# Lagrange-Labs/mapreduce-plonky2

Measured on AMD Instinct MI355X. Metric: leaf proofs/sec (whole node) + NTT GB/s vs HBM peak, 2^20-row table build, 1/2/4/8 GPU, higher is better.
Workload: dtype u64 (Goldilocks field)

## Files before the change

### mapreduce-plonky2_amd/csrc/fri.h

```cpp
#pragma once
#include "gl.cuh"

namespace mp2g {

struct ChState {
  u64 state[12];
  u64 in[8];
  u64 out[8];
  u32 n_in, n_out;
};
struct OracleRef {
  const u64* coeffs;
  const u64* values;
  const u64* levels;
  u64 coeff_bstride, value_bstride, level_bstride;
  u32 w;
};
struct FriShape {
  u32 log_n, rate_bits, cap_h, n_oracles;
  u32 n_polys;
  u32 zs_oracle, zs_count;
  u32 lookup_count;
  OracleRef o[8];
};
GLHD u32 fri_batch_len(const FriShape& sh, u32 batch) { return batch ? sh.zs_count + sh.lookup_count : sh.n_polys; }
GLHD void fri_batch_poly(const FriShape& sh, u32 batch, u32 j, u32& o, u32& p) {
  const u32 zo = sh.zs_oracle, wz = sh.o[zo].w - sh.lookup_count;
  if (batch) { o = zo; p = j < sh.zs_count ? j : wz + (j - sh.zs_count); return; }
  for (u32 oi = 0; oi < sh.n_oracles; oi++) {
    const u32 w = oi == zo ? wz : sh.o[oi].w;
    if (j < w) { o = oi; p = j; return; }
    j -= w;
  }
  o = zo; p = wz + j;
}
struct FriLayers {
  u32 n_layers;
  u32 arity_bits[8];
  const u64* values[8];
  const u64* levels[8];
  u64 value_bstride[8], level_bstride[8];
};

hipError_t challenger_init(hipStream_t s, ChState* st, u32 B);
hipError_t challenger_step(hipStream_t s, int variant, ChState* st, u32 B, const u64* obs, u64 obs_bstride, u32 n_obs,
                           u64* out, u64 out_bstride, u32 n_get);
hipError_t fri_openings(hipStream_t s, const FriShape& sh, u32 B, const u64* zeta, u64 zeta_bstride, u64* out);
hipError_t fri_final_poly(hipStream_t s, const FriShape& sh, u32 B, const u64* alpha, u64 alpha_bstride, const u64* zeta,
                          u64 zeta_bstride, u64* comp, u64* quot, u64* final_poly);
hipError_t fri_fold_values(hipStream_t s, u32 B, u32 log_m, u32 ab, const u64* in, u64 in_bstride, u64* out, u64 out_bstride,
                           const u64* beta, u64 beta_bstride, u64 shift);
hipError_t fri_fold_coeffs(hipStream_t s, u32 B, u32 n_in, u32 ab, const u64* in, u64 in_bstride, u64* out, u64 out_bstride,
                           const u64* beta, u64 beta_bstride, bool aos_out);
hipError_t fri_soa_to_aos(hipStream_t s, u32 B, u32 n, const u64* in, u64 in_bstride, u32 n_in, u64* out, u64 out_bstride);
#define FRI_POW_STRIDE 16
hipError_t fri_pow(hipStream_t s, int variant, const ChState* st, u32 B, u32 bits, u64* witness);
hipError_t fri_queries(hipStream_t s, const FriShape& sh, const FriLayers& ly, u32 B, u32 num_queries, const u64* chal,
                       u64 chal_bstride, u64* proof, u64 proof_bstride, u64 q_off, u64 q_words);
hipError_t bind_public_inputs(hipStream_t s, u32 B, u64* wires, u64 wires_bstride, u64 n, u32 row, const u64* pi_hash);
hipError_t copy_rows(hipStream_t s, u32 B, const u64* src, u64 src_bstride, u64* dst, u64 dst_bstride, u32 words);
}
```

### mapreduce-plonky2_amd/csrc/fri.hip

```cpp
#include "fri.h"
#include "poseidon_wave.cuh"

namespace mp2g {

template <int V>
__device__ void ch_duplex(ChState& c) {
  for (u32 i = 0; i < c.n_in; i++) c.state[i] = c.in[i];
  c.n_in = 0;
  u64 s[12];
#pragma unroll
  for (int i = 0; i < 12; i++) s[i] = c.state[i];
  perm<V>(s);
#pragma unroll
  for (int i = 0; i < 12; i++) c.state[i] = s[i];
#pragma unroll
  for (int i = 0; i < 8; i++) c.out[i] = s[i];
  c.n_out = 8;
}
template <int V>
__global__ void ch_kernel(ChState* st, u32 B, const u64* obs, u64 obs_bstride, u32 n_obs, u64* out, u64 out_bstride, u32 n_get) {
  u32 b = blockIdx.x * blockDim.x + threadIdx.x;
  if (b >= B) return;
  ChState c = st[b];
  const u64* o = obs + b * obs_bstride;
  for (u32 i = 0; i < n_obs; i++) {
    c.n_out = 0;
    c.in[c.n_in++] = o[i];
    if (c.n_in == 8) ch_duplex<V>(c);
  }
  u64* dst = out + b * out_bstride;
  for (u32 i = 0; i < n_get; i++) {
    if (c.n_in || !c.n_out) ch_duplex<V>(c);
    dst[i] = c.out[--c.n_out];
  }
  st[b] = c;
}
__global__ void __launch_bounds__(64) ch_wave_kernel(ChState* st, u32 B, const u64* obs, u64 obs_bstride, u32 n_obs, u64* out,
                                                     u64 out_bstride, u32 n_get) {
  const u32 gid = blockIdx.x * blockDim.x + threadIdx.x;
  const u32 braw = gid >> 4, l = gid & 15;
  const bool active = braw < B;
  const u32 b = active ? braw : B - 1;
  ChState* c = st + b;
  u64 x = l < 12 ? c->state[l] : 0;
  u64 inb = l < 8 ? c->in[l] : 0, outb = l < 8 ? c->out[l] : 0;
  u32 n_in = c->n_in, n_out = c->n_out;
  const u64* o = obs + b * obs_bstride;
  auto duplex = [&]() {
    if (l < n_in) x = inb;
    n_in = 0;
    x = wp2_perm(x, (int)l);
    outb = x;
    n_out = 8;
  };
  for (u32 i = 0; i < n_obs; i++) {
    u64 e = o[i];
    n_out = 0;
    if (l == n_in) inb = e;
    if (++n_in == 8) duplex();
  }
  u64* dst = out + b * out_bstride;
  for (u32 i = 0; i < n_get; i++) {
    if (n_in || !n_out) duplex();
    --n_out;
    if (active && l == n_out) dst[i] = outb;
  }
  if (!active) return;
  if (l < 12) c->state[l] = x;
  if (l < 8) { c->in[l] = inb; c->out[l] = outb; }
  if (l == 0) { c->n_in = n_in; c->n_out = n_out; }
}
__global__ void ch_init_kernel(ChState* st, u32 B) {
  u32 b = blockIdx.x * blockDim.x + threadIdx.x;
  if (b >= B) return;
  ChState c;
  for (int i = 0; i < 12; i++) c.state[i] = 0;
  for (int i = 0; i < 8; i++) { c.in[i] = 0; c.out[i] = 0; }
  c.n_in = c.n_out = 0;
  st[b] = c;
}
hipError_t challenger_init(hipStream_t s, ChState* st, u32 B) {
  hipLaunchKernelGGL(ch_init_kernel, dim3((B + 63) / 64), dim3(64), 0, s, st, B);
  return hipGetLastError();
}
hipError_t challenger_step(hipStream_t s, int variant, ChState* st, u32 B, const u64* obs, u64 obs_bstride, u32 n_obs,
                           u64* out, u64 out_bstride, u32 n_get) {
  if (variant == MP2G_POSEIDON2)
    hipLaunchKernelGGL(ch_wave_kernel, dim3((B * 16 + 63) / 64), dim3(64), 0, s, st, B, obs, obs_bstride, n_obs, out, out_bstride, n_get);
  else
    hipLaunchKernelGGL((ch_kernel<MP2G_POSEIDON>), dim3((B + 63) / 64), dim3(64), 0, s, st, B, obs, obs_bstride, n_obs, out, out_bstride, n_get);
  return hipGetLastError();
}

__global__ void __launch_bounds__(256) openings_kernel(FriShape sh, const u64* zeta , u64 zeta_bstride, u64* out ) {
  const u32 j = blockIdx.x, b = blockIdx.y, t = threadIdx.x;
  const u32 n = 1u << sh.log_n;
  u32 o, p;
  gl2 x = gl2_make(zeta[b * zeta_bstride], zeta[b * zeta_bstride + 1]);
  if (j >= sh.n_polys) {
    fri_batch_poly(sh, 1, j - sh.n_polys, o, p);
    x = gl2_scale(x, gl_root_of_unity(sh.log_n));
  } else {
    fri_batch_poly(sh, 0, j, o, p);
  }
  const u64* c = sh.o[o].coeffs + b * sh.o[o].coeff_bstride + ((u64)p << sh.log_n);
  gl2 x256 = gl2_pow(x, 256), acc = gl2_make(0, 0);
  if (t < n) {
    u32 top = ((n - 1 - t) >> 8);
    for (int k = (int)top; k >= 0; k--) {
      acc = gl2_mul(acc, x256);
      acc.a = gl_add(acc.a, c[t + ((u32)k << 8)]);
    }
    acc = gl2_mul(acc, gl2_pow(x, t));
  }
  __shared__ u64 ra[256], rb[256];
  ra[t] = acc.a; rb[t] = acc.b;
  __syncthreads();
  for (int s = 128; s > 0; s >>= 1) {
    if ((int)t < s) { ra[t] = gl_add(ra[t], ra[t + s]); rb[t] = gl_add(rb[t], rb[t + s]); }
    __syncthreads();
  }
  if (t == 0) {
    u64* d = out + ((u64)b * (sh.n_polys + sh.zs_count + sh.lookup_count) + j) * 2;
    d[0] = ra[0]; d[1] = rb[0];
  }
}

__global__ void __launch_bounds__(256) compose_kernel(FriShape sh, const u64* alpha, u64 alpha_bstride, u64* comp) {
  const u32 n = 1u << sh.log_n;
  const u32 i = blockIdx.x * 256 + threadIdx.x, b = blockIdx.y, batch = blockIdx.z;
  if (i >= n) return;
  gl2 al = gl2_make(alpha[b * alpha_bstride], alpha[b * alpha_bstride + 1]);
  gl2 acc = gl2_make(0, 0);
  const u32 zo = sh.zs_oracle, wz = sh.o[zo].w - sh.lookup_count;
  auto run = [&](u32 o, u32 first, u32 count) {
    const u64* base = sh.o[o].coeffs + b * sh.o[o].coeff_bstride + i;
    for (int p = (int)(first + count) - 1; p >= (int)first; p--) {
      acc = gl2_mul(acc, al);
      acc.a = gl_add(acc.a, base[(u64)p << sh.log_n]);
    }
  };
  if (sh.lookup_count) run(zo, wz, sh.lookup_count);
  if (batch == 0) {
    for (int o = (int)sh.n_oracles - 1; o >= 0; o--) run((u32)o, 0, (u32)o == zo ? wz : sh.o[o].w);
  } else {
    run(zo, 0, sh.zs_count);
  }
  u64* d = comp + (((u64)b * 2 + batch) * 2) * n;
  d[i] = acc.a;
  d[n + i] = acc.b;
}

__global__ void __launch_bounds__(1024) divide_kernel(u32 log_n, const u64* zeta, u64 zeta_bstride, const u64* comp, u64* quot) {
  const u32 n = 1u << log_n, batch = blockIdx.x, b = blockIdx.y, t = threadIdx.x;
  const u32 T = n < 1024 ? n : 1024, S = n / T;
  gl2 z = gl2_make(zeta[b * zeta_bstride], zeta[b * zeta_bstride + 1]);
  if (batch == 1) z = gl2_scale(z, gl_root_of_unity(log_n));
  const u64* c0 = comp + (((u64)b * 2 + batch) * 2) * n;
  const u64* c1 = c0 + n;
  u64* q0 = quot + (((u64)b * 2 + batch) * 2) * n;
  u64* q1 = q0 + n;
  __shared__ u64 la[1024], lb[1024];
  gl2 L = gl2_make(0, 0);
  if (t < T) {
    for (int k = (int)S - 1; k >= 0; k--) {
      L = gl2_mul(L, z);
      L.a = gl_add(L.a, c0[t * S + k]);
      L.b = gl_add(L.b, c1[t * S + k]);
    }
  }
  la[t] = 0; lb[t] = 0;
  __syncthreads();
  if (t < T && t >= 1) { la[t - 1] = L.a; lb[t - 1] = L.b; }
  __syncthreads();
  gl2 zp = gl2_pow(z, S);
  for (u32 d = 1; d < T; d <<= 1) {
    gl2 add = gl2_make(0, 0);
    if (t + d < T) add = gl2_mul(zp, gl2_make(la[t + d], lb[t + d]));
    __syncthreads();
    if (t < T) { la[t] = gl_add(la[t], add.a); lb[t] = gl_add(lb[t], add.b); }
    __syncthreads();
    zp = gl2_mul(zp, zp);
  }
  if (t < T) {
    gl2 s = gl2_make(la[t], lb[t]);
    for (int k = (int)S - 1; k >= 0; k--) {
      u32 i = t * S + k;
      s = gl2_mul(s, z);
      s.a = gl_add(s.a, c0[i]);
      s.b = gl_add(s.b, c1[i]);
      if (i >= 1) { q0[i - 1] = s.a; q1[i - 1] = s.b; }
    }
    if (t == T - 1) { q0[n - 1] = 0; q1[n - 1] = 0; }
  }
}
__global__ void __launch_bounds__(256) combine_kernel(u32 log_n, u32 zs_count, const u64* alpha, u64 alpha_bstride, const u64* quot, u64* final_poly) {
  const u32 n = 1u << log_n, i = blockIdx.x * 256 + threadIdx.x, b = blockIdx.y;
  if (i >= n) return;
  gl2 sh = gl2_pow(gl2_make(alpha[b * alpha_bstride], alpha[b * alpha_bstride + 1]), zs_count);
  const u64* q = quot + (u64)b * 4 * n;
  gl2 r = gl2_add(gl2_mul(gl2_make(q[i], q[n + i]), sh), gl2_make(q[2 * n + i], q[3 * n + i]));
  final_poly[(u64)b * 2 * n + i] = r.a;
  final_poly[(u64)b * 2 * n + n + i] = r.b;
}

template <int AB>
__global__ void __launch_bounds__(256) fold_values_kernel(u32 log_m, const u64* in, u64 in_bstride, u64* out, u64 out_bstride,
                                                            const u64* beta, u64 beta_bstride, u64 shift_inv, u64 w_m_inv, u64 arity_inv) {
  constexpr int A = 1 << AB;
  const u32 m = 1u << log_m, chunks = m >> AB;
  const u32 c = blockIdx.x * 256 + threadIdx.x, b = blockIdx.y;
  if (c >= chunks) return;
  const u64* v0 = in + b * in_bstride + ((u64)c << AB);
  const u64* v1 = v0 + m;
  gl2 x[A];
#pragma unroll
  for (int k = 0; k < A; k++) x[k] = gl2_make(v0[k], v1[k]);
  const u64 wA_inv = gl_pow(w_m_inv, m >> AB);
#pragma unroll
  for (int s = 1; s <= AB; s++) {
    const int mm = 1 << s, h = mm >> 1;
    u64 wstep = wA_inv;
    for (int e = s; e < AB; e++) wstep = gl_sqr(wstep);
    u64 w = 1;
#pragma unroll
    for (int j = 0; j < h; j++) {
#pragma unroll
      for (int k = 0; k < A; k += mm) {
        gl2 t = j == 0 ? x[k + j + h] : gl2_scale(x[k + j + h], w);
        gl2 u = x[k + j];
        x[k + j] = gl2_add(u, t);
        x[k + j + h] = gl2_sub(u, t);
      }
      w = gl_mul(w, wstep);
    }
  }
  u64 x0_inv = gl_mul(shift_inv, gl_pow(w_m_inv, bitrev32(c, log_m - AB)));
  gl2 g = gl2_scale(gl2_make(beta[b * beta_bstride], beta[b * beta_bstride + 1]), x0_inv);
  gl2 acc = x[A - 1];
#pragma unroll
  for (int j = A - 2; j >= 0; j--) acc = gl2_add(gl2_mul(acc, g), x[j]);
  acc = gl2_scale(acc, arity_inv);
  u64* o = out + b * out_bstride;
  o[c] = acc.a;
  o[chunks + c] = acc.b;
}
__global__ void __launch_bounds__(256) fold_coeffs_kernel(u32 n_out, u32 ab, const u64* in, u64 in_bstride, u32 n_in, u64* out, u64 out_bstride,
                                                            const u64* beta, u64 beta_bstride, int aos_out) {
  const u32 i = blockIdx.x * 256 + threadIdx.x, b = blockIdx.y;
  if (i >= n_out) return;
  const u32 A = 1u << ab;
  const u64* c0 = in + b * in_bstride + ((u64)i << ab);
  const u64* c1 = c0 + n_in;
  gl2 be = gl2_make(beta[b * beta_bstride], beta[b * beta_bstride + 1]);
  gl2 acc = gl2_make(0, 0);
  for (int j = (int)A - 1; j >= 0; j--) acc = gl2_add(gl2_mul(acc, be), gl2_make(c0[j], c1[j]));
  u64* o = out + b * out_bstride;
  if (aos_out) { o[2 * i] = acc.a; o[2 * i + 1] = acc.b; }
  else { o[i] = acc.a; o[n_out + i] = acc.b; }
}
__global__ void soa_to_aos_kernel(u32 n, const u64* in, u64 in_bstride, u32 n_in, u64* out, u64 out_bstride) {
  const u32 i = blockIdx.x * blockDim.x + threadIdx.x, b = blockIdx.y;
  if (i >= n) return;
  out[b * out_bstride + 2 * i] = in[b * in_bstride + i];
  out[b * out_bstride + 2 * i + 1] = in[b * in_bstride + n_in + i];
}

#define POW_THREADS 256
#define POW_STRIDE 16
template <int V>
__global__ void __launch_bounds__(POW_THREADS) pow_kernel(const ChState* st, u32 bits, unsigned long long* witness) {
  const u32 b = blockIdx.y;
  const ChState& c = st[b];
  unsigned long long* wit = witness + (u64)b * POW_STRIDE;
  __shared__ unsigned long long s_best;
  u64 base[12];
#pragma unroll
  for (int i = 0; i < 12; i++) base[i] = c.state[i];
  const u32 pos = c.n_in;
#pragma unroll
  for (int i = 0; i < 8; i++)
    if ((u32)i < pos) base[i] = c.in[i];
  const u64 stride = (u64)gridDim.x * blockDim.x;
  for (u64 cand = (u64)blockIdx.x * blockDim.x + threadIdx.x;; cand += stride) {
    if (threadIdx.x == 0) s_best = atomicMin(wit, ~0ull);
    __syncthreads();
    const unsigned long long best = s_best;
    __syncthreads();
    if (cand - threadIdx.x > best) break;
    u64 s[12];
#pragma unroll
    for (int i = 0; i < 12; i++) s[i] = base[i];
#pragma unroll
    for (int i = 0; i < 8; i++)
      if ((u32)i == pos) s[i] = cand;
    perm<V>(s);
    if (cand < GL_P && (bits == 0 || (s[7] >> (64 - bits)) == 0)) atomicMin(wit, (unsigned long long)cand);
  }
}
__global__ void fill_u64_kernel(u64* p, u64 v, u32 n) {
  u32 i = blockIdx.x * blockDim.x + threadIdx.x;
  if (i < n) p[i] = v;
}

__global__ void __launch_bounds__(256) query_kernel(FriShape sh, FriLayers ly, const u64* chal , u64 chal_bstride,
                                                      u64* proof, u64 proof_bstride, u64 q_off, u64 q_words) {
  const u32 q = blockIdx.x, b = blockIdx.y, t = threadIdx.x;
  const u32 lg = sh.log_n + sh.rate_bits;
  const u64 N = (u64)1 << lg;
  u64 x = chal[b * chal_bstride + q] % N;
  u64* o = proof + b * proof_bstride + q_off + q * q_words;
  const u32 depth = lg - sh.cap_h;
  for (u32 oi = 0; oi < sh.n_oracles; oi++) {
    const OracleRef& r = sh.o[oi];
    const u64* vals = r.values + b * r.value_bstride;
    for (u32 p = t; p < r.w; p += 256) o[p] = vals[(u64)p * N + x];
    o += r.w;
    const u64* lv = r.levels + b * r.level_bstride;
    for (u32 e = t; e < depth * 4; e += 256) {
      u32 l = e >> 2, k = e & 3;
      u64 off = 0;
      for (u32 j = 0; j < l; j++) off += (u64)4 << (lg - j);
      o[e] = lv[off + 4 * ((x >> l) ^ 1) + k];
    }
    o += depth * 4;
  }
  u32 clg = lg;
  for (u32 li = 0; li < ly.n_layers; li++) {
    const u32 ab = ly.arity_bits[li], A = 1u << ab;
    const u64 m = (u64)1 << clg;
    x >>= ab;
    clg -= ab;
    const u64* v = ly.values[li] + b * ly.value_bstride[li];
    for (u32 e = t; e < 2 * A; e += 256) o[e] = v[(e & 1) * m + (x << ab) + (e >> 1)];
    o += 2 * A;
    const u32 d2 = clg - sh.cap_h;
    const u64* lv = ly.levels[li] + b * ly.level_bstride[li];
    for (u32 e = t; e < d2 * 4; e += 256) {
      u32 l = e >> 2, k = e & 3;
      u64 off = 0;
      for (u32 j = 0; j < l; j++) off += (u64)4 << (clg - j);
      o[e] = lv[off + 4 * ((x >> l) ^ 1) + k];
    }
    o += d2 * 4;
  }
}
__global__ void copy_rows_kernel(const u64* src, u64 src_bstride, u64* dst, u64 dst_bstride, u32 words) {
  u32 i = blockIdx.x * blockDim.x + threadIdx.x, b = blockIdx.y;
  if (i < words) dst[b * dst_bstride + i] = src[b * src_bstride + i];
}

__global__ void bind_pi_kernel(u64* wires, u64 wires_bstride, u64 n, u32 row, const u64* pi_hash, u32 B) {
  u32 t = blockIdx.x * blockDim.x + threadIdx.x;
  if (t < 4 * B) wires[(t >> 2) * wires_bstride + (u64)(t & 3) * n + row] = pi_hash[t];
}

#define HIPCHK(x) do { hipError_t e_ = (x); if (e_ != hipSuccess) return e_; } while (0)

hipError_t fri_openings(hipStream_t s, const FriShape& sh, u32 B, const u64* zeta, u64 zeta_bstride, u64* out) {
  hipLaunchKernelGGL(openings_kernel, dim3(sh.n_polys + sh.zs_count + sh.lookup_count, B), dim3(256), 0, s, sh, zeta, zeta_bstride, out);
  return hipGetLastError();
}
hipError_t fri_final_poly(hipStream_t s, const FriShape& sh, u32 B, const u64* alpha, u64 alpha_bstride, const u64* zeta, u64 zeta_bstride,
                          u64* comp, u64* quot, u64* final_poly) {
  const u32 n = 1u << sh.log_n;
  hipLaunchKernelGGL(compose_kernel, dim3((n + 255) / 256, B, 2), dim3(256), 0, s, sh, alpha, alpha_bstride, comp);
  hipLaunchKernelGGL(divide_kernel, dim3(2, B), dim3(1024), 0, s, sh.log_n, zeta, zeta_bstride, comp, quot);
  hipLaunchKernelGGL(combine_kernel, dim3((n + 255) / 256, B), dim3(256), 0, s, sh.log_n, sh.zs_count + sh.lookup_count, alpha, alpha_bstride, quot,
                     final_poly);
  return hipGetLastError();
}
hipError_t fri_fold_values(hipStream_t s, u32 B, u32 log_m, u32 ab, const u64* in, u64 in_bstride, u64* out, u64 out_bstride,
                           const u64* beta, u64 beta_bstride, u64 shift) {
  const u32 chunks = (1u << log_m) >> ab;
  const u64 shift_inv = gl_inv(shift), w_m_inv = gl_inv(gl_root_of_unity(log_m)), a_inv = gl_inv((u64)1 << ab);
  dim3 g((chunks + 255) / 256, B), bl(256);
#define FV(N) case N: hipLaunchKernelGGL((fold_values_kernel<N>), g, bl, 0, s, log_m, in, in_bstride, out, out_bstride, beta, beta_bstride, shift_inv, w_m_inv, a_inv); break;
  switch (ab) { FV(1) FV(2) FV(3) FV(4) default: return hipErrorInvalidValue; }
#undef FV
  return hipGetLastError();
}
hipError_t fri_fold_coeffs(hipStream_t s, u32 B, u32 n_in, u32 ab, const u64* in, u64 in_bstride, u64* out, u64 out_bstride,
                           const u64* beta, u64 beta_bstride, bool aos_out) {
  const u32 n_out = n_in >> ab;
  hipLaunchKernelGGL(fold_coeffs_kernel, dim3((n_out + 255) / 256, B), dim3(256), 0, s, n_out, ab, in, in_bstride, n_in, out, out_bstride, beta, beta_bstride, aos_out ? 1 : 0);
  return hipGetLastError();
}
hipError_t fri_soa_to_aos(hipStream_t s, u32 B, u32 n, const u64* in, u64 in_bstride, u32 n_in, u64* out, u64 out_bstride) {
  hipLaunchKernelGGL(soa_to_aos_kernel, dim3((n + 255) / 256, B), dim3(256), 0, s, n, in, in_bstride, n_in, out, out_bstride);
  return hipGetLastError();
}
hipError_t fri_pow(hipStream_t s, int variant, const ChState* st, u32 B, u32 bits, u64* witness) {
  hipLaunchKernelGGL(fill_u64_kernel, dim3((B * POW_STRIDE + 63) / 64), dim3(64), 0, s, witness, ~(u64)0, B * POW_STRIDE);
  const u32 lanes = 1u << 19;
  u32 blocks = lanes / POW_THREADS / (B ? B : 1);
  if (blocks < 8) blocks = 8;
  if (blocks > 1024) blocks = 1024;
  dim3 g(blocks, B), bl(POW_THREADS);
  if (variant == MP2G_POSEIDON2) hipLaunchKernelGGL((pow_kernel<MP2G_POSEIDON2>), g, bl, 0, s, st, bits, (unsigned long long*)witness);
  else hipLaunchKernelGGL((pow_kernel<MP2G_POSEIDON>), g, bl, 0, s, st, bits, (unsigned long long*)witness);
  return hipGetLastError();
}
hipError_t fri_queries(hipStream_t s, const FriShape& sh, const FriLayers& ly, u32 B, u32 num_queries, const u64* chal, u64 chal_bstride,
                       u64* proof, u64 proof_bstride, u64 q_off, u64 q_words) {
  if (!num_queries) return hipSuccess;
  hipLaunchKernelGGL(query_kernel, dim3(num_queries, B), dim3(256), 0, s, sh, ly, chal, chal_bstride, proof, proof_bstride, q_off, q_words);
  return hipGetLastError();
}
hipError_t bind_public_inputs(hipStream_t s, u32 B, u64* wires, u64 wires_bstride, u64 n, u32 row, const u64* pi_hash) {
  hipLaunchKernelGGL(bind_pi_kernel, dim3((4 * B + 63) / 64), dim3(64), 0, s, wires, wires_bstride, n, row, pi_hash, B);
  return hipGetLastError();
}
hipError_t copy_rows(hipStream_t s, u32 B, const u64* src, u64 src_bstride, u64* dst, u64 dst_bstride, u32 words) {
  if (!words) return hipSuccess;
  hipLaunchKernelGGL(copy_rows_kernel, dim3((words + 255) / 256, B), dim3(256), 0, s, src, src_bstride, dst, dst_bstride, words);
  return hipGetLastError();
}
}
```

### mapreduce-plonky2_amd/csrc/gates.h

```cpp
#pragma once
#include "gl.cuh"
#include "mp2g.h"
namespace mp2g {
struct GateTable {
  u32 n_gates, num_selectors;
  u32 num_lookup_selectors;
  mp2g_gate g[MP2G_MAX_GATES];
};
const char* gate_table_check(const GateTable& t, u32 num_constants, u32 wires_w);
u32 gate_num_constraints(const mp2g_gate& g);
u32 gate_degree(const mp2g_gate& g);
hipError_t gate_constraints_lde(hipStream_t s, u32 B, const GateTable& t, const u64* C, const u64* W, u64 w_bstride, u32 lg,
                                const u64* alphas, u64 al_bstride, u32 nc, const u64* pi_hash, u64* q);
hipError_t gate_constraints_points(hipStream_t s, const GateTable& t, const u64* consts, const u64* wires, u64 npts, u32 max_j,
                                   const u64* pi_hash, u64* out);
hipError_t gate_check(hipStream_t s, u32 B, const GateTable& t, const u64* consts, const u64* wires, u64 w_bstride, u64 npts,
                      const u64* pi_hash, u32* flags);
}
```

### mapreduce-plonky2_amd/csrc/gates.hip

```cpp
#include "gates.h"
#include "poseidon.cuh"

namespace mp2g {

u32 gate_num_constraints(const mp2g_gate& g) {
  switch (g.kind) {
    case MP2G_GATE_CONSTANT: return g.p0;
    case MP2G_GATE_PUBLIC_INPUT: return 4;
    case MP2G_GATE_ARITHMETIC: return g.p0;
    case MP2G_GATE_BASE_SUM: return 1 + g.p0;
    case MP2G_GATE_ARITHMETIC_EXT: case MP2G_GATE_MUL_EXT: return 2 * g.p0;
    case MP2G_GATE_POSEIDON2: case MP2G_GATE_POSEIDON: return 1 + 4 + 36 + 22 + 48 + 12;
    case MP2G_GATE_POSEIDON_MDS: return 24;
    case MP2G_GATE_COSET_INTERPOLATION: return 4 + 4 * (((1u << g.p0) - 2) / (g.p1 - 1));
    case MP2G_GATE_U32_ARITHMETIC: return 36 * g.p0;
    case MP2G_GATE_U32_RANGE_CHECK: return 17 * g.p0;
    case MP2G_GATE_U32_SUBTRACTION: return 19 * g.p0;
    case MP2G_GATE_U32_ADD_MANY: return 21 * g.p1;
    case MP2G_GATE_COMPARISON: return g.p1 ? 6 + 5 * g.p1 + (g.p0 + g.p1 - 1) / g.p1 : 0;
    case MP2G_GATE_EXPONENTIATION: return g.p0 + 1;
    case MP2G_GATE_REDUCING: case MP2G_GATE_REDUCING_EXT: return 2 * g.p0;
    case MP2G_GATE_RANDOM_ACCESS: return (g.p0 + 2) * g.p1 + g.p2;
    case MP2G_GATE_U32_INTERLEAVE: return 34 * g.p0;
    case MP2G_GATE_UNINTERLEAVE_TO_B32: case MP2G_GATE_UNINTERLEAVE_TO_U32: return 67 * g.p0;
// ... 273 lines not shown
        s[i + 4] = gl_sub(rhs, delta);
      }
#pragma unroll
      for (int i = 8; i < 12; i++) s[i] = wire(i);
#pragma unroll 1
      for (int r = 0; r < 30; r++) {
        if (r >= 4 && r < 26) {
          u64 in = wire(65 + (r - 4));
          emit(diff(s[0], c_p_rc[12 * r], in));
          s[0] = p2_sbox(in, 0);
#pragma unroll
          for (int i = 1; i < 12; i++) s[i] = gl_addw(s[i], c_p_rc[12 * r + i]);
        } else if (r == 0) {
#pragma unroll
          for (int i = 0; i < 12; i++) s[i] = p2_sbox(s[i], c_p_rc[i]);
        } else {
          const int base = r < 4 ? 29 + 12 * (r - 1) : 87 + 12 * (r - 26);
#pragma unroll
          for (int i = 0; i < 12; i++) {
            u64 in = wire(base + i);
            emit(diff(s[i], c_p_rc[12 * r + i], in));
            s[i] = p2_sbox(in, 0);
          }
        }
        poseidon_mds(s);
      }
#pragma unroll
      for (int i = 0; i < 12; i++) emit(diff0(s[i], wire(12 + i)));
      break;
    }
    case MP2G_GATE_POSEIDON_MDS: {
      u64 s0[12], s1[12];
#pragma unroll
      for (int i = 0; i < 12; i++) { s0[i] = wire(2 * i); s1[i] = wire(2 * i + 1); }
      poseidon_mds(s0);
      poseidon_mds(s1);
#pragma unroll
      for (int i = 0; i < 12; i++) {
        emit(gl_sub(wire(24 + 2 * i), gl_canon(s0[i])));
        emit(gl_sub(wire(25 + 2 * i), gl_canon(s1[i])));
      }
      break;
    }
    case MP2G_GATE_COSET_INTERPOLATION: {
      const u32 npts = 1u << g.p0, deg = g.p1, nint = (npts - 2) / (deg - 1);
      const u32 w_pt = 1 + 2 * npts, w_val = w_pt + 2, w_int = w_val + 2, w_sh = w_int + 4 * nint;
      const Alg pt{wire(w_pt), wire(w_pt + 1)}, sh{wire(w_sh), wire(w_sh + 1)};
      Alg d0 = alg_sub(pt, alg_scale(sh, wire(0)));
      emit(d0.a); emit(d0.b);
      const u64 om = gl_root_of_unity(g.p0), ninv = gl_inv(npts);
      u64 xi = 1;
      Alg ev{0, 0}, pr{1, 0};
      u32 start = 0, end = deg;
      for (u32 c = 0; c <= nint; c++) {
        for (u32 i = start; i < end; i++) {
          Alg val = alg_scale(Alg{wire(1 + 2 * i), wire(2 + 2 * i)}, gl_mul(xi, ninv));
          Alg term{gl_sub(sh.a, xi), sh.b};
          Alg nev = alg_add(alg_mul(ev, term), alg_mul(val, pr));
          pr = alg_mul(pr, term);
          ev = nev;
          xi = gl_mul(xi, om);
        }
        if (c == nint) break;
        Alg iev{wire(w_int + 2 * c), wire(w_int + 2 * c + 1)}, ipr{wire(w_int + 2 * (nint + c)), wire(w_int + 2 * (nint + c) + 1)};
        Alg d1 = alg_sub(iev, ev), d2 = alg_sub(ipr, pr);
        emit(d1.a); emit(d1.b); emit(d2.a); emit(d2.b);
        ev = iev; pr = ipr;
        start = 1 + (deg - 1) * (c + 1);
        end = start + deg - 1 < npts ? start + deg - 1 : npts;
      }
      Alg d3 = alg_sub(Alg{wire(w_val), wire(w_val + 1)}, ev);
      emit(d3.a); emit(d3.b);
      break;
    }
    case MP2G_GATE_U32_ARITHMETIC: {
      const u32 ops = g.p0;
      for (u32 i = 0; i < ops; i++) {
        const u32 b = 6 * i;
        const u64 computed = gl_mul_add(wire(b), wire(b + 1), wire(b + 2));
        const u64 lo = wire(b + 3), hi = wire(b + 4), inv = wire(b + 5);
        const u64 hi_not_max = gl_sub(gl_mul(inv, gl_sub(0xFFFFFFFFull, hi)), 1);
        emit(gl_mul(hi_not_max, lo));
        emit(gl_sub(gl_mul_add(hi, (u64)1 << 32, lo), computed));
        u64 clo = 0, chi = 0, lm[16];
        load16(6 * ops + 32 * i + 16, 16, lm);
#pragma unroll
        for (int j = 15; j >= 0; j--) { emit(range4(lm[j])); chi = horner4(chi, lm[j]); }
        load16(6 * ops + 32 * i, 16, lm);
#pragma unroll
        for (int j = 15; j >= 0; j--) { emit(range4(lm[j])); clo = horner4(clo, lm[j]); }
        emit(subx(clo, lo));
        emit(subx(chi, hi));
      }
      break;
    }
    case MP2G_GATE_U32_RANGE_CHECK: {
      const u32 k = g.p0;
      for (u32 i = 0; i < k; i++) {
        u64 lm[16];
        load16(k + 16 * i, 16, lm);
        u64 acc = 0;
#pragma unroll
        for (int j = 15; j >= 0; j--) acc = horner4(acc, lm[j]);
        emit(subx(acc, wire(i)));
#pragma unroll
        for (int j = 0; j < 16; j++) emit(range4(lm[j]));
      }
      break;
    }
    case MP2G_GATE_U32_SUBTRACTION: {
      const u32 ops = g.p0;
      for (u32 i = 0; i < ops; i++) {
        const u32 b = 5 * i;
        const u64 initial = gl_sub(gl_sub(wire(b), wire(b + 1)), wire(b + 2));
        const u64 res = wire(b + 3), bo = wire(b + 4);
        emit(gl_sub(res, gl_add(initial, gl_mul((u64)1 << 32, bo))));
        u64 comb = 0, lm[16];
        load16(5 * ops + 16 * i, 16, lm);
#pragma unroll
        for (int j = 15; j >= 0; j--) { emit(range4(lm[j])); comb = horner4(comb, lm[j]); }
        emit(subx(comb, res));
        emit(gl_mul(bo, gl_sub(1, bo)));
      }
      break;
    }
    case MP2G_GATE_U32_ADD_MANY: {
      const u32 na = g.p0, ops = g.p1, per = na + 3;
      for (u32 i = 0; i < ops; i++) {
        const u32 b = per * i;
        u64 computed = wire(b + na);
        for (u32 j = 0; j < na; j++) computed = gl_add(computed, wire(b + j));
        const u64 res = wire(b + na + 1), co = wire(b + na + 2);
        emit(gl_sub(gl_mul_add(co, (u64)1 << 32, res), computed));
        u64 cres = 0, ccar = 0, lm[16];
        {
          const u64 l17 = wire(per * ops + 18 * i + 17), l16 = wire(per * ops + 18 * i + 16);
          load16(per * ops + 18 * i, 16, lm);
          emit(range4(l17)); ccar = l17;
          emit(range4(l16)); ccar = horner4(ccar, l16);
        }
#pragma unroll
        for (int j = 15; j >= 0; j--) { emit(range4(lm[j])); cres = horner4(cres, lm[j]); }
        emit(subx(cres, res));
        emit(subx(ccar, co));
      }
      break;
    }
    case MP2G_GATE_COMPARISON: {
      const u32 nch = g.p1, cb = (g.p0 + nch - 1) / nch, cs = 1u << cb;
      const u32 o_fc = 4, o_sc = 4 + nch, o_ed = 4 + 2 * nch, o_ce = 4 + 3 * nch, o_iv = 4 + 4 * nch, o_bits = 4 + 5 * nch;
      u64 a1 = 0, a2 = 0;
      for (u32 i = nch; i-- > 0;) { a1 = gl_add(gl_mul_small(a1, cs), wire(o_fc + i)); a2 = gl_add(gl_mul_small(a2, cs), wire(o_sc + i)); }
      emit(gl_sub(a1, wire(0)));
      emit(gl_sub(a2, wire(1)));
      u64 msd = 0;
      for (u32 i = 0; i < nch; i++) {
        const u64 f = wire(o_fc + i), sc = wire(o_sc + i), ce = wire(o_ce + i), iv = wire(o_iv + i);
        u64 p1 = f, p2 = sc;
        for (u32 x = 1; x < cs; x++) { p1 = mulx(p1, gl_sub(f, x)); p2 = mulx(p2, gl_sub(sc, x)); }
        emit(p1);
        emit(p2);
        const u64 diff = gl_sub(sc, f);
        emit(gl_sub(gl_mul(diff, wire(o_ed + i)), gl_sub(1, ce)));
        emit(gl_mul(ce, diff));
        emit(gl_sub(iv, gl_mul(ce, msd)));
        msd = gl_add(iv, gl_mul(gl_sub(1, ce), diff));
      }
      const u64 msd_w = wire(3);
      emit(gl_sub(msd_w, msd));
      u64 bc = 0;
      for (u32 i = cb + 1; i-- > 0;) bc = gl_add(gl_add(bc, bc), wire(o_bits + i));
      for (u32 i = 0; i <= cb; i++) { const u64 bit = wire(o_bits + i); emit(gl_mul(bit, gl_sub(1, bit))); }
      emit(gl_sub(gl_add(cs, msd_w), bc));
      emit(gl_sub(wire(2), wire(o_bits + cb)));
      break;
    }
    case MP2G_GATE_EXPONENTIATION: {
      const u32 nb = g.p0;
      const u64 base = wire(0);
      u64 prev_int = 1;
      for (u32 i = 0; i < nb; i++) {
        u64 prev = i == 0 ? 1 : gl_mul(prev_int, prev_int);
        u64 bit = wire(1 + (nb - 1 - i));
        u64 mulby = gl_mul_add(bit, base, gl_sub(1, bit));
        u64 cur = wire(nb + 2 + i);
        emit(gl_sub(gl_mul(prev, mulby), cur));
        prev_int = cur;
      }
      emit(gl_sub(wire(nb + 1), prev_int));
      break;
    }
    case MP2G_GATE_REDUCING:
    case MP2G_GATE_REDUCING_EXT: {
      const u32 n = g.p0;
      const bool ext = g.kind == MP2G_GATE_REDUCING_EXT;
      const u32 start_accs = 6 + (ext ? 2 * n : n);
      Alg alpha{wire(2), wire(3)}, acc{wire(4), wire(5)};
      for (u32 i = 0; i < n; i++) {
        Alg coeff = ext ? Alg{wire(6 + 2 * i), wire(7 + 2 * i)} : Alg{wire(6 + i), 0};
        Alg nxt = i == n - 1 ? Alg{wire(0), wire(1)} : Alg{wire(start_accs + 2 * i), wire(start_accs + 2 * i + 1)};
        Alg d = alg_sub(alg_add(alg_mul(acc, alpha), coeff), nxt);
        emit(d.a); emit(d.b);
        acc = nxt;
      }
      break;
    }
    case MP2G_GATE_RANDOM_ACCESS: {
      const u32 bits = g.p0, copies = g.p1, extra = g.p2, vs = 1u << bits;
      const u32 routed = (2 + vs) * copies + extra;
      for (u32 c = 0; c < copies; c++) {
        const u32 w0 = (2 + vs) * c, b0 = routed + c * bits;
        switch (bits) {
          case 1: ra_copy<1>(wire, emit, w0, b0); break;
          case 2: ra_copy<2>(wire, emit, w0, b0); break;
          case 3: ra_copy<3>(wire, emit, w0, b0); break;
          case 4: ra_copy<4>(wire, emit, w0, b0); break;
          default: {
            u64 items[32];
            for (u32 i = 0; i < bits; i++) {
              u64 b = wire(b0 + i);
              emit(gl_mul(b, gl_sub(b, 1)));
            }
            u64 idx = 0;
            for (u32 i = bits; i-- > 0;) idx = gl_add(gl_add(idx, idx), wire(b0 + i));
            emit(gl_sub(idx, wire(w0)));
            {
              const u64 b = wire(b0);
              for (u32 k = 0; k < vs / 2; k++) {
                u64 x = wire(w0 + 2 + 2 * k), y = wire(w0 + 3 + 2 * k);
                items[k] = gl_add(x, gl_mul(b, gl_sub(y, x)));
              }
            }
            for (u32 i = 1, len = vs / 2; i < bits; i++, len >>= 1) {
              const u64 b = wire(b0 + i);
              for (u32 k = 0; k < len / 2; k++) items[k] = gl_add(items[2 * k], gl_mul(b, gl_sub(items[2 * k + 1], items[2 * k])));
            }
            emit(gl_sub(items[0], wire(w0 + 1)));
          }
        }
      }
      for (u32 i = 0; i < extra; i++) emit(gl_sub(cst(i), wire((2 + vs) * copies + i)));
      break;
    }
    case MP2G_GATE_U32_INTERLEAVE: {
      const u32 ops = g.p0;
      u64 bt[16];
      for (u32 i = 0; i < ops; i++) {
        u64 x = 0, xi = 0;
        for (u32 h = 0; h < 2; h++) {
          load16(2 * ops + 32 * i + 16 * h, 16, bt);
#pragma unroll
          for (int j = 0; j < 16; j++) {
            emit(mulx(bt[j], gl_sub(1, bt[j])));
            x = gl_add(gl_add(x, x), bt[j]);
            xi = gl_add(gl_mul_small(xi, 4), bt[j]);
          }
        }
        emit(gl_sub(x, wire(2 * i)));
        emit(gl_sub(xi, wire(2 * i + 1)));
      }
      break;
    }
    case MP2G_GATE_UNINTERLEAVE_TO_B32:
    case MP2G_GATE_UNINTERLEAVE_TO_U32: {
      const u32 ops = g.p0;
      const bool spread = g.kind == MP2G_GATE_UNINTERLEAVE_TO_B32;
      u64 bt[16];
      for (u32 i = 0; i < ops; i++) {
        u64 x = 0, ev = 0, od = 0;
        for (u32 h = 0; h < 4; h++) {
          load16(3 * ops + 64 * i + 16 * h, 16, bt);
#pragma unroll
          for (int j = 0; j < 16; j++) {
            emit(mulx(bt[j], gl_sub(1, bt[j])));
            x = gl_add(gl_add(x, x), bt[j]);
            u64& d = (j & 1) ? ev : od;
            d = gl_add(spread ? gl_mul_small(d, 4) : gl_add(d, d), bt[j]);
          }
        }
        emit(gl_sub(x, wire(3 * i)));
        emit(gl_sub(ev, wire(3 * i + 1)));
        emit(gl_sub(od, wire(3 * i + 2)));
      }
      break;
    }
    default: break;
  }
}

template <class ConstAll>
GLD u64 gate_filter(const GateTable& t, u32 gi, ConstAll call) {
  const mp2g_gate& g = t.g[gi];
  const u64 s = call(g.selector_index);
  u64 f = 1;
  for (u32 r = g.group_start; r < g.group_end; r++)
    if (r != gi) f = gl_mul(f, gl_sub(r, s));
  if (t.num_selectors > 1) f = gl_mul(f, gl_sub(0xFFFFFFFFull, s));
  return f;
}

template <u32 KIND>
__global__ void __launch_bounds__(256) gate_constraints_lde_kernel(mp2g_gate g, u32 gi, u32 num_selectors, u32 cst_off, u32 n_cons,
                                                                   const u64* __restrict__ C, const u64* __restrict__ W,
                                                                   u64 w_bstride, u32 lg, const u64* __restrict__ alphas,
                                                                   u64 al_bstride, u32 nc, const u64* __restrict__ pi_hash,
                                                                   u64* __restrict__ q, int first) {
  __shared__ u64 apw[2][MP2G_MAX_GATE_CONSTRAINTS];
  const u64 N = (u64)1 << lg;
  const u32 p = blockIdx.x * 256 + threadIdx.x, b = blockIdx.y;
  for (u32 j = threadIdx.x; j < 2 * n_cons; j += 256) {
    const u32 a = j >= n_cons ? 1 : 0, e = j - a * n_cons;
    apw[a][e] = a < nc ? gl_pow(alphas[b * al_bstride + a], e) : 0;
  }
  __syncthreads();
  if (p >= N) return;
  g.kind = KIND;
  const u64* w = W + b * w_bstride + p;
  const u64* c = C + p;
  const u64* pih = pi_hash + 4 * b;
  auto wire = [&](u32 j) { return w[(u64)j << lg]; };
  auto cst = [&](u32 j) { return c[(u64)(cst_off + j) << lg]; };
  u64 f = 1;
  {
    const u64 s = c[(u64)g.selector_index << lg];
    for (u32 r = g.group_start; r < g.group_end; r++)
      if (r != gi) f = gl_mul(f, gl_sub(r, s));
    if (num_selectors > 1) f = gl_mul(f, gl_sub(0xFFFFFFFFull, s));
  }
  LazySum acc[2];
  u32 j = 0;
  eval_gate<true>(g, wire, cst, pih, [&](u64 v) {
#pragma unroll
    for (u32 a = 0; a < 2; a++) acc[a].add(v, apw[a][j]);
    j++;
  });
  const u32 i = bitrev32(p, lg);
  for (u32 a = 0; a < nc; a++) {
    u64 r = gl_mul(f, acc[a].value());
    u64* dst = q + (((u64)b * nc + a) << lg) + i;
    *dst = first ? r : gl_add(*dst, r);
  }
}

#define MP2G_MAX_LIGHT_GATES 12
struct LightGates {
  u32 n;
  mp2g_gate g[MP2G_MAX_LIGHT_GATES];
  u32 gi[MP2G_MAX_LIGHT_GATES];
};
static bool gate_is_light(const mp2g_gate& g) {
  switch (g.kind) {
    case MP2G_GATE_CONSTANT: case MP2G_GATE_PUBLIC_INPUT: case MP2G_GATE_ARITHMETIC: case MP2G_GATE_BASE_SUM:
    case MP2G_GATE_ARITHMETIC_EXT: case MP2G_GATE_MUL_EXT: return true;
    default: return false;
  }
}
__global__ void __launch_bounds__(256) gate_constraints_lde_light_kernel(LightGates lg_, u32 num_selectors, u32 cst_off, u32 max_cons,
                                                                         const u64* __restrict__ C, const u64* __restrict__ W,
                                                                         u64 w_bstride, u32 lg, const u64* __restrict__ alphas,
                                                                         u64 al_bstride, u32 nc, const u64* __restrict__ pi_hash,
                                                                         u64* __restrict__ q, int first) {
  __shared__ u64 apw[2][MP2G_MAX_GATE_CONSTRAINTS];
  const u64 N = (u64)1 << lg;
  const u32 p = blockIdx.x * 256 + threadIdx.x, b = blockIdx.y;
  for (u32 j = threadIdx.x; j < 2 * max_cons; j += 256) {
    const u32 a = j >= max_cons ? 1 : 0, e = j - a * max_cons;
    apw[a][e] = a < nc ? gl_pow(alphas[b * al_bstride + a], e) : 0;
  }
  __syncthreads();
  if (p >= N) return;
  const u64* w = W + b * w_bstride + p;
  const u64* c = C + p;
  const u64* pih = pi_hash + 4 * b;
  auto wire = [&](u32 j) { return w[(u64)j << lg]; };
  auto cst = [&](u32 j) { return c[(u64)(cst_off + j) << lg]; };
  u64 total[2] = {0, 0};
  for (u32 k = 0; k < lg_.n; k++) {
    mp2g_gate g = lg_.g[k];
    const u32 gi = lg_.gi[k];
    u64 f = 1;
    {
      const u64 s = c[(u64)g.selector_index << lg];
      for (u32 r = g.group_start; r < g.group_end; r++)
        if (r != gi) f = gl_mul(f, gl_sub(r, s));
      if (num_selectors > 1) f = gl_mul(f, gl_sub(0xFFFFFFFFull, s));
    }
    LazySum acc[2];
    u32 j = 0;
    auto emit = [&](u64 v) {
#pragma unroll
      for (u32 a = 0; a < 2; a++) acc[a].add(v, apw[a][j]);
      j++;
    };
    switch (g.kind) {
#define LIGHT_CASE(K) case K: g.kind = K; eval_gate<true>(g, wire, cst, pih, emit); break;
      LIGHT_CASE(MP2G_GATE_CONSTANT)
      LIGHT_CASE(MP2G_GATE_PUBLIC_INPUT)
      LIGHT_CASE(MP2G_GATE_ARITHMETIC)
      LIGHT_CASE(MP2G_GATE_BASE_SUM)
      LIGHT_CASE(MP2G_GATE_ARITHMETIC_EXT)
      LIGHT_CASE(MP2G_GATE_MUL_EXT)
#undef LIGHT_CASE
      default: break;
    }
    for (u32 a = 0; a < nc; a++) total[a] = gl_add(total[a], gl_mul(f, acc[a].value()));
  }
  const u32 i = bitrev32(p, lg);
  for (u32 a = 0; a < nc; a++) {
    u64* dst = q + (((u64)b * nc + a) << lg) + i;
    *dst = first ? total[a] : gl_add(*dst, total[a]);
  }
}

__global__ void __launch_bounds__(256) gate_constraints_points_kernel(GateTable t, const u64* __restrict__ consts,
                                                                      const u64* __restrict__ wires, u64 npts, u32 max_j,
                                                                      const u64* __restrict__ pih, u64* __restrict__ out) {
  const u64 p = (u64)blockIdx.x * 256 + threadIdx.x;
  if (p >= npts) return;
  auto wire = [&](u32 j) { return wires[(u64)j * npts + p]; };
  auto call = [&](u32 j) { return consts[(u64)j * npts + p]; };
  const u32 ns = t.num_selectors + t.num_lookup_selectors;
  auto cst = [&](u32 j) { return consts[(u64)(ns + j) * npts + p]; };
  for (u32 j = 0; j < max_j; j++) out[(u64)j * npts + p] = 0;
  for (u32 gi = 0; gi < t.n_gates; gi++) {
    if (t.g[gi].kind == MP2G_GATE_NOOP) continue;
    const u64 f = gate_filter(t, gi, call);
    u32 j = 0;
    eval_gate<false>(t.g[gi], wire, cst, pih, [&](u64 v) {
      u64* o = out + (u64)j * npts + p;
      *o = gl_add(*o, gl_mul(f, v));
      j++;
    });
  }
}

__global__ void __launch_bounds__(256) gate_check_kernel(GateTable t, const u64* __restrict__ consts, const u64* __restrict__ wires,
                                                         u64 w_bstride, u64 npts, const u64* __restrict__ pi_hash, u32* __restrict__ flags) {
  const u64 p = (u64)blockIdx.x * 256 + threadIdx.x;
  const u32 b = blockIdx.y;
  if (p >= npts) return;
  const u64* w = wires + b * w_bstride;
  auto wire = [&](u32 j) { return w[(u64)j * npts + p]; };
  auto call = [&](u32 j) { return consts[(u64)j * npts + p]; };
  const u32 ns = t.num_selectors + t.num_lookup_selectors;
  auto cst = [&](u32 j) { return consts[(u64)(ns + j) * npts + p]; };
  bool bad = false;
  for (u32 gi = 0; gi < t.n_gates; gi++) {
    if (t.g[gi].kind == MP2G_GATE_NOOP) continue;
    if (gate_filter(t, gi, call) == 0) continue;
    eval_gate<false>(t.g[gi], wire, cst, pi_hash + 4 * b, [&](u64 v) { bad |= v != 0; });
  }
  if (bad) atomicOr(&flags[b], 2u);
}
hipError_t gate_check(hipStream_t s, u32 B, const GateTable& t, const u64* consts, const u64* wires, u64 w_bstride, u64 npts,
                      const u64* pi_hash, u32* flags) {
  if (!npts || !B) return hipSuccess;
  hipLaunchKernelGGL(gate_check_kernel, dim3((u32)((npts + 255) / 256), B), dim3(256), 0, s, t, consts, wires, w_bstride, npts, pi_hash,
                     flags);
  return hipGetLastError();
}

hipError_t gate_constraints_lde(hipStream_t s, u32 B, const GateTable& t, const u64* C, const u64* W, u64 w_bstride, u32 lg,
                                const u64* alphas, u64 al_bstride, u32 nc, const u64* pi_hash, u64* q) {
  if (nc < 1 || nc > 2) return hipErrorInvalidValue;
  const u64 N = (u64)1 << lg;
  const dim3 grid((u32)((N + 255) / 256), B), block(256);
  int first = 1;
  LightGates lgs{};
  u32 light_cons = 0;
  for (u32 gi = 0; gi < t.n_gates; gi++) {
    const u32 n_cons = gate_num_constraints(t.g[gi]);
    if (n_cons && gate_is_light(t.g[gi]) && lgs.n < MP2G_MAX_LIGHT_GATES) {
      lgs.g[lgs.n] = t.g[gi]; lgs.gi[lgs.n] = gi; lgs.n++;
      if (n_cons > light_cons) light_cons = n_cons;
    }
  }
  if (lgs.n < 2) lgs.n = 0;
  if (lgs.n) {
    hipLaunchKernelGGL(gate_constraints_lde_light_kernel, grid, block, 0, s, lgs, t.num_selectors, t.num_selectors + t.num_lookup_selectors,
                       light_cons, C, W, w_bstride, lg, alphas, al_bstride, nc, pi_hash, q, first);
    first = 0;
  }
  for (u32 gi = 0; gi < t.n_gates; gi++) {
    const mp2g_gate& g = t.g[gi];
    const u32 n_cons = gate_num_constraints(g);
    if (!n_cons) continue;
    bool fused = false;
    for (u32 k = 0; k < lgs.n; k++) fused |= lgs.gi[k] == gi;
    if (fused) continue;
#define GATE_CASE(K)                                                                                                        \
  case K:                                                                                                                   \
    hipLaunchKernelGGL(gate_constraints_lde_kernel<K>, grid, block, 0, s, g, gi, t.num_selectors,                          \
                       t.num_selectors + t.num_lookup_selectors, n_cons, C, W, w_bstride, lg, alphas, al_bstride, nc, pi_hash, q, \
                       first);                                                                                              \
    break;
    switch (g.kind) {
      GATE_CASE(MP2G_GATE_CONSTANT)
      GATE_CASE(MP2G_GATE_PUBLIC_INPUT)
      GATE_CASE(MP2G_GATE_ARITHMETIC)
      GATE_CASE(MP2G_GATE_BASE_SUM)
      GATE_CASE(MP2G_GATE_ARITHMETIC_EXT)
      GATE_CASE(MP2G_GATE_MUL_EXT)
      GATE_CASE(MP2G_GATE_POSEIDON2)
      GATE_CASE(MP2G_GATE_EXPONENTIATION)
      GATE_CASE(MP2G_GATE_REDUCING)
      GATE_CASE(MP2G_GATE_REDUCING_EXT)
      GATE_CASE(MP2G_GATE_RANDOM_ACCESS)
      GATE_CASE(MP2G_GATE_POSEIDON)
      GATE_CASE(MP2G_GATE_POSEIDON_MDS)
      GATE_CASE(MP2G_GATE_COSET_INTERPOLATION)
      GATE_CASE(MP2G_GATE_U32_ARITHMETIC)
      GATE_CASE(MP2G_GATE_U32_RANGE_CHECK)
      GATE_CASE(MP2G_GATE_U32_SUBTRACTION)
      GATE_CASE(MP2G_GATE_U32_ADD_MANY)
      GATE_CASE(MP2G_GATE_COMPARISON)
      GATE_CASE(MP2G_GATE_U32_INTERLEAVE)
      GATE_CASE(MP2G_GATE_UNINTERLEAVE_TO_B32)
      GATE_CASE(MP2G_GATE_UNINTERLEAVE_TO_U32)
      default: return hipErrorInvalidValue;
    }
#undef GATE_CASE
    first = 0;
  }
  if (first) return hipMemsetAsync(q, 0, (size_t)B * nc * N * sizeof(u64), s);
  return hipGetLastError();
}
hipError_t gate_constraints_points(hipStream_t s, const GateTable& t, const u64* consts, const u64* wires, u64 npts, u32 max_j,
                                   const u64* pi_hash, u64* out) {
  if (!npts) return hipSuccess;
  hipLaunchKernelGGL(gate_constraints_points_kernel, dim3((u32)((npts + 255) / 256)), dim3(256), 0, s, t, consts, wires, npts, max_j,
                     pi_hash, out);
  return hipGetLastError();
}
}
```

### mapreduce-plonky2_amd/csrc/ntt.h

```cpp
#pragma once
#include "gl.cuh"
#include <map>
#include <memory>

namespace mp2g {

struct NttPlan {
  u32 log_n = 0, log_n1 = 0, log_n2 = 0;
  u64 *tw_a = nullptr, *tw_b = nullptr, *tw4_lo = nullptr, *tw4_hi = nullptr, *tw4_full = nullptr;
  u64 *tc_a = nullptr, *tc_b = nullptr;
  u64 n_inv = 0;
  ~NttPlan();
};
struct CosetTables {
  u32 log_n = 0, logK = 0;
  u64 shift = 0;
  u64 *lo = nullptr, *hi = nullptr, *full = nullptr;
  ~CosetTables();
};

struct NttEngine {
  hipStream_t stream = nullptr;
  std::map<u32, std::unique_ptr<NttPlan>> plans;
  std::map<u64, std::unique_ptr<CosetTables>> cosets;
  u64* scratch = nullptr;
  size_t scratch_words = 0;
  u64 generation = 0;
  ~NttEngine();

  hipError_t plan(u32 log_n, bool inverse, NttPlan** out);
  hipError_t coset(u32 log_n, u32 logK, u64 shift, CosetTables** out);
  hipError_t ensure_scratch(size_t words);
  hipError_t run(const u64* in, u64* out, u32 log_n, u32 polys, u32 logK, u64 in_poly_stride,
                 u64 out_poly_stride, bool inverse, const CosetTables* pre, bool bitrev_out);
  hipError_t scale_powers(u64* data, u32 log_n, u32 batch, u64 base, u64 first);
};

}
```

### mapreduce-plonky2_amd/csrc/ntt.hip

```cpp
#include "ntt.h"
#include <cstdlib>

namespace mp2g {

__device__ __forceinline__ int lds_pad(int a) { return a + (a >> 4); }

struct NttArgs {
  const u64* in;
  u64* out;
  u64 in_poly_stride, out_poly_stride;
  u32 logK;
  u32 log_n, log_n1, log_n2;
  u32 batch;
  const u64* tw;
  const u64* tw4_lo;
  const u64* tw4_hi;
  const u64* pre_lo;
  const u64* pre_hi;
  const u64* tw4_full;
  const u64* pre_full;
  u64 post;
  u32 bitrev_out;
  u32 inverse;
  const u64* tc;
// ... 242 lines not shown
  }
}

template <int LT, int LW>
__global__ void __launch_bounds__((NttGeom<LT, LW>::NT)) ntt_cols_kernel(NttArgs a, u64* dst_dense) {
  constexpr int T = 1 << LT, W = 1 << LW, E = T << LW, NT = NttGeom<LT, LW>::NT;
  extern __shared__ __align__(16) u64 smem[];
  u64* s = smem;
  u64* tw = smem + lds_pad(E) + 1;
  const int tid = threadIdx.x;
  for (int i = tid; i < R8Tw<LT>::LDS_WORDS; i += NT) tw[i] = a.tw[R8Tw<LT>::LDS_OFF + i];
  const u32 tiles_per = 1u << (a.log_n2 - LW);
  u32 bid = blockIdx.x;
  if ((gridDim.x & 7) == 0) bid = (bid & 7) * (gridDim.x >> 3) + (bid >> 3);
  const u32 b = bid / tiles_per, c0 = (bid % tiles_per) << LW;
  const u32 coset = b & ((1u << a.logK) - 1);
  const u64* src = in_base(a, b);
  for (int e = tid; e < E; e += NT) {
    int c = e & (W - 1), j = e >> LW;
    u64 v = src[((u64)j << a.log_n2) + c0 + c];
    if (a.pre_full) {
      v = gl_mul(v, a.pre_full[((u64)coset << a.log_n) + ((u64)j << a.log_n2) + c0 + c]);
    } else if (a.pre_lo) {
      v = gl_mul(v, a.pre_lo[((u64)coset << a.log_n2) + c0 + c]);
      v = gl_mul(v, a.pre_hi[((u64)coset << LT) + j]);
    }
    s[lds_pad(e)] = v;
  }
  __syncthreads();
  dif_all<LT, LT - 1, true, LW, NT>(s, tw, a.tw, tid, a.inverse != 0);
  u64* dst = dst_dense ? dst_dense + (u64)b * ((u64)1 << a.log_n) : out_base(a, b);
  for (int e = tid; e < E; e += NT) {
    int c = e & (W - 1), j = e >> LW;
    u64 v = s[lds_pad(e)];
    u64 w;
    if (a.tw4_full) {
      w = a.tw4_full[((u64)j << a.log_n2) + c0 + c];
    } else {
      u32 k1 = bitrev32((u32)j, LT);
      u32 ex = (c0 + c) * k1;
      w = gl_mul(a.tw4_lo[ex & 4095], a.tw4_hi[ex >> 12]);
    }
    dst[((u64)j << a.log_n2) + c0 + c] = gl_mul(v, w);
  }
}

template <int LT, int LW, bool COLS> struct WaveGeom {
  static constexpr int NBR = LT > 12 ? 2 : 1;
  static constexpr int LTS = LT - 3 * NBR;
  static constexpr int LWL = 9 - LTS;
  static constexpr bool OK = LT >= 3 && LT <= 13 && (!COLS || LT <= 12) && ((1 << LT) << LW) == 8 * NttGeom<LT, LW>::NT && (!COLS || LW >= LWL);
};
template <int LT, int LW, bool COLS> struct ShiftGeom {
  using G = WaveGeom<LT, LW, COLS>;
  static constexpr int L0 = LT - 3;
  static constexpr bool OK = G::OK && G::NBR == 1 && G::LTS >= 6 && (COLS ? (LW + L0 - 3 >= 6) : (LW == 0 && L0 - 3 >= 6));
  static constexpr int TC_WORDS = 64 << (L0 - 3);
};
__device__ __forceinline__ void wave_sync() {
  __builtin_amdgcn_fence(__ATOMIC_RELEASE, "wavefront");
  __builtin_amdgcn_wave_barrier();
  __builtin_amdgcn_fence(__ATOMIC_ACQUIRE, "wavefront");
}
template <int LT, int LTS, int HI, int R, bool COLS, int LWL, int LWS, bool MERGED = false>
__device__ __forceinline__ void wave_round(u64* s, int base, const u64* tw, int lane, bool inverse, const u64* __restrict__ tcw = nullptr) {
  constexpr int LO = HI - R + 1, WL = 1 << LWL;
  constexpr int ITEMS = 512 >> R;
#pragma unroll
  for (int item0 = 0; item0 < ITEMS; item0 += 64) {
    int item = item0 + lane;
    int c, rest;
    if (COLS) { c = item & (WL - 1); rest = item >> LWL; }
    else { rest = item & ((1 << (LTS - R)) - 1); c = item >> (LTS - R); }
    int below = rest & ((1 << LO) - 1), above = rest >> LO;
    int j0 = (above << (HI + 1)) | below;
    u64 x[1 << R];
#pragma unroll
    for (int m = 0; m < (1 << R); m++) {
      int j = j0 + (m << LO);
      x[m] = s[lds_pad(base + (COLS ? (j << LWS) + c : (c << LTS) + j))];
    }
    butterfly<LT, HI, R, false, MERGED>(x, below, tw, tcw, inverse);
#pragma unroll
    for (int m = 0; m < (1 << R); m++) {
      int j = j0 + (m << LO);
      s[lds_pad(base + (COLS ? (j << LWS) + c : (c << LTS) + j))] = x[m];
    }
  }
}
template <int LT, int LTS, int HI, bool COLS, int LWL, int LWS, bool SHIFT = false>
__device__ __forceinline__ void wave_rounds(u64* s, int base, const u64* tw, int lane, bool inverse, const u64* __restrict__ tcw = nullptr) {
  if constexpr (HI >= 0) {
    constexpr int R = (HI + 1 >= 3) ? 3 : HI + 1;
    wave_sync();
    wave_round<LT, LTS, HI, R, COLS, LWL, LWS, SHIFT>(s, base, tw, lane, inverse, tcw);
    wave_rounds<LT, LTS, HI - R, COLS, LWL, LWS, false>(s, base, tw, lane, inverse);
  }
}

template <int LT, int LW, bool SHIFT = false>
__global__ void __launch_bounds__((NttGeom<LT, LW>::NT)) __attribute__((amdgpu_waves_per_eu(8))) ntt_rows_v2_kernel(NttArgs a) {
  using G = WaveGeom<LT, LW, false>;
  static_assert(!SHIFT || ShiftGeom<LT, LW, false>::OK, "tile shape without wave-uniform shift twiddles");
  constexpr int T = 1 << LT, E = T << LW, NT = NttGeom<LT, LW>::NT, LTS = G::LTS, L0 = LT - 3;
  extern __shared__ __align__(16) u64 smem[];
  u64* s = smem;
  u64* tw = smem + lds_pad(E) + 1;
  const int tid = threadIdx.x, lane = tid & 63, wave = tid >> 6;
  for (int i = tid; i < R8Tw<LT>::LDS_WORDS; i += NT) tw[i] = a.tw[R8Tw<LT>::LDS_OFF + i];
  const u32 n1 = 1u << a.log_n1;
  const u64 total_rows = (u64)a.batch << a.log_n1;
  const u64 row0 = (u64)blockIdx.x << LW;
  const bool two_pass = a.log_n1 != 0, inverse = a.inverse != 0;
  {
    const int c = tid >> L0, below = tid & ((1 << L0) - 1);
    const u64 g = row0 + c;
    u64 x[8];
    if (g < total_rows) {
      u32 b = (u32)(g >> a.log_n1), jr = (u32)(g & (n1 - 1));
      if (two_pass) {
        const u64* src = out_base(a, b) + ((u64)jr << LT);
#pragma unroll
        for (int m = 0; m < 8; m++) x[m] = src[below + (m << L0)];
      } else {
        const u64* src = in_base(a, b);
#pragma unroll
        for (int m = 0; m < 8; m++) x[m] = src[below + (m << L0)];
        if (a.pre_lo) {
          const u64* pre = a.pre_lo + ((u64)(b & ((1u << a.logK) - 1)) << LT);
#pragma unroll
          for (int m = 0; m < 8; m++) x[m] = gl_mul(x[m], pre[below + (m << L0)]);
        }
      }
    } else {
#pragma unroll
      for (int m = 0; m < 8; m++) x[m] = 0;
    }
    if constexpr (SHIFT) {
      butterfly<LT, 2, 3>(x, 0, nullptr, nullptr, inverse);
      shift_twiddles(x, __builtin_amdgcn_readfirstlane(below >> (L0 - 3)), inverse);
    } else {
      butterfly<LT, LT - 1, 3, true>(x, below, tw, a.tw, inverse);
    }
#pragma unroll
    for (int m = 0; m < 8; m++) s[lds_pad((c << LT) + below + (m << L0))] = x[m];
  }
  __syncthreads();
  if constexpr (G::NBR == 2) {
    dif_round<LT, LT - 4, 3, false, LW, NT>(s, tw, a.tw, tid, inverse);
    __syncthreads();
  }
  if constexpr (SHIFT) {
    const int r = __builtin_amdgcn_readfirstlane((int)bitrev32((u32)(wave & 7), 3));
    wave_rounds<LT, LTS, LTS - 1, false, G::LWL, 0, true>(s, wave << 9, tw, lane, inverse, a.tc + (r << (L0 - 3)));
  } else {
    wave_rounds<LT, LTS, LTS - 1, false, G::LWL, 0>(s, wave << 9, tw, lane, inverse);
  }
  if (a.bitrev_out) {
    wave_sync();
    u64 v[8];
#pragma unroll
    for (int k = 0; k < 8; k++) v[k] = s[lds_pad((wave << 9) + lane + (k << 6))];
    if (a.post) {
#pragma unroll
      for (int k = 0; k < 8; k++) v[k] = gl_mul(v[k], a.post);
    }
#pragma unroll
    for (int k = 0; k < 8; k++) {
      int e = (wave << 9) + lane + (k << 6);
      int r = e >> LT, p = e & (T - 1);
      u64 g = row0 + r;
      if (g >= total_rows) continue;
      u32 b = (u32)(g >> a.log_n1), jr = (u32)(g & (n1 - 1));
      out_base(a, b)[((u64)jr << LT) + p] = v[k];
    }
  } else {
    __syncthreads();
    for (int e = tid; e < E; e += NT) {
      int r = e >> LT, p = e & (T - 1);
      u64 g = row0 + r;
      if (g >= total_rows) continue;
      u32 b = (u32)(g >> a.log_n1), jr = (u32)(g & (n1 - 1));
      u64 v = s[lds_pad((r << LT) + (int)bitrev32((u32)p, LT))];
      if (a.post) v = gl_mul(v, a.post);
      out_base(a, b)[((u64)jr << LT) + p] = v;
    }
  }
}

template <int LT, int LW, bool SHIFT = false>
__global__ void __launch_bounds__((NttGeom<LT, LW>::NT)) __attribute__((amdgpu_waves_per_eu(8))) ntt_cols_v2_kernel(NttArgs a, u64* dst_dense) {
  using G = WaveGeom<LT, LW, true>;
  static_assert(!SHIFT || ShiftGeom<LT, LW, true>::OK, "tile shape without wave-uniform shift twiddles");
  constexpr int W = 1 << LW, E = (1 << LT) << LW, NT = NttGeom<LT, LW>::NT, LTS = G::LTS, LWL = G::LWL;
  extern __shared__ __align__(16) u64 smem[];
  u64* s = smem;
  u64* tw = smem + lds_pad(E) + 1;
  const int tid = threadIdx.x, lane = tid & 63, wave = tid >> 6;
  for (int i = tid; i < R8Tw<LT>::LDS_WORDS; i += NT) tw[i] = a.tw[R8Tw<LT>::LDS_OFF + i];
  const u32 tiles_per = 1u << (a.log_n2 - LW);
  u32 bid = blockIdx.x;
  if ((gridDim.x & 7) == 0) bid = (bid & 7) * (gridDim.x >> 3) + (bid >> 3);
  const u32 b = bid / tiles_per, c0 = (bid % tiles_per) << LW;
  const u32 coset = b & ((1u << a.logK) - 1);
  const u64* src = in_base(a, b);
  const bool inverse = a.inverse != 0;
  {
    const int c = tid & (W - 1), below = tid >> LW;
    u64 x[8];
#pragma unroll
    for (int m = 0; m < 8; m++) x[m] = src[((u64)(below + (m << LTS)) << a.log_n2) + c0 + c];
    if (a.pre_full) {
      const u64* pre = a.pre_full + ((u64)coset << a.log_n) + c0 + c;
#pragma unroll
      for (int m = 0; m < 8; m++) x[m] = gl_mul(x[m], pre[(u64)(below + (m << LTS)) << a.log_n2]);
    } else if (a.pre_lo) {
      u64 pl = a.pre_lo[((u64)coset << a.log_n2) + c0 + c];
#pragma unroll
      for (int m = 0; m < 8; m++) x[m] = gl_mul(gl_mul(x[m], pl), a.pre_hi[((u64)coset << LT) + below + (m << LTS)]);
    }
    if constexpr (SHIFT) {
      butterfly<LT, 2, 3>(x, 0, nullptr, nullptr, inverse);
      shift_twiddles(x, __builtin_amdgcn_readfirstlane(below >> (LTS - 3)), inverse);
    } else {
      butterfly<LT, LT - 1, 3, true>(x, below, tw, a.tw, inverse);
    }
#pragma unroll
    for (int m = 0; m < 8; m++) s[lds_pad(((below + (m << LTS)) << LW) + c)] = x[m];
  }
  __syncthreads();
  {
    constexpr int GW = W >> LWL;
    const int cg = wave & (GW - 1), jh = wave / GW;
    if constexpr (SHIFT) {
      const int r = __builtin_amdgcn_readfirstlane((int)bitrev32((u32)jh, 3));
      wave_rounds<LT, LTS, LTS - 1, true, LWL, LW, true>(s, ((jh << LTS) << LW) + (cg << LWL), tw, lane, inverse, a.tc + (r << (LTS - 3)));
    } else {
      wave_rounds<LT, LTS, LTS - 1, true, LWL, LW>(s, ((jh << LTS) << LW) + (cg << LWL), tw, lane, inverse);
    }
  }
  __syncthreads();
  u64* dst = dst_dense ? dst_dense + (u64)b * ((u64)1 << a.log_n) : out_base(a, b);
#pragma unroll
  for (int k = 0; k < 8; k++) {
    int e = tid + k * NT;
    int c = e & (W - 1), j = e >> LW;
    u64 v = s[lds_pad(e)];
    u64 w;
    if (a.tw4_full) {
      w = a.tw4_full[((u64)j << a.log_n2) + c0 + c];
    } else {
      u32 k1 = bitrev32((u32)j, LT);
      u32 ex = (c0 + c) * k1;
      w = gl_mul(a.tw4_lo[ex & 4095], a.tw4_hi[ex >> 12]);
    }
    dst[((u64)j << a.log_n2) + c0 + c] = gl_mul(v, w);
  }
}

__global__ void r8_round_twiddles_kernel(u64* out, u64 w, u32 lo, u32 shift) {
  u32 i = blockIdx.x * blockDim.x + threadIdx.x;
  if (i >= (7u << lo)) return;
  u32 r = (i >> lo) + 1, below = i & ((1u << lo) - 1);
  out[i] = gl_pow(w, ((u64)below << shift) * r);
}
__global__ void merged_twiddles_kernel(u64* out, u64 w, u32 lb) {
  u32 i = blockIdx.x * blockDim.x + threadIdx.x;
  if (i >= (64u << lb)) return;
  out[i] = gl_pow(w, (u64)(i & ((1u << lb) - 1)) * (i >> lb));
}
__global__ void powers_kernel(u64* out, u64 base, u64 first, u64 stride_exp, u32 count) {
  u32 i = blockIdx.x * blockDim.x + threadIdx.x;
  if (i >= count) return;
  out[i] = gl_mul(first, gl_pow(base, (u64)i * stride_exp));
}
__global__ void coset_tables_kernel(u64* lo, u64* hi, u64 shift, u64 w_nk, u32 log_n1, u32 log_n2, u32 K) {
  u32 i = blockIdx.x * blockDim.x + threadIdx.x;
  u32 n1 = 1u << log_n1, n2 = 1u << log_n2;
  u32 per = n1 + n2;
  if (i >= per * K) return;
  u32 j = i / per, r = i % per;
  u64 sj = gl_mul(shift, gl_pow(w_nk, j));
  if (r < n2) lo[(u64)j * n2 + r] = gl_pow(sj, r);
  else hi[(u64)j * n1 + (r - n2)] = gl_pow(sj, (u64)(r - n2) << log_n2);
}
__global__ void tw4_full_kernel(u64* out, u64 wn, u32 log_n1, u32 log_n2) {
  u64 i = (u64)blockIdx.x * blockDim.x + threadIdx.x;
  if (i >= ((u64)1 << (log_n1 + log_n2))) return;
  u32 j = (u32)(i >> log_n2), i2 = (u32)(i & ((1u << log_n2) - 1));
  out[i] = gl_pow(wn, (u64)i2 * bitrev32(j, log_n1));
}
__global__ void pre_full_kernel(u64* out, u64 shift, u64 w_nk, u32 log_n, u32 K) {
  u64 i = (u64)blockIdx.x * blockDim.x + threadIdx.x;
  if (i >= ((u64)K << log_n)) return;
  u32 c = (u32)(i >> log_n);
  out[i] = gl_pow(gl_mul(shift, gl_pow(w_nk, c)), i & (((u64)1 << log_n) - 1));
}
__global__ void scale_powers_kernel(u64* data, u32 log_n, u32 batch, u64 base, u64 first) {
  u64 i = (u64)blockIdx.x * blockDim.x + threadIdx.x;
  if (i >= ((u64)batch << log_n)) return;
  u64 k = i & (((u64)1 << log_n) - 1);
  data[i] = gl_mul(data[i], gl_mul(first, gl_pow(base, k)));
}

#define HIPCHK(x) do { hipError_t e_ = (x); if (e_ != hipSuccess) return e_; } while (0)

static hipError_t dev_alloc(u64** p, size_t words) { return hipMalloc((void**)p, words * sizeof(u64)); }

NttPlan::~NttPlan() {
  (void)hipFree(tw_a); (void)hipFree(tw_b); (void)hipFree(tw4_lo); (void)hipFree(tw4_hi); (void)hipFree(tw4_full);
  (void)hipFree(tc_a); (void)hipFree(tc_b);
}
CosetTables::~CosetTables() { (void)hipFree(lo); (void)hipFree(hi); (void)hipFree(full); }

static u32 split_log_n1(u32 log_n) {
  if (log_n <= 13) return 0;
  u32 l1 = (log_n + 1) / 2;
  if (log_n >= 22) l1 = log_n - 12;
  return l1;
}
template <int LT> static constexpr int rows_lw() { return LT >= 12 ? 0 : (LT == 11 ? 2 : 12 - LT); }
template <int LT> static constexpr int cols_lw() { return LT >= 11 ? 2 : (LT == 10 ? 3 : 12 - LT); }
template <int LT> static constexpr bool shift_rows_lt() { return ShiftGeom<LT, rows_lw<LT>(), false>::OK; }
template <int LT> static constexpr bool shift_cols_lt() { return ShiftGeom<LT, cols_lw<LT>(), true>::OK; }
static bool shift_rows_ok(u32 lt) {
  switch (lt) { case 12: return shift_rows_lt<12>(); case 13: return shift_rows_lt<13>(); default: return false; }
}
static bool shift_cols_ok(u32 lt) {
  switch (lt) { case 9: return shift_cols_lt<9>(); case 10: return shift_cols_lt<10>(); case 11: return shift_cols_lt<11>(); case 12: return shift_cols_lt<12>(); default: return false; }
}
hipError_t NttEngine::plan(u32 log_n, bool inverse, NttPlan** out) {
  u32 key = log_n * 2 + (inverse ? 1 : 0);
  auto it = plans.find(key);
  if (it != plans.end()) { *out = it->second.get(); return hipSuccess; }
  std::unique_ptr<NttPlan> p(new NttPlan());
  p->log_n = log_n;
  p->log_n1 = split_log_n1(log_n);
  p->log_n2 = log_n - p->log_n1;
  u64 wn = gl_root_of_unity(log_n);
  if (inverse) wn = gl_inv(wn);
  auto powers = [&](u64** dst, u64 base, u32 count) -> hipError_t {
    HIPCHK(dev_alloc(dst, count ? count : 1));
    if (count) hipLaunchKernelGGL(powers_kernel, dim3((count + 255) / 256), dim3(256), 0, stream, *dst, base, (u64)1, (u64)1, count);
    return hipGetLastError();
  };
  u64 w2 = gl_pow(wn, (u64)1 << p->log_n1), w1 = gl_pow(wn, (u64)1 << p->log_n2);
  auto stage_tw = [&](u64** dst, u64 base, u32 lt) -> hipError_t {
    HIPCHK(dev_alloc(dst, (size_t)1 << lt));
    u32 off = 0;
    for (u32 rho = 0; (int)lt - 3 - 3 * (int)rho >= 1; rho++) {
      u32 lo = lt - 3 - 3 * rho, count = 7u << lo;
      hipLaunchKernelGGL(r8_round_twiddles_kernel, dim3((count + 255) / 256), dim3(256), 0, stream, *dst + off, base, lo, 3 * rho);
      HIPCHK(hipGetLastError());
      off += count;
    }
    return hipSuccess;
  };
  auto merged_tw = [&](u64** dst, u64 base, u32 lt) -> hipError_t {
    const u32 lb = lt - 6, count = 64u << lb;
    HIPCHK(dev_alloc(dst, count));
    hipLaunchKernelGGL(merged_twiddles_kernel, dim3((count + 255) / 256), dim3(256), 0, stream, *dst, base, lb);
    return hipGetLastError();
  };
  HIPCHK(stage_tw(&p->tw_b, w2, p->log_n2));
  if (shift_rows_ok(p->log_n2)) HIPCHK(merged_tw(&p->tc_b, w2, p->log_n2));
  if (p->log_n1) {
    HIPCHK(stage_tw(&p->tw_a, w1, p->log_n1));
    if (shift_cols_ok(p->log_n1)) HIPCHK(merged_tw(&p->tc_a, w1, p->log_n1));
    HIPCHK(powers(&p->tw4_lo, wn, 4096));
    HIPCHK(powers(&p->tw4_hi, gl_pow(wn, 4096), log_n > 12 ? (1u << (log_n - 12)) : 1));
    if (log_n <= 22) {
      HIPCHK(dev_alloc(&p->tw4_full, (size_t)1 << log_n));
      hipLaunchKernelGGL(tw4_full_kernel, dim3((u32)((((u64)1 << log_n) + 255) / 256)), dim3(256), 0, stream, p->tw4_full, wn, p->log_n1, p->log_n2);
      HIPCHK(hipGetLastError());
    }
  }
  p->n_inv = inverse ? gl_inv(((u64)1 << log_n) % GL_P) : 0;
  *out = p.get();
  plans[key] = std::move(p);
  return hipSuccess;
}

hipError_t NttEngine::coset(u32 log_n, u32 logK, u64 shift, CosetTables** out) {
  u64 key = ((u64)log_n << 8 | logK) ^ (shift * 0x9E3779B97F4A7C15ULL);
  auto it = cosets.find(key);
  if (it != cosets.end() && it->second->shift == shift && it->second->log_n == log_n && it->second->logK == logK) {
    *out = it->second.get(); return hipSuccess;
  }
  std::unique_ptr<CosetTables> c(new CosetTables());
  c->log_n = log_n; c->logK = logK; c->shift = shift;
  u32 log_n1 = split_log_n1(log_n), log_n2 = log_n - log_n1;
  u32 K = 1u << logK, n1 = 1u << log_n1, n2 = 1u << log_n2;
  HIPCHK(dev_alloc(&c->lo, (size_t)K * n2));
  HIPCHK(dev_alloc(&c->hi, (size_t)K * n1));
  u32 total = (n1 + n2) * K;
  hipLaunchKernelGGL(coset_tables_kernel, dim3((total + 255) / 256), dim3(256), 0, stream, c->lo, c->hi, shift,
                     gl_root_of_unity(log_n + logK), log_n1, log_n2, K);
  HIPCHK(hipGetLastError());
  if (log_n1 && ((u64)K << log_n) <= ((u64)1 << 23)) {
    HIPCHK(dev_alloc(&c->full, (size_t)K << log_n));
    u64 tot = (u64)K << log_n;
    hipLaunchKernelGGL(pre_full_kernel, dim3((u32)((tot + 255) / 256)), dim3(256), 0, stream, c->full, shift,
                       gl_root_of_unity(log_n + logK), log_n, K);
    HIPCHK(hipGetLastError());
  }
  *out = c.get();
  if (cosets.count(key)) generation++;
  cosets[key] = std::move(c);
  return hipSuccess;
}

hipError_t NttEngine::ensure_scratch(size_t words) {
  if (words <= scratch_words) return hipSuccess;
  if (scratch) HIPCHK(hipFree(scratch));
  scratch = nullptr; scratch_words = 0;
  generation++;
  HIPCHK(dev_alloc(&scratch, words));
  scratch_words = words;
  return hipSuccess;
}

template <int LT, int LW> static size_t lds_bytes() {
  int e = (1 << LT) << LW;
  return (size_t)(e + (e >> 4) + 1 + R8Tw<LT>::LDS_WORDS + 1) * sizeof(u64);
}

#define MP2G_MAX_DEVICES 64
static bool* attr_flag(bool* flags) {
  int dev = 0;
  (void)hipGetDevice(&dev);
  return &flags[dev >= 0 && dev < MP2G_MAX_DEVICES ? dev : 0];
}
static bool use_v1() {
  static int v = -1;
  if (v < 0) { const char* e = getenv("MP2G_NTT_V1"); v = e ? atoi(e) : 0; }
  return v != 0;
}
template <int LT, int LW>
static hipError_t launch_rows(const NttArgs& a, bool nat_two_pass, hipStream_t st) {
  constexpr int NT = NttGeom<LT, LW>::NT;
  size_t lds = lds_bytes<LT, LW>();
  u64 total_rows = (u64)a.batch << a.log_n1;
  if constexpr (ShiftGeom<LT, LW, false>::OK) {
    if (!nat_two_pass && !use_v1() && a.tc) {
      static bool flags[MP2G_MAX_DEVICES];
      bool* attr = attr_flag(flags);
      if (!*attr) { HIPCHK(hipFuncSetAttribute((const void*)ntt_rows_v2_kernel<LT, LW, true>, hipFuncAttributeMaxDynamicSharedMemorySize, (int)lds)); *attr = true; }
      hipLaunchKernelGGL((ntt_rows_v2_kernel<LT, LW, true>), dim3((u32)((total_rows + (1u << LW) - 1) >> LW)), dim3(NT), lds, st, a);
      return hipGetLastError();
    }
  }
  if constexpr (WaveGeom<LT, LW, false>::OK) {
    if (!nat_two_pass && !use_v1()) {
      static bool flags[MP2G_MAX_DEVICES];
      bool* attr = attr_flag(flags);
      if (!*attr) { HIPCHK(hipFuncSetAttribute((const void*)ntt_rows_v2_kernel<LT, LW>, hipFuncAttributeMaxDynamicSharedMemorySize, (int)lds)); *attr = true; }
      hipLaunchKernelGGL((ntt_rows_v2_kernel<LT, LW>), dim3((u32)((total_rows + (1u << LW) - 1) >> LW)), dim3(NT), lds, st, a);
      return hipGetLastError();
    }
  }
  if (nat_two_pass) {
    static bool flags[MP2G_MAX_DEVICES];
    bool* attr = attr_flag(flags);
    if (!*attr) { HIPCHK(hipFuncSetAttribute((const void*)ntt_rows_nat_kernel<LT, LW>, hipFuncAttributeMaxDynamicSharedMemorySize, (int)lds)); *attr = true; }
    hipLaunchKernelGGL((ntt_rows_nat_kernel<LT, LW>), dim3((u32)(total_rows >> LW)), dim3(NT), lds, st, a);
  } else {
    static bool flags[MP2G_MAX_DEVICES];
    bool* attr = attr_flag(flags);
    if (!*attr) { HIPCHK(hipFuncSetAttribute((const void*)ntt_rows_kernel<LT, LW>, hipFuncAttributeMaxDynamicSharedMemorySize, (int)lds)); *attr = true; }
    hipLaunchKernelGGL((ntt_rows_kernel<LT, LW>), dim3((u32)((total_rows + (1u << LW) - 1) >> LW)), dim3(NT), lds, st, a);
  }
  return hipGetLastError();
}
template <int LT, int LW>
static hipError_t launch_cols(const NttArgs& a, u64* dst_dense, hipStream_t st) {
  constexpr int NT = NttGeom<LT, LW>::NT;
  size_t lds = lds_bytes<LT, LW>();
  if constexpr (ShiftGeom<LT, LW, true>::OK) {
    if (!use_v1() && a.tc) {
      static bool flags[MP2G_MAX_DEVICES];
      bool* attr = attr_flag(flags);
      if (!*attr) { HIPCHK(hipFuncSetAttribute((const void*)ntt_cols_v2_kernel<LT, LW, true>, hipFuncAttributeMaxDynamicSharedMemorySize, (int)lds)); *attr = true; }
      hipLaunchKernelGGL((ntt_cols_v2_kernel<LT, LW, true>), dim3(a.batch << (a.log_n2 - LW)), dim3(NT), lds, st, a, dst_dense);
      return hipGetLastError();
    }
  }
  if constexpr (WaveGeom<LT, LW, true>::OK) {
    if (!use_v1()) {
      static bool flags[MP2G_MAX_DEVICES];
      bool* attr = attr_flag(flags);
      if (!*attr) { HIPCHK(hipFuncSetAttribute((const void*)ntt_cols_v2_kernel<LT, LW>, hipFuncAttributeMaxDynamicSharedMemorySize, (int)lds)); *attr = true; }
      hipLaunchKernelGGL((ntt_cols_v2_kernel<LT, LW>), dim3(a.batch << (a.log_n2 - LW)), dim3(NT), lds, st, a, dst_dense);
      return hipGetLastError();
    }
  }
  static bool flags[MP2G_MAX_DEVICES];
  bool* attr = attr_flag(flags);
  if (!*attr) { HIPCHK(hipFuncSetAttribute((const void*)ntt_cols_kernel<LT, LW>, hipFuncAttributeMaxDynamicSharedMemorySize, (int)lds)); *attr = true; }
  hipLaunchKernelGGL((ntt_cols_kernel<LT, LW>), dim3(a.batch << (a.log_n2 - LW)), dim3(NT), lds, st, a, dst_dense);
  return hipGetLastError();
}
#define ROWS_CASE(N) case N: return launch_rows<N, rows_lw<N>()>(a, nat, st);
static hipError_t dispatch_rows(u32 lt, const NttArgs& a, bool nat, hipStream_t st) {
  switch (lt) {
    ROWS_CASE(1) ROWS_CASE(2) ROWS_CASE(3) ROWS_CASE(4) ROWS_CASE(5) ROWS_CASE(6)
    ROWS_CASE(7) ROWS_CASE(8) ROWS_CASE(9) ROWS_CASE(10) ROWS_CASE(11) ROWS_CASE(12) ROWS_CASE(13)
    default: return hipErrorInvalidValue;
  }
}
#define COLS_CASE(N) case N: return launch_cols<N, cols_lw<N>()>(a, dense, st);
static hipError_t dispatch_cols(u32 lt, const NttArgs& a, u64* dense, hipStream_t st) {
  switch (lt) {
    COLS_CASE(7) COLS_CASE(8) COLS_CASE(9) COLS_CASE(10) COLS_CASE(11) COLS_CASE(12)
    default: return hipErrorInvalidValue;
  }
}

hipError_t NttEngine::run(const u64* in, u64* out, u32 log_n, u32 polys, u32 logK, u64 in_poly_stride,
                          u64 out_poly_stride, bool inverse, const CosetTables* pre, bool bitrev_out) {
  if (log_n == 0 || log_n > 24) return hipErrorInvalidValue;
  NttPlan* p;
  HIPCHK(plan(log_n, inverse, &p));
  NttArgs a{};
  a.in = in; a.out = out;
  a.in_poly_stride = in_poly_stride; a.out_poly_stride = out_poly_stride;
  a.logK = logK; a.log_n = log_n; a.log_n1 = p->log_n1; a.log_n2 = p->log_n2;
  a.batch = polys << logK;
  a.tw4_lo = p->tw4_lo; a.tw4_hi = p->tw4_hi; a.tw4_full = p->tw4_full;
  a.pre_lo = pre ? pre->lo : nullptr; a.pre_hi = pre ? pre->hi : nullptr; a.pre_full = pre ? pre->full : nullptr;
  a.post = p->n_inv;
  a.bitrev_out = bitrev_out ? 1 : 0;
  a.inverse = inverse ? 1 : 0;
  if (p->log_n1 == 0) {
    a.tw = p->tw_b; a.tc = p->tc_b;
    return dispatch_rows(p->log_n2, a, false, stream);
  }
  u64* dense = nullptr;
  if (!bitrev_out) {
    HIPCHK(ensure_scratch((size_t)a.batch << log_n));
    dense = scratch;
  }
  a.tw = p->tw_a; a.tc = p->tc_a;
  HIPCHK(dispatch_cols(p->log_n1, a, dense, stream));
  a.tw = p->tw_b; a.tc = p->tc_b;
  a.pre_lo = a.pre_hi = a.pre_full = nullptr;
  if (!bitrev_out) a.in = dense;
  return dispatch_rows(p->log_n2, a, !bitrev_out, stream);
}

hipError_t NttEngine::scale_powers(u64* data, u32 log_n, u32 batch, u64 base, u64 first) {
  u64 total = (u64)batch << log_n;
  hipLaunchKernelGGL(scale_powers_kernel, dim3((u32)((total + 255) / 256)), dim3(256), 0, stream, data, log_n, batch, base, first);
  return hipGetLastError();
}

NttEngine::~NttEngine() { if (scratch) (void)hipFree(scratch); }

}
```

### mapreduce-plonky2_amd/csrc/prover.hip

```cpp
#include "ctx.h"
#include "fri.h"
#include "zperm.h"
#include "gates.h"
#include "lookup.h"
#include <cstring>
#include <new>
#include <vector>

using namespace mp2g;

#define CK(x) do { hipError_t e_ = (x); if (e_ != hipSuccess) return fail("%s: %s (%s:%d)", #x, hipGetErrorString(e_), __FILE__, __LINE__); } while (0)
#define NEED(c, msg) do { if (!(c)) return fail("invalid argument: %s", msg); } while (0)

struct mp2g_challenger {
  mp2g_ctx* ctx = nullptr;
  int variant = 0;
  uint32_t count = 0;
  DevBuf st;
};

struct mp2g_prover {
  mp2g_ctx* ctx = nullptr;
  mp2g_fri_params P{};
  uint32_t B = 0;
  uint32_t Bcap = 0;
  bool have_pre = false;
  size_t capw = 0, levels_words = 0, proof_words = 0, q_words = 0, q_off = 0, final_off = 0, final_len = 0, n_open = 0;
  DevBuf coeffs[8], values[8], levels[8];
  DevBuf ch, chal, zeta, alpha, betas, comp, quot, final_poly, witness, qchal;
  DevBuf fvals[9], flevels[8], fcoeffs[9];
  uint32_t num_routed = 0, degree = 0;
  bool quotient = false;
  DevBuf pre_values, zs_values, chunk_q, bg, alphas, qvals;
  GateTable gates{};
  LookupDev lookups{};
  DevBuf lut_tables, lut_eval;
  int64_t pi_row = -1;
  bool wcheck = false;
  DevBuf wflags;
  bool timing = false;
  hipEvent_t ev[MP2G_N_STAGES + 1] = {};
  bool graph_on = false;
  int plain_calls = 0;
  hipGraphExec_t gexec = nullptr;
  const void* gkey[12] = {};
  u64 ggen = 0;
  void drop_graph() {
    if (gexec) (void)hipGraphExecDestroy(gexec);
    gexec = nullptr;
  }
  std::vector<std::pair<DevBuf*, size_t>> shared;
  const u64* bound_base = nullptr;
  size_t bound_total = 0;
  bool counted = false;
  hipError_t want(DevBuf& d, size_t bytes) {
    if (!ctx->share_scratch) return d.alloc(bytes);
    for (auto& e : shared)
      if (e.first == &d) { e.second = bytes; bound_base = nullptr; return hipSuccess; }
    shared.emplace_back(&d, bytes);
    bound_base = nullptr;
    return hipSuccess;
  }
  ~mp2g_prover() {
    drop_graph();
    for (hipEvent_t e : ev)
      if (e) (void)hipEventDestroy(e);
  }
};
#define STAGE_MARK(pr, i) do { if ((pr)->timing) CK(hipEventRecord((pr)->ev[i], (pr)->ctx->stream)); } while (0)

namespace {
struct ProverGuard {
  mp2g_prover* pr = nullptr;
  ~ProverGuard();
};
}

namespace mp2g {
int params_check(const mp2g_fri_params* p) {
  NEED(p, "params");
  NEED(p->variant <= 1, "variant");
  NEED(p->log_n >= 1 && p->log_n <= 20, "1 <= log_n <= 20");
  NEED(p->rate_bits >= 1 && p->rate_bits <= 6, "rate_bits");
  NEED(p->n_oracles >= 1 && p->n_oracles <= 8, "n_oracles");
  NEED(p->n_layers <= 8, "n_layers");
  NEED(p->pow_bits <= 32, "pow_bits <= 32");
  NEED(p->num_queries <= 64, "num_queries <= 64");
  NEED(p->zs_oracle < p->n_oracles && p->zs_count <= p->oracle_w[p->zs_oracle], "zs_oracle/zs_count");
  uint32_t deg = p->log_n, lg = p->log_n + p->rate_bits;
  NEED(p->cap_height <= lg, "cap_height");
  for (uint32_t i = 0; i < p->n_layers; i++) {
    NEED(p->arity_bits[i] >= 1 && p->arity_bits[i] <= 4, "arity_bits in 1..4");
    NEED(deg >= p->arity_bits[i], "arity exceeds degree");
    deg -= p->arity_bits[i];
    lg -= p->arity_bits[i];
    NEED(lg >= p->cap_height, "layer smaller than cap");
  }
  for (uint32_t o = 0; o < p->n_oracles; o++) NEED(p->oracle_w[o] >= 1, "oracle_w >= 1");
  NEED(p->num_lookup_polys <= 16, "num_lookup_polys <= 16");
  NEED((uint64_t)p->zs_count * (1 + p->num_lookup_polys) <= p->oracle_w[p->zs_oracle], "Z + lookup polynomials exceed the zs oracle");
  return 0;
}
}

extern "C" {

uint32_t mp2g_reduction_arity_bits(uint32_t degree_bits, uint32_t rate_bits, uint32_t cap_height, uint32_t arity_bits,
                                   uint32_t final_poly_bits, uint32_t* out) {
  uint32_t n = 0;
  if (arity_bits == 0) return 0;
  while (degree_bits > final_poly_bits && degree_bits >= arity_bits && degree_bits + rate_bits >= cap_height + arity_bits && n < 8) {
    out[n++] = arity_bits;
    degree_bits -= arity_bits;
  }
  return n;
}
size_t mp2g_fri_n_openings(const mp2g_fri_params* p) {
  size_t t = p->zs_count + (size_t)p->zs_count * p->num_lookup_polys;
  for (uint32_t o = 0; o < p->n_oracles; o++) t += p->oracle_w[o];
  return t;
}
static size_t query_words(const mp2g_fri_params* p) {
  uint32_t lg = p->log_n + p->rate_bits;
  size_t q = 0;
  for (uint32_t o = 0; o < p->n_oracles; o++) q += p->oracle_w[o] + 4 * (lg - p->cap_height);
  uint32_t cur = lg;
  for (uint32_t i = 0; i < p->n_layers; i++) {
    cur -= p->arity_bits[i];
    q += ((size_t)2 << p->arity_bits[i]) + 4 * (cur - p->cap_height);
  }
  return q;
}
static size_t final_poly_len(const mp2g_fri_params* p) {
  uint32_t deg = p->log_n;
  for (uint32_t i = 0; i < p->n_layers; i++) deg -= p->arity_bits[i];
  return (size_t)1 << deg;
}
size_t mp2g_fri_proof_words(const mp2g_fri_params* p) {
  return p->n_layers * ((size_t)4 << p->cap_height) + p->num_queries * query_words(p) + 2 * final_poly_len(p) + 1;
}

int mp2g_challenger_create(mp2g_ctx* c, int variant, uint32_t count, mp2g_challenger** out) {
  NEED(c && out && count >= 1, "ctx/out/count");
  NEED(variant == 0 || variant == 1, "variant");
  mp2g_challenger* ch = new (std::nothrow) mp2g_challenger();
  if (!ch) return fail("out of memory");
  ch->ctx = c; ch->variant = variant; ch->count = count;
  hipError_t e = ch->st.alloc(sizeof(ChState) * count);
  if (e == hipSuccess) e = challenger_init(c->stream, (ChState*)ch->st.p, count);
  if (e != hipSuccess) { delete ch; return fail("challenger_create: %s", hipGetErrorString(e)); }
  *out = ch;
  return 0;
}
int mp2g_challenger_observe(mp2g_challenger* ch, const uint64_t* elems, uint32_t n) {
  NEED(ch && (elems || !n), "challenger/elems");
  if (!n) return 0;
  mp2g_ctx* c = ch->ctx;
  DevBuf d;
  CK(d.alloc((size_t)ch->count * n * sizeof(u64)));
  CK(hipMemcpyAsync(d.p, elems, (size_t)ch->count * n * sizeof(u64), hipMemcpyHostToDevice, c->stream));
  CK(challenger_step(c->stream, ch->variant, (ChState*)ch->st.p, ch->count, d.p, n, n, d.p, 0, 0));
  CK(hipStreamSynchronize(c->stream));
  return 0;
}
int mp2g_challenger_get(mp2g_challenger* ch, uint32_t n, uint64_t* out) {
  NEED(ch && (out || !n), "challenger/out");
  if (!n) return 0;
  mp2g_ctx* c = ch->ctx;
  DevBuf d;
  CK(d.alloc((size_t)ch->count * n * sizeof(u64)));
  CK(challenger_step(c->stream, ch->variant, (ChState*)ch->st.p, ch->count, d.p, 0, 0, d.p, n, n));
  CK(hipMemcpyAsync(out, d.p, (size_t)ch->count * n * sizeof(u64), hipMemcpyDeviceToHost, c->stream));
  CK(hipStreamSynchronize(c->stream));
  return 0;
}
void mp2g_challenger_free(mp2g_challenger* ch) {
  if (!ch) return;
  (void)hipStreamSynchronize(ch->ctx->stream);
  delete ch;
}

int mp2g_fri_fold(mp2g_ctx* c, const uint64_t* evals, uint32_t log_m, uint32_t arity_bits, const uint64_t beta[2],
                  uint64_t shift, uint64_t* out) {
  NEED(c && evals && beta && out, "ctx/pointers");
  NEED(arity_bits >= 1 && arity_bits <= 4 && log_m >= arity_bits && log_m <= 28, "arity_bits in 1..4, log_m >= arity_bits");
  NEED(shift != 0 && shift < GL_P, "shift");
  const size_t m = (size_t)1 << log_m, m2 = m >> arity_bits;
  std::vector<u64> soa(2 * m);
  for (size_t i = 0; i < m; i++) { soa[i] = evals[2 * i]; soa[m + i] = evals[2 * i + 1]; }
  DevBuf din, dout, db;
  CK(din.alloc(2 * m * sizeof(u64)));
  CK(dout.alloc(2 * m2 * sizeof(u64)));
  CK(db.alloc(2 * sizeof(u64)));
  CK(hipMemcpyAsync(din.p, soa.data(), 2 * m * sizeof(u64), hipMemcpyHostToDevice, c->stream));
  CK(hipMemcpyAsync(db.p, beta, 2 * sizeof(u64), hipMemcpyHostToDevice, c->stream));
  CK(fri_fold_values(c->stream, 1, log_m, arity_bits, din.p, 0, dout.p, 0, db.p, 0, shift));
  std::vector<u64> res(2 * m2);
  CK(hipMemcpyAsync(res.data(), dout.p, 2 * m2 * sizeof(u64), hipMemcpyDeviceToHost, c->stream));
  CK(hipStreamSynchronize(c->stream));
  for (size_t i = 0; i < m2; i++) { out[2 * i] = res[i]; out[2 * i + 1] = res[m2 + i]; }
  return 0;
}
int mp2g_fri_pow(mp2g_ctx* c, int variant, const uint64_t state[12], uint32_t pos, uint32_t bits, uint64_t* witness) {
  NEED(c && state && witness, "ctx/pointers");
  NEED(variant == 0 || variant == 1, "variant");
  NEED(pos < 8 && bits <= 32, "pos < 8, bits <= 32");
  ChState h{};
  for (int i = 0; i < 12; i++) h.state[i] = state[i];
  for (uint32_t i = 0; i < pos; i++) h.in[i] = state[i];
  h.n_in = pos;
  DevBuf ds, dw;
  CK(ds.alloc(sizeof(ChState)));
  CK(dw.alloc(FRI_POW_STRIDE * sizeof(u64)));
  CK(hipMemcpyAsync(ds.p, &h, sizeof h, hipMemcpyHostToDevice, c->stream));
  CK(fri_pow(c->stream, variant, (const ChState*)ds.p, 1, bits, dw.p));
  CK(hipMemcpyAsync(witness, dw.p, sizeof(u64), hipMemcpyDeviceToHost, c->stream));
  CK(hipStreamSynchronize(c->stream));
  return 0;
}

static int prover_create_impl(mp2g_ctx* c, const mp2g_fri_params* params, uint32_t batch, bool alloc_oracles, mp2g_prover** out) {
  NEED(c && out, "ctx/out");
  NEED(batch >= 1 && batch <= 4096, "1 <= batch <= 4096");
  int rc = params_check(params);
  if (rc) return rc;
  mp2g_prover* pr = new (std::nothrow) mp2g_prover();
  if (!pr) return fail("out of memory");
  pr->ctx = c; pr->P = *params; pr->B = pr->Bcap = batch;
  const mp2g_fri_params& P = pr->P;
  const size_t n = (size_t)1 << P.log_n, N = n << P.rate_bits, B = batch;
  const uint32_t lg = P.log_n + P.rate_bits;
  pr->capw = (size_t)4 << P.cap_height;
  pr->levels_words = merkle_levels_words(lg, P.cap_height);
  pr->proof_words = mp2g_fri_proof_words(&P);
  pr->q_words = query_words(&P);
  pr->q_off = P.n_layers * pr->capw;
  pr->final_len = final_poly_len(&P);
  pr->final_off = pr->q_off + P.num_queries * pr->q_words;
  pr->n_open = mp2g_fri_n_openings(&P);
  hipError_t e = hipSuccess;
  auto A = [&](DevBuf& d, size_t words) { if (e == hipSuccess) e = d.alloc(words * sizeof(u64)); };
  auto S = [&](DevBuf& d, size_t words) { if (e == hipSuccess) e = pr->want(d, words * sizeof(u64)); };
  for (uint32_t o = 0; o < P.n_oracles && alloc_oracles; o++) {
    if (o == 0) {
      A(pr->coeffs[o], (size_t)P.oracle_w[o] * n); A(pr->values[o], (size_t)P.oracle_w[o] * N); A(pr->levels[o], pr->levels_words);
    } else {
      S(pr->coeffs[o], B * P.oracle_w[o] * n); S(pr->values[o], B * P.oracle_w[o] * N); S(pr->levels[o], B * pr->levels_words);
    }
  }
  if (e == hipSuccess) e = pr->ch.alloc(B * sizeof(ChState));
  A(pr->chal, B * 8); A(pr->zeta, B * 2); A(pr->alpha, B * 2); A(pr->betas, B * 16);
  S(pr->comp, B * 4 * n); S(pr->quot, B * 4 * n); S(pr->final_poly, B * 2 * n);
  A(pr->witness, B * FRI_POW_STRIDE); A(pr->qchal, B * (P.num_queries ? P.num_queries : 1));
  size_t m = N, nc = n;
  uint32_t clg = lg;
  S(pr->fvals[0], B * 2 * m);
  for (uint32_t li = 0; li < P.n_layers; li++) {
    clg -= P.arity_bits[li];
    S(pr->flevels[li], B * merkle_levels_words(clg, P.cap_height));
    m >>= P.arity_bits[li]; nc >>= P.arity_bits[li];
    S(pr->fvals[li + 1], B * 2 * m);
    S(pr->fcoeffs[li + 1], B * 2 * nc);
  }
  if (e != hipSuccess) { delete pr; return fail("prover_create: %s", hipGetErrorString(e)); }
  *out = pr;
  return 0;
}
int mp2g_prover_create(mp2g_ctx* c, const mp2g_fri_params* params, uint32_t batch, mp2g_prover** out) {
  return prover_create_impl(c, params, batch, true, out);
}
}
ProverGuard::~ProverGuard() { if (pr) mp2g_prover_free(pr); }
extern "C" {
void mp2g_prover_free(mp2g_prover* pr) {
  if (!pr) return;
  mp2g_ctx* c = pr->ctx;
  (void)hipStreamSynchronize(c->stream);
  const bool counted = pr->counted;
  delete pr;
  if (counted && c->scratch_users && --c->scratch_users == 0) c->prover_scratch.release();
}
static hipError_t commit_oracle_coeffs(mp2g_prover* pr, uint32_t o, uint32_t nb) {
  mp2g_ctx* c = pr->ctx;
  const mp2g_fri_params& P = pr->P;
  const u64 n = (u64)1 << P.log_n, N = n << P.rate_bits;
  const uint32_t w = P.oracle_w[o], lg = P.log_n + P.rate_bits;
  hipError_t e;
  CosetTables* pre;
  e = c->ntt.coset(P.log_n, P.rate_bits, GL_MULT_GEN, &pre);
  if (e != hipSuccess) return e;
  e = c->ntt.run(pr->coeffs[o].p, pr->values[o].p, P.log_n, nb * w, P.rate_bits, n, N, false, pre, true);
  if (e != hipSuccess) return e;
  e = leaf_hash_poly_major(c->stream, P.variant, pr->values[o].p, w, N, N, pr->levels[o].p, nb, (u64)w * N, pr->levels_words);
  if (e != hipSuccess) return e;
  return merkle_reduce(c->stream, P.variant, pr->levels[o].p, lg, P.cap_height, nb, pr->levels_words);
}
static hipError_t commit_oracle(mp2g_prover* pr, uint32_t o, const u64* d_values, uint32_t nb) {
  const mp2g_fri_params& P = pr->P;
  const u64 n = (u64)1 << P.log_n;
  hipError_t e = pr->ctx->ntt.run(d_values, pr->coeffs[o].p, P.log_n, nb * P.oracle_w[o], 0, n, n, true, nullptr, false);
  if (e != hipSuccess) return e;
  return commit_oracle_coeffs(pr, o, nb);
}
int mp2g_prover_set_preprocessed_dev(mp2g_prover* pr, const uint64_t* d_values) {
  NEED(pr && d_values, "prover/values");
  const size_t words = (size_t)pr->P.oracle_w[0] << pr->P.log_n;
  CK(pr->pre_values.alloc(words * sizeof(u64)));
  CK(hipMemcpyAsync(pr->pre_values.p, d_values, words * sizeof(u64), hipMemcpyDeviceToDevice, pr->ctx->stream));
  CK(commit_oracle(pr, 0, (const u64*)d_values, 1));
  pr->drop_graph();
  pr->have_pre = true;
  return 0;
}
int mp2g_prover_enable_permutation(mp2g_prover* pr, uint32_t num_routed, uint32_t degree) {
  NEED(pr && pr->have_pre, "call mp2g_prover_set_preprocessed_dev first");
  const mp2g_fri_params& P = pr->P;
  NEED(P.n_oracles >= 3 && P.zs_oracle == 2, "needs wires = oracle 1 and Z/partial products = oracle 2");
  NEED(degree >= 1 && num_routed >= degree && num_routed % degree == 0 && num_routed / degree <= 16, "num_routed/degree");
  NEED(num_routed <= P.oracle_w[0] && num_routed <= P.oracle_w[1], "num_routed exceeds the sigma / wire counts");
  NEED(P.zs_count >= 1 && P.zs_count <= 2, "1 or 2 challenges");
  NEED(P.oracle_w[2] == P.zs_count * (num_routed / degree + P.num_lookup_polys), "oracle_w[2] must be zs_count * (num_routed/degree + num_lookup_polys)");
  const size_t n = (size_t)1 << P.log_n;
  CK(pr->want(pr->zs_values, (size_t)pr->Bcap * P.oracle_w[2] * n * sizeof(u64)));
  CK(pr->want(pr->chunk_q, (size_t)pr->Bcap * P.zs_count * (num_routed / degree) * n * sizeof(u64)));
  CK(pr->bg.alloc((size_t)pr->Bcap * 8 * sizeof(u64)));
  CK(pr->alphas.alloc((size_t)pr->Bcap * 2 * sizeof(u64)));
  pr->num_routed = num_routed; pr->degree = degree;
  pr->drop_graph();
  return 0;
}
int mp2g_prover_enable_quotient(mp2g_prover* pr) {
  NEED(pr && pr->num_routed, "call mp2g_prover_enable_permutation first");
  const mp2g_fri_params& P = pr->P;
  NEED(P.n_oracles == 4 && P.rate_bits == 3, "needs the four plonky2 oracles and rate_bits 3 (quotient degree factor 8)");
  NEED(P.oracle_w[3] == P.zs_count * 8, "oracle_w[3] must be zs_count * 8 quotient chunks");
  NEED(P.log_n + 3 <= 24, "log_n <= 21");
  CK(pr->want(pr->qvals, (size_t)pr->Bcap * P.zs_count * ((size_t)8 << P.log_n) * sizeof(u64)));
  pr->quotient = true;
  pr->drop_graph();
  return 0;
}
int mp2g_prover_set_gates(mp2g_prover* pr, const mp2g_gate* gates, uint32_t n_gates, uint32_t num_selectors) {
  NEED(pr && pr->quotient, "call mp2g_prover_enable_quotient first");
  NEED(n_gates <= MP2G_MAX_GATES, "at most MP2G_MAX_GATES gates");
  GateTable t{};
  t.n_gates = n_gates; t.num_selectors = num_selectors;
  t.num_lookup_selectors = pr->gates.num_lookup_selectors;
  if (n_gates) {
    NEED(gates, "gates");
    for (uint32_t i = 0; i < n_gates; i++) t.g[i] = gates[i];
    const char* msg = gate_table_check(t, pr->P.oracle_w[0] - pr->num_routed, pr->P.oracle_w[1]);
    if (msg) return fail("invalid gate table: %s", msg);
    for (uint32_t i = 0; i < n_gates; i++) {
      uint32_t fdeg = t.g[i].group_end - t.g[i].group_start - 1 + (num_selectors > 1 ? 1 : 0);
      if (fdeg + gate_degree(t.g[i]) > 9) return fail("invalid gate table: filtered degree of gate %u exceeds quotient degree factor + 1 = 9", i);
    }
  }
  pr->gates = t;
  pr->drop_graph();
  return 0;
}
}

static int fri_tail(mp2g_prover* pr, const FriShape& sh, ChState* st, u64* d_proof) {
  mp2g_ctx* c = pr->ctx;
  hipStream_t s = c->stream;
  const mp2g_fri_params& P = pr->P;
  const uint32_t B = pr->B, lg = P.log_n + P.rate_bits, V = P.variant;
  const u64 n = (u64)1 << P.log_n, N = n << P.rate_bits;
  const size_t capw = pr->capw;
  u64* chal = pr->chal.p;
  CK(challenger_step(s, V, st, B, chal, 0, 0, pr->alpha.p, 2, 2));
  CK(fri_final_poly(s, sh, B, pr->alpha.p, 2, pr->zeta.p, 2, pr->comp.p, pr->quot.p, pr->final_poly.p));
  CosetTables* pre;
  CK(c->ntt.coset(P.log_n, P.rate_bits, GL_MULT_GEN, &pre));
  CK(c->ntt.run(pr->final_poly.p, pr->fvals[0].p, P.log_n, 2 * B, P.rate_bits, n, N, false, pre, true));

  FriLayers ly{};
  ly.n_layers = P.n_layers;
  u64 m = N, nc = n, shift = GL_MULT_GEN;
  uint32_t clg = lg;
  u64* proof = (u64*)d_proof;
  const u64* cur_coeffs = pr->final_poly.p;
  for (uint32_t li = 0; li < P.n_layers; li++) {
    const uint32_t ab = P.arity_bits[li];
    const uint32_t log_leaves = clg - ab;
    const size_t lw = merkle_levels_words(log_leaves, P.cap_height);
    CK(leaf_hash_ext_soa(s, V, pr->fvals[li].p, pr->fvals[li].p + m, ab, (u64)1 << log_leaves, pr->flevels[li].p, B, 2 * m, lw));
    CK(merkle_reduce(s, V, pr->flevels[li].p, log_leaves, P.cap_height, B, lw));
    CK(copy_rows(s, B, pr->flevels[li].p + lw - capw, lw, proof + li * capw, pr->proof_words, (u32)capw));
    u64* beta = pr->betas.p + 2 * li;
    CK(challenger_step(s, V, st, B, proof + li * capw, pr->proof_words, (u32)capw, beta, 16, 2));
    ly.arity_bits[li] = ab;
    ly.values[li] = pr->fvals[li].p; ly.value_bstride[li] = 2 * m;
    ly.levels[li] = pr->flevels[li].p; ly.level_bstride[li] = lw;
    CK(fri_fold_values(s, B, clg, ab, pr->fvals[li].p, 2 * m, pr->fvals[li + 1].p, 2 * (m >> ab), beta, 16, shift));
    const bool last = li + 1 == P.n_layers;
    if (last) CK(fri_fold_coeffs(s, B, (u32)nc, ab, cur_coeffs, 2 * nc, proof + pr->final_off, pr->proof_words, beta, 16, true));
    else CK(fri_fold_coeffs(s, B, (u32)nc, ab, cur_coeffs, 2 * nc, pr->fcoeffs[li + 1].p, 2 * (nc >> ab), beta, 16, false));
    cur_coeffs = pr->fcoeffs[li + 1].p;
    shift = gl_pow(shift, (u64)1 << ab);
    m >>= ab; nc >>= ab; clg -= ab;
  }
  if (P.n_layers == 0) CK(fri_soa_to_aos(s, B, (u32)n, pr->final_poly.p, 2 * n, (u32)n, proof + pr->final_off, pr->proof_words));
  CK(challenger_step(s, V, st, B, proof + pr->final_off, pr->proof_words, (u32)(2 * pr->final_len), chal, 8, 0));
  STAGE_MARK(pr, 5);
  CK(fri_pow(s, V, st, B, P.pow_bits, pr->witness.p));
  STAGE_MARK(pr, 6);
  CK(copy_rows(s, B, pr->witness.p, FRI_POW_STRIDE, proof + pr->final_off + 2 * pr->final_len, pr->proof_words, 1));
  CK(challenger_step(s, V, st, B, pr->witness.p, FRI_POW_STRIDE, 1, chal, 8, 1));
  if (P.num_queries) {
    CK(challenger_step(s, V, st, B, chal, 0, 0, pr->qchal.p, P.num_queries, P.num_queries));
    CK(fri_queries(s, sh, ly, B, P.num_queries, pr->qchal.p, P.num_queries, proof, pr->proof_words, pr->q_off, pr->q_words));
  }
  return 0;
}

extern "C" {

static int prove_impl(mp2g_prover* pr, const uint64_t* const* d_values, const uint64_t* d_circuit_digest,
                      const uint64_t* d_pi_hash, uint64_t* d_caps, uint64_t* d_openings, uint64_t* d_proof);
static int bind_scratch(mp2g_prover* pr) {
  if (pr->shared.empty()) return 0;
  mp2g_ctx* c = pr->ctx;
  if (!pr->counted) { pr->counted = true; c->scratch_users++; }
  size_t total = 0;
  for (auto& e : pr->shared) total += (e.second + 255) & ~(size_t)255;
  if (c->prover_scratch.bytes < total) {
    CK(hipStreamSynchronize(c->stream));
    hipError_t e = c->prover_scratch.alloc(total);
    if (e != hipSuccess) return fail("prover scratch of %zu bytes: %s", total, hipGetErrorString(e));
  }
  if (pr->bound_base == c->prover_scratch.p && pr->bound_total == total) return 0;
  size_t off = 0;
  for (auto& e : pr->shared) {
    e.first->borrow(c->prover_scratch.p + off / sizeof(u64), e.second);
    off += (e.second + 255) & ~(size_t)255;
  }
  pr->bound_base = c->prover_scratch.p;
  pr->bound_total = total;
  pr->drop_graph();
  return 0;
}
int mp2g_prover_prove_dev(mp2g_prover* pr, const uint64_t* const* d_values, const uint64_t* d_circuit_digest,
                          const uint64_t* d_pi_hash, uint64_t* d_caps, uint64_t* d_openings, uint64_t* d_proof) {
  NEED(pr && d_values && d_circuit_digest && d_pi_hash && d_caps && d_openings && d_proof, "prover/pointers");
  NEED(pr->have_pre, "call mp2g_prover_set_preprocessed_dev first");
  { int rcb = bind_scratch(pr); if (rcb) return rcb; }
  if (!pr->graph_on || pr->timing || pr->plain_calls == 0) {
    pr->plain_calls++;
    return prove_impl(pr, d_values, d_circuit_digest, d_pi_hash, d_caps, d_openings, d_proof);
  }
  const void* key[12] = {d_circuit_digest, d_pi_hash, d_caps, d_openings, d_proof};
  for (uint32_t o = 1; o < pr->P.n_oracles && o < 8; o++) key[4 + o] = d_values[o - 1];
  hipStream_t s = pr->ctx->stream;
  if (pr->gexec && memcmp(key, pr->gkey, sizeof key) == 0 && pr->ggen == pr->ctx->ntt.generation) {
    CK(hipGraphLaunch(pr->gexec, s));
    return 0;
  }
  pr->drop_graph();
  hipGraph_t g = nullptr;
  if (pr->quotient)
    CK(pr->ctx->ntt.ensure_scratch((size_t)pr->B * pr->P.zs_count * ((size_t)8 << pr->P.log_n)));
  for (uint32_t o = 1; o < pr->P.n_oracles; o++) CK(pr->ctx->ntt.ensure_scratch((size_t)pr->B * pr->P.oracle_w[o] << pr->P.log_n));
  const u64 gen0 = pr->ctx->ntt.generation;
  CK(hipStreamBeginCapture(s, hipStreamCaptureModeThreadLocal));
  int rc = prove_impl(pr, d_values, d_circuit_digest, d_pi_hash, d_caps, d_openings, d_proof);
  hipError_t e = hipStreamEndCapture(s, &g);
  if (!rc && e == hipSuccess && pr->ctx->ntt.generation != gen0) {
    if (g) (void)hipGraphDestroy(g);
    return fail("graph capture: an NTT buffer was reallocated inside the capture");
  }
  if (rc || e != hipSuccess) {
    if (g) (void)hipGraphDestroy(g);
    return rc ? rc : fail("graph capture: %s", hipGetErrorString(e));
  }
  e = hipGraphInstantiate(&pr->gexec, g, nullptr, nullptr, 0);
  (void)hipGraphDestroy(g);
  if (e != hipSuccess) { pr->gexec = nullptr; return fail("hipGraphInstantiate: %s", hipGetErrorString(e)); }
  memcpy(pr->gkey, key, sizeof key);
  pr->ggen = gen0;
  CK(hipGraphLaunch(pr->gexec, s));
  return 0;
}
int mp2g_prover_enable_graph(mp2g_prover* pr, int on) {
  NEED(pr, "prover");
  pr->graph_on = on != 0;
  if (!on) pr->drop_graph();
  return 0;
}
static int prove_impl(mp2g_prover* pr, const uint64_t* const* d_values, const uint64_t* d_circuit_digest,
                      const uint64_t* d_pi_hash, uint64_t* d_caps, uint64_t* d_openings, uint64_t* d_proof) {
  mp2g_ctx* c = pr->ctx;
  hipStream_t s = c->stream;
  const mp2g_fri_params& P = pr->P;
  const uint32_t B = pr->B, V = P.variant;
  const u64 n = (u64)1 << P.log_n, N = n << P.rate_bits;
  const size_t capw = pr->capw, LW = pr->levels_words;
  ChState* st = (ChState*)pr->ch.p;
  u64* chal = pr->chal.p;
  const u64 caps_b = P.n_oracles * capw;

  STAGE_MARK(pr, 0);
  if (pr->pi_row >= 0)
    CK(bind_public_inputs(s, B, (u64*)d_values[0], (u64)P.oracle_w[1] * n, n, (u32)pr->pi_row, (const u64*)d_pi_hash));
  if (pr->wcheck) {
    CK(hipMemsetAsync(pr->wflags.p, 0, B * sizeof(u32), s));
    if (pr->gates.n_gates)
      CK(gate_check(s, B, pr->gates, pr->pre_values.p, (const u64*)d_values[0], (u64)P.oracle_w[1] * n, n, (const u64*)d_pi_hash,
                    (u32*)pr->wflags.p));
  }
  CK(challenger_init(s, st, B));
  CK(challenger_step(s, V, st, B, (const u64*)d_circuit_digest, 0, 4, chal, 8, 0));
  CK(challenger_step(s, V, st, B, (const u64*)d_pi_hash, 4, 4, chal, 8, 0));
  CK(copy_rows(s, B, pr->levels[0].p + LW - capw, 0, (u64*)d_caps, caps_b, (u32)capw));
  for (uint32_t o = 1; o < P.n_oracles; o++) {
    const u64* vals = (const u64*)d_values[o - 1];
    if (o == 2 && pr->num_routed) {
      CK(zpp_compute(s, B, (const u64*)d_values[0], (u64)P.oracle_w[1] * n, pr->pre_values.p + (u64)(P.oracle_w[0] - pr->num_routed) * n,
                     P.log_n, pr->num_routed, pr->degree, pr->bg.p, pr->bg.p + P.zs_count, 8, P.zs_count, pr->chunk_q.p, pr->zs_values.p,
                     (u64)P.oracle_w[2] * n));
      if (pr->lookups.n_luts) {
        CK(lookup_table_polys(s, B, pr->lookups, pr->bg.p, 8, P.zs_count, pr->lut_eval.p));
        CK(lookup_polys(s, B, pr->lookups, (const u64*)d_values[0], (u64)P.oracle_w[1] * n, P.log_n, pr->bg.p, 8, P.zs_count,
                        pr->zs_values.p + (u64)P.zs_count * (pr->num_routed / pr->degree) * n, (u64)P.oracle_w[2] * n, pr->lut_eval.p,
                        pr->wcheck ? (u32*)pr->wflags.p : nullptr));
      }
      vals = pr->zs_values.p;
      if (pr->wcheck)
        CK(zpp_wrap_check(s, B, pr->chunk_q.p, pr->zs_values.p, (u64)P.oracle_w[2] * n, P.log_n, pr->num_routed / pr->degree, P.zs_count,
                          (u32*)pr->wflags.p));
    }
    if (o == 3 && pr->quotient) {
      const u32 nc = P.zs_count;
      if (pr->gates.n_gates)
        CK(gate_constraints_lde(s, B, pr->gates, pr->values[0].p, pr->values[1].p, (u64)P.oracle_w[1] * N, P.log_n + 3, pr->alphas.p, 2,
                                nc, (const u64*)d_pi_hash, pr->qvals.p));
      if (pr->lookups.n_luts)
        CK(quotient_lookup_values(s, B, pr->lookups, pr->values[0].p, pr->gates.num_selectors, pr->values[1].p, (u64)P.oracle_w[1] * N,
                                  pr->values[2].p, (u64)P.oracle_w[2] * N, nc * (pr->num_routed / pr->degree), P.log_n, pr->bg.p, 8,
                                  pr->lut_eval.p, pr->alphas.p, 2, nc, pr->qvals.p));
      CK(quotient_perm_values(s, B, pr->values[1].p, (u64)P.oracle_w[1] * N, pr->values[0].p + (u64)(P.oracle_w[0] - pr->num_routed) * N,
                              pr->values[2].p, (u64)P.oracle_w[2] * N, P.log_n, pr->num_routed, pr->degree, pr->bg.p, 8,
                              pr->alphas.p, 2, nc, pr->gates.n_gates != 0, pr->qvals.p));
      CK(c->ntt.run(pr->qvals.p, pr->coeffs[3].p, P.log_n + 3, B * nc, 0, N, N, true, nullptr, false));
      CK(c->ntt.scale_powers(pr->coeffs[3].p, P.log_n + 3, B * nc, gl_inv(GL_MULT_GEN), 1));
      CK(commit_oracle_coeffs(pr, 3, B));
    } else {
      NEED(vals, "d_values[o]");
      CK(commit_oracle(pr, o, vals, B));
    }
    u64* cap_dst = (u64*)d_caps + o * capw;
    CK(copy_rows(s, B, pr->levels[o].p + LW - capw, LW, cap_dst, caps_b, (u32)capw));
    const uint32_t nch = P.zs_count >= 1 && P.zs_count <= 2 ? P.zs_count : 2;
    uint32_t n_get = o == 1 ? (pr->lookups.n_luts ? 4 : 2) * nch : (o == 2 ? nch : 0);
    u64* dst = chal;
    u64 dst_stride = 8;
    if (pr->num_routed && o == 1) { dst = pr->bg.p; dst_stride = 8; }
    if (pr->num_routed && o == 2) { dst = pr->alphas.p; dst_stride = 2; }
    CK(challenger_step(s, V, st, B, cap_dst, caps_b, (u32)capw, dst, dst_stride, n_get));
    if (o <= 3) STAGE_MARK(pr, o);
  }
  if (P.n_oracles < 4) for (uint32_t o = P.n_oracles; o <= 3; o++) STAGE_MARK(pr, o);
  CK(challenger_step(s, V, st, B, chal, 0, 0, pr->zeta.p, 2, 2));

  FriShape sh{};
  sh.log_n = P.log_n; sh.rate_bits = P.rate_bits; sh.cap_h = P.cap_height; sh.n_oracles = P.n_oracles;
  sh.zs_oracle = P.zs_oracle; sh.zs_count = P.zs_count; sh.lookup_count = P.zs_count * P.num_lookup_polys;
  for (uint32_t o = 0; o < P.n_oracles; o++) {
    OracleRef& r = sh.o[o];
    r.coeffs = pr->coeffs[o].p; r.values = pr->values[o].p; r.levels = pr->levels[o].p; r.w = P.oracle_w[o];
    r.coeff_bstride = o ? (u64)r.w * n : 0;
    r.value_bstride = o ? (u64)r.w * N : 0;
    r.level_bstride = o ? LW : 0;
    sh.n_polys += r.w;
  }
  CK(fri_openings(s, sh, B, pr->zeta.p, 2, (u64*)d_openings));
  CK(challenger_step(s, V, st, B, (const u64*)d_openings, 2 * pr->n_open, (u32)(2 * pr->n_open), chal, 8, 0));
  STAGE_MARK(pr, 4);
  int rc = fri_tail(pr, sh, st, (u64*)d_proof);
  if (rc) return rc;
  STAGE_MARK(pr, 7);
  return 0;
}
int mp2g_prover_set_lookups(mp2g_prover* pr, const mp2g_lookup* luts, uint32_t n_luts) {
  NEED(pr && pr->quotient, "call mp2g_prover_enable_quotient first");
  NEED(n_luts <= MP2G_MAX_LUTS, "at most MP2G_MAX_LUTS lookup tables");
  const mp2g_fri_params& P = pr->P;
  LookupDev L{};
  if (!n_luts) {
    NEED(P.num_lookup_polys == 0, "params.num_lookup_polys != 0 needs lookup tables");
    pr->lookups = L;
    pr->gates.num_lookup_selectors = 0;
    pr->drop_graph();
    return 0;
  }
  NEED(luts && pr->gates.n_gates, "luts; call mp2g_prover_set_gates first");
  L.n_luts = n_luts;
  L.num_lu_slots = pr->num_routed / 2; L.num_lut_slots = pr->num_routed / 3;
  L.lu_degree = pr->degree - 1;
  NEED(L.lu_degree >= 1 && L.num_lu_slots <= 40 && L.num_lut_slots >= 1, "slot geometry (num_routed <= 80, degree >= 2)");
  L.num_sldc = (L.num_lu_slots + L.lu_degree - 1) / L.lu_degree;
  L.lut_degree = (L.num_lut_slots + L.num_sldc - 1) / L.num_sldc;
  NEED(P.num_lookup_polys == L.num_sldc + 1, "params.num_lookup_polys must be ceil((num_routed/2) / (degree-1)) + 1");
  NEED(P.oracle_w[1] >= 3 * L.num_lut_slots && P.oracle_w[1] >= 2 * L.num_lu_slots, "wires");
  const uint32_t n_sel = 4 + n_luts, num_constants = P.oracle_w[0] - pr->num_routed;
  NEED(pr->gates.num_selectors + n_sel <= num_constants, "the constants must hold 4 + n_luts lookup selectors after the selectors");
  const uint64_t n = (uint64_t)1 << P.log_n;
  size_t total = 0;
  for (uint32_t r = 0; r < n_luts; r++) {
    const mp2g_lookup& u = luts[r];
    NEED(u.table && u.table_len >= 1 && u.table_len <= 65536, "table");
    NEED(u.last_lu_row < u.last_lut_row && u.last_lut_row <= u.first_lut_row && (uint64_t)u.first_lut_row + 1 < n, "lookup rows");
    NEED((uint64_t)(u.first_lut_row - u.last_lut_row + 1) * L.num_lut_slots >= u.table_len, "the table does not fit its LookupTableGate rows");
    total += (size_t)u.table_len * 2;
  }
  pr->drop_graph();
  pr->lookups = LookupDev{};
  pr->gates.num_lookup_selectors = 0;
  CK(pr->lut_tables.alloc(total * sizeof(uint16_t)));
  CK(pr->lut_eval.alloc((size_t)pr->Bcap * P.zs_count * MP2G_MAX_LUTS * sizeof(u64)));
  size_t off = 0;
  for (uint32_t r = 0; r < n_luts; r++) {
    const mp2g_lookup& u = luts[r];
    L.last_lu_row[r] = u.last_lu_row; L.last_lut_row[r] = u.last_lut_row; L.first_lut_row[r] = u.first_lut_row; L.table_len[r] = u.table_len;
    L.table[r] = (const uint16_t*)pr->lut_tables.p + off;
    CK(hipMemcpyAsync((uint16_t*)pr->lut_tables.p + off, u.table, (size_t)u.table_len * 2 * sizeof(uint16_t), hipMemcpyHostToDevice, pr->ctx->stream));
    off += (size_t)u.table_len * 2;
  }
  CK(hipStreamSynchronize(pr->ctx->stream));
  pr->lookups = L;
  pr->gates.num_lookup_selectors = n_sel;
  const char* msg = gate_table_check(pr->gates, num_constants, P.oracle_w[1]);
  if (msg) { pr->lookups = LookupDev{}; pr->gates.num_lookup_selectors = 0; return fail("invalid gate table with lookups: %s", msg); }
  pr->drop_graph();
  return 0;
}
int mp2g_prover_bind_public_inputs(mp2g_prover* pr, int64_t row) {
  NEED(pr, "prover");
  NEED(row < (int64_t)1 << pr->P.log_n, "row < 2^log_n");
  NEED(pr->P.n_oracles >= 2 && pr->P.oracle_w[1] >= 4, "needs a wires oracle of at least 4 columns");
  pr->pi_row = row < 0 ? -1 : row;
  pr->drop_graph();
  return 0;
}
int mp2g_prover_set_active(mp2g_prover* pr, uint32_t n) {
  NEED(pr && n >= 1 && n <= pr->Bcap, "1 <= n <= the batch the prover was created for");
  if (n != pr->B) pr->drop_graph();
  pr->B = n;
  return 0;
}
int mp2g_prover_enable_witness_check(mp2g_prover* pr, int on) {
  NEED(pr && pr->num_routed, "call mp2g_prover_enable_permutation first");
  if (on && !pr->wflags.p) CK(pr->wflags.alloc((size_t)pr->Bcap * sizeof(u32)));
  pr->wcheck = on != 0;
  pr->drop_graph();
  return 0;
}
int mp2g_prover_witness_check_enabled(const mp2g_prover* pr) { return pr && pr->wcheck ? 1 : 0; }
int mp2g_prover_witness_status(mp2g_prover* pr, uint32_t* flags) {
  NEED(pr && pr->wcheck, "call mp2g_prover_enable_witness_check first");
  std::vector<uint32_t> h(pr->B);
  CK(hipMemcpyAsync(h.data(), pr->wflags.p, pr->B * sizeof(u32), hipMemcpyDeviceToHost, pr->ctx->stream));
  CK(hipStreamSynchronize(pr->ctx->stream));
  if (flags) memcpy(flags, h.data(), pr->B * sizeof(u32));
  for (uint32_t b = 0; b < pr->B; b++)
    if (h[b])
      return fail("invalid witness: proof %u of the batch violates%s%s%s", b, (h[b] & 1) ? " a copy constraint" : "",
                  (h[b] & 2) ? " a gate constraint" : "", (h[b] & 4) ? " the lookup argument" : "");
  return 0;
}
}
namespace mp2g { int prover_flags_to_host_async(mp2g_prover* pr, uint32_t* h_dst); }
int mp2g::prover_flags_to_host_async(mp2g_prover* pr, uint32_t* h_dst) {
  NEED(pr && pr->wcheck && h_dst, "prover with the witness check on / destination");
  CK(hipMemcpyAsync(h_dst, pr->wflags.p, pr->B * sizeof(u32), hipMemcpyDeviceToHost, pr->ctx->stream));
  return 0;
}
extern "C" {
int mp2g_prover_enable_timing(mp2g_prover* pr, int on) {
  NEED(pr, "prover");
  if (on)
    for (hipEvent_t& e : pr->ev)
      if (!e) CK(hipEventCreate(&e));
  pr->timing = on != 0;
  return 0;
}
int mp2g_prover_stage_ms(mp2g_prover* pr, float out[MP2G_N_STAGES]) {
  NEED(pr && out, "prover/out");
  NEED(pr->timing, "call mp2g_prover_enable_timing first");
  CK(hipStreamSynchronize(pr->ctx->stream));
  for (int i = 0; i < MP2G_N_STAGES; i++) CK(hipEventElapsedTime(&out[i], pr->ev[i], pr->ev[i + 1]));
  return 0;
}

int mp2g_partial_products_and_zs(mp2g_ctx* c, const uint64_t* wires, uint32_t wires_w, const uint64_t* sigmas, uint32_t log_n,
                                 uint32_t num_routed, uint32_t degree, const uint64_t* betas, const uint64_t* gammas, uint32_t nc,
                                 uint64_t* out) {
  NEED(c && wires && sigmas && betas && gammas && out, "ctx/pointers");
  NEED(log_n >= 1 && log_n <= 20 && nc >= 1 && nc <= 4, "log_n/nc");
  NEED(degree >= 1 && num_routed >= degree && num_routed % degree == 0 && num_routed / degree <= 16 && num_routed <= wires_w, "num_routed/degree");
  const size_t n = (size_t)1 << log_n, chunks = num_routed / degree;
  DevBuf dw, ds, dc, dq, dout;
  CK(dw.alloc(wires_w * n * sizeof(u64)));
  CK(ds.alloc(num_routed * n * sizeof(u64)));
  CK(dc.alloc(2 * nc * sizeof(u64)));
  CK(dq.alloc(nc * chunks * n * sizeof(u64)));
  CK(dout.alloc(nc * chunks * n * sizeof(u64)));
  CK(hipMemcpyAsync(dw.p, wires, wires_w * n * sizeof(u64), hipMemcpyHostToDevice, c->stream));
  CK(hipMemcpyAsync(ds.p, sigmas, num_routed * n * sizeof(u64), hipMemcpyHostToDevice, c->stream));
  CK(hipMemcpyAsync(dc.p, betas, nc * sizeof(u64), hipMemcpyHostToDevice, c->stream));
  CK(hipMemcpyAsync(dc.p + nc, gammas, nc * sizeof(u64), hipMemcpyHostToDevice, c->stream));
  CK(zpp_compute(c->stream, 1, dw.p, 0, ds.p, log_n, num_routed, degree, dc.p, dc.p + nc, 0, nc, dq.p, dout.p, 0));
  CK(hipMemcpyAsync(out, dout.p, nc * chunks * n * sizeof(u64), hipMemcpyDeviceToHost, c->stream));
  CK(hipStreamSynchronize(c->stream));
  return 0;
}

uint32_t mp2g_gate_num_constraints(const mp2g_gate* g) { return g ? gate_num_constraints(*g) : 0; }
uint32_t mp2g_gate_degree(const mp2g_gate* g) { return g ? gate_degree(*g) : 0; }
int mp2g_eval_gate_constraints(mp2g_ctx* c, const mp2g_gate* gates, uint32_t n_gates, uint32_t num_selectors, const uint64_t* consts,
                               uint32_t num_constants, const uint64_t* wires, uint32_t wires_w, uint64_t npts,
                               const uint64_t pi_hash[4], uint64_t* out) {
  NEED(c && gates && consts && wires && pi_hash && out, "ctx/pointers");
  NEED(n_gates >= 1 && n_gates <= MP2G_MAX_GATES, "1..MP2G_MAX_GATES gates");
  NEED(npts >= 1 && npts <= ((uint64_t)1 << 28), "npts");
  GateTable t{};
  t.n_gates = n_gates; t.num_selectors = num_selectors;
  uint32_t max_j = 0;
  for (uint32_t i = 0; i < n_gates; i++) {
    t.g[i] = gates[i];
    uint32_t k = gate_num_constraints(gates[i]);
    if (k > max_j) max_j = k;
  }
  const char* msg = gate_table_check(t, num_constants, wires_w);
  if (msg) return fail("invalid gate table: %s", msg);
  if (!max_j) return 0;
  DevBuf dc, dw, dp, dout;
  CK(dc.alloc((size_t)num_constants * npts * sizeof(u64)));
  CK(dw.alloc((size_t)wires_w * npts * sizeof(u64)));
  CK(dp.alloc(4 * sizeof(u64)));
  CK(dout.alloc((size_t)max_j * npts * sizeof(u64)));
  CK(hipMemcpyAsync(dc.p, consts, (size_t)num_constants * npts * sizeof(u64), hipMemcpyHostToDevice, c->stream));
  CK(hipMemcpyAsync(dw.p, wires, (size_t)wires_w * npts * sizeof(u64), hipMemcpyHostToDevice, c->stream));
  CK(hipMemcpyAsync(dp.p, pi_hash, 4 * sizeof(u64), hipMemcpyHostToDevice, c->stream));
  CK(gate_constraints_points(c->stream, t, dc.p, dw.p, npts, max_j, dp.p, dout.p));
  CK(hipMemcpyAsync(out, dout.p, (size_t)max_j * npts * sizeof(u64), hipMemcpyDeviceToHost, c->stream));
  CK(hipStreamSynchronize(c->stream));
  return 0;
}

int mp2g_batch_eval_ext(const mp2g_batch* b, const uint64_t point[2], uint64_t* out) {
  NEED(b && point && out, "batch/point/out");
  NEED(point[0] < GL_P && point[1] < GL_P, "point canonical");
  mp2g_ctx* c = b->ctx;
  FriShape sh{};
  sh.log_n = b->log_n; sh.rate_bits = b->rate_bits; sh.cap_h = b->cap_h; sh.n_oracles = 1; sh.n_polys = b->w;
  sh.o[0].coeffs = b->coeffs.p; sh.o[0].w = b->w;
  DevBuf dz, dout;
  CK(dz.alloc(2 * sizeof(u64)));
  CK(dout.alloc((size_t)b->w * 2 * sizeof(u64)));
  CK(hipMemcpyAsync(dz.p, point, 2 * sizeof(u64), hipMemcpyHostToDevice, c->stream));
  CK(fri_openings(c->stream, sh, 1, dz.p, 0, dout.p));
  CK(hipMemcpyAsync(out, dout.p, (size_t)b->w * 2 * sizeof(u64), hipMemcpyDeviceToHost, c->stream));
  CK(hipStreamSynchronize(c->stream));
  return 0;
}

int mp2g_fri_prove(mp2g_ctx* c, const mp2g_fri_params* params, mp2g_batch* const* oracles, const uint64_t zeta[2],
                   mp2g_challenger* ch, uint64_t* proof) {
  NEED(c && params && oracles && zeta && ch && proof, "ctx/pointers");
  NEED(ch->ctx == c && ch->count == 1, "challenger must live on this context with count 1");
  NEED(ch->variant == (int)params->variant, "challenger / params hash variant differ");
  mp2g_prover* pr;
  int rc = prover_create_impl(c, params, 1, false, &pr);
  if (rc) return rc;
  ProverGuard guard;
  guard.pr = pr;
  const mp2g_fri_params& P = pr->P;
  FriShape sh{};
  sh.log_n = P.log_n; sh.rate_bits = P.rate_bits; sh.cap_h = P.cap_height; sh.n_oracles = P.n_oracles;
  sh.zs_oracle = P.zs_oracle; sh.zs_count = P.zs_count; sh.lookup_count = P.zs_count * P.num_lookup_polys;
  for (uint32_t o = 0; o < P.n_oracles; o++) {
    const mp2g_batch* b = oracles[o];
    if (!b || b->ctx != c || b->log_n != P.log_n || b->w != P.oracle_w[o] || b->rate_bits != P.rate_bits ||
        b->cap_h != P.cap_height || b->variant != (int)P.variant) {
      return fail("oracle %u does not match the FRI parameters", o);
    }
    OracleRef& r = sh.o[o];
    r.coeffs = b->coeffs.p; r.values = b->values.p; r.levels = b->levels.p; r.w = b->w;
    sh.n_polys += r.w;
  }
  DevBuf dproof;
  hipError_t e = dproof.alloc(pr->proof_words * sizeof(u64));
  if (e == hipSuccess) e = hipMemcpyAsync(pr->zeta.p, zeta, 2 * sizeof(u64), hipMemcpyHostToDevice, c->stream);
  if (e != hipSuccess) return fail("fri_prove setup: %s", hipGetErrorString(e));
  rc = bind_scratch(pr);
  if (!rc) rc = fri_tail(pr, sh, (ChState*)ch->st.p, dproof.p);
  if (!rc) {
    e = hipMemcpyAsync(proof, dproof.p, pr->proof_words * sizeof(u64), hipMemcpyDeviceToHost, c->stream);
    if (e == hipSuccess) e = hipStreamSynchronize(c->stream);
    if (e != hipSuccess) rc = fail("fri_prove copy-out: %s", hipGetErrorString(e));
  }
  return rc;
}

int mp2g_pcs_prove(mp2g_ctx* c, const mp2g_fri_params* params, const uint64_t* const* values, const uint64_t circuit_digest[4],
                   const uint64_t pi_hash[4], uint64_t* caps, uint64_t* openings, uint64_t* proof) {
  NEED(c && values && circuit_digest && pi_hash && caps && openings && proof, "ctx/pointers");
  mp2g_prover* pr;
  int rc = mp2g_prover_create(c, params, 1, &pr);
  if (rc) return rc;
  ProverGuard guard;
  guard.pr = pr;
  const mp2g_fri_params& P = pr->P;
  const size_t n = (size_t)1 << P.log_n;
  DevBuf dv[8], dd, dp, dcaps, dopen, dproof;
  const uint64_t* dptr[8] = {};
  hipError_t e = hipSuccess;
  for (uint32_t o = 0; o < P.n_oracles && e == hipSuccess; o++) {
    e = dv[o].alloc(P.oracle_w[o] * n * sizeof(u64));
    if (e == hipSuccess) e = hipMemcpyAsync(dv[o].p, values[o], P.oracle_w[o] * n * sizeof(u64), hipMemcpyHostToDevice, c->stream);
    if (o) dptr[o - 1] = dv[o].p;
  }
  if (e == hipSuccess) e = dd.alloc(32);
  if (e == hipSuccess) e = dp.alloc(32);
  if (e == hipSuccess) e = dcaps.alloc(P.n_oracles * pr->capw * sizeof(u64));
  if (e == hipSuccess) e = dopen.alloc(pr->n_open * 2 * sizeof(u64));
  if (e == hipSuccess) e = dproof.alloc(pr->proof_words * sizeof(u64));
  if (e == hipSuccess) e = hipMemcpyAsync(dd.p, circuit_digest, 32, hipMemcpyHostToDevice, c->stream);
  if (e == hipSuccess) e = hipMemcpyAsync(dp.p, pi_hash, 32, hipMemcpyHostToDevice, c->stream);
  if (e != hipSuccess) return fail("pcs_prove setup: %s", hipGetErrorString(e));
  rc = mp2g_prover_set_preprocessed_dev(pr, dv[0].p);
  if (!rc) rc = mp2g_prover_prove_dev(pr, dptr, dd.p, dp.p, dcaps.p, dopen.p, dproof.p);
  if (!rc) {
    e = hipMemcpyAsync(caps, dcaps.p, P.n_oracles * pr->capw * sizeof(u64), hipMemcpyDeviceToHost, c->stream);
    if (e == hipSuccess) e = hipMemcpyAsync(openings, dopen.p, pr->n_open * 2 * sizeof(u64), hipMemcpyDeviceToHost, c->stream);
    if (e == hipSuccess) e = hipMemcpyAsync(proof, dproof.p, pr->proof_words * sizeof(u64), hipMemcpyDeviceToHost, c->stream);
    if (e == hipSuccess) e = hipStreamSynchronize(c->stream);
    if (e != hipSuccess) rc = fail("pcs_prove copy-out: %s", hipGetErrorString(e));
  }
  return rc;
}

}
```

### mapreduce-plonky2_amd/csrc/zperm.h

```cpp
#pragma once
#include "gl.cuh"
namespace mp2g {
hipError_t zpp_compute(hipStream_t s, u32 B, const u64* wires, u64 wires_bstride, const u64* sigmas, u32 log_n, u32 num_routed,
                       u32 degree, const u64* betas, const u64* gammas, u64 chal_bstride, u32 nc, u64* chunk_q, u64* out,
                       u64 out_bstride);
hipError_t quotient_perm_values(hipStream_t s, u32 B, const u64* W, u64 w_bstride, const u64* S, const u64* Z, u64 z_bstride,
                                u32 log_n, u32 num_routed, u32 degree, const u64* bg, u64 bg_bstride, const u64* alphas,
                                u64 al_bstride, u32 nc, bool gates, u64* q);
hipError_t zpp_wrap_check(hipStream_t s, u32 B, const u64* chunk_q, const u64* zs, u64 zs_bstride, u32 log_n, u32 chunks, u32 nc,
                          u32* flags);
}
```

### mapreduce-plonky2_amd/csrc/zperm.hip

```cpp
#include "zperm.h"

namespace mp2g {

#define ZP_MAX_CHUNKS 16
#define ZP_MAX_ROUTED 256
__device__ __forceinline__ void fill_k_is(u64* kis, u32 num_routed) {
  for (u32 j = threadIdx.x; j < num_routed; j += blockDim.x) kis[j] = gl_pow(GL_MULT_GEN, j);
  __syncthreads();
}

__global__ void __launch_bounds__(256) zpp_chunk_kernel(const u64* __restrict__ wires, u64 wires_bstride, const u64* __restrict__ sigmas,
                                                        u32 log_n, u32 num_routed, u32 degree, const u64* __restrict__ betas,
                                                        const u64* __restrict__ gammas, u64 chal_bstride, u32 nc, u64* __restrict__ chunk_q) {
  const u32 n = 1u << log_n, i = blockIdx.x * 256 + threadIdx.x, c = blockIdx.y, b = blockIdx.z;
  __shared__ u64 kis[ZP_MAX_ROUTED];
  fill_k_is(kis, num_routed);
  if (i >= n) return;
  const u32 chunks = num_routed / degree;
  const u64 beta = betas[b * chal_bstride + c], gamma = gammas[b * chal_bstride + c];
  const u64 bx = gl_mul(beta, gl_pow(gl_root_of_unity(log_n), i));
  const u64* w = wires + b * wires_bstride + i;
  const u64* sg = sigmas + i;
  u64 num[ZP_MAX_CHUNKS], den[ZP_MAX_CHUNKS];
  u32 j = 0;
  for (u32 k = 0; k < chunks; k++) {
    u64 pn = 1, pd = 1;
    for (u32 t = 0; t < degree; t++, j++) {
      u64 wv = w[(u64)j << log_n];
      const u64 wg = gl_addw(wv, gamma);
      pn = gl_mulw(pn, gl_mul_addw(bx, kis[j], wg));
      pd = gl_mulw(pd, gl_mul_addw(beta, sg[(u64)j << log_n], wg));
    }
    num[k] = pn; den[k] = gl_canon(pd);
  }
  u64 pre[ZP_MAX_CHUNKS];
  u64 acc = 1;
  for (u32 k = 0; k < chunks; k++) { pre[k] = acc; acc = gl_mul(acc, den[k] ? den[k] : 1); }
  u64 inv = gl_inv(acc);
  u64* out = chunk_q + ((u64)(b * nc + c) * chunks << log_n) + i;
  for (int k = (int)chunks - 1; k >= 0; k--) {
    u64 dinv = den[k] ? gl_mul(inv, pre[k]) : 0;
    inv = gl_mul(inv, den[k] ? den[k] : 1);
    out[(u64)k << log_n] = gl_mul(num[k], dinv);
  }
}
__global__ void __launch_bounds__(1024) zpp_scan_kernel(const u64* __restrict__ chunk_q, u32 log_n, u32 chunks, u32 nc, u64* __restrict__ out,
                                                        u64 out_bstride) {
  const u32 n = 1u << log_n, c = blockIdx.x, b = blockIdx.y, t = threadIdx.x;
  const u32 T = n < 1024 ? n : 1024, S = n / T;
  const u32 num_prods = chunks - 1;
  const u64* q = chunk_q + ((u64)(b * nc + c) * chunks << log_n);
  __shared__ u64 sc[1024];
  u64 local = 1;
  if (t < T)
    for (u32 r = 0; r < S; r++)
      for (u32 k = 0; k < chunks; k++) local = gl_mul(local, q[((u64)k << log_n) + t * S + r]);
  sc[t] = local;
  __syncthreads();
  for (u32 d = 1; d < T; d <<= 1) {
    u64 v = (t >= d && t < T) ? sc[t - d] : 1;
    __syncthreads();
    if (t < T) sc[t] = gl_mul(sc[t], v);
    __syncthreads();
  }
  if (t >= T) return;
  u64 z = t ? sc[t - 1] : 1;
  u64* zrow = out + b * out_bstride + ((u64)c << log_n);
  u64* pp = out + b * out_bstride + ((u64)nc << log_n) + ((u64)c * num_prods << log_n);
  for (u32 r = 0; r < S; r++) {
    u32 i = t * S + r;
    zrow[i] = z;
    u64 acc = z;
    for (u32 k = 0; k < chunks; k++) {
      acc = gl_mul(acc, q[((u64)k << log_n) + i]);
      if (k < num_prods) pp[((u64)k << log_n) + i] = acc;
    }
    z = acc;
  }
}

__global__ void __launch_bounds__(256) quotient_perm_kernel(const u64* __restrict__ W, u64 w_bstride, const u64* __restrict__ S,
                                                            const u64* __restrict__ Z, u64 z_bstride, u32 log_n, u32 num_routed,
                                                            u32 degree, const u64* __restrict__ bg, u64 bg_bstride,
                                                            const u64* __restrict__ alphas, u64 al_bstride, u32 nc, bool gates,
                                                            u64* __restrict__ q) {
  const u32 lg = log_n + 3;
  const u64 N = (u64)1 << lg;
  const u32 p = blockIdx.x * 256 + threadIdx.x, b = blockIdx.y;
  const u32 i = bitrev32(p, lg);
  __shared__ u64 zh_inv[8];
  __shared__ u64 kis[ZP_MAX_ROUTED];
  fill_k_is(kis, num_routed);
  if (threadIdx.x < 8) {
    u64 gn = gl_pow(GL_MULT_GEN, (u64)1 << log_n);
    zh_inv[threadIdx.x] = gl_inv(gl_sub(gl_mul(gn, gl_pow(gl_root_of_unity(3), threadIdx.x)), 1));
  }
  __syncthreads();
  if (p >= N) return;
  const u32 chunks = num_routed / degree, num_prods = chunks - 1;
  const u64 pn = bitrev32((i + 8) & (u32)(N - 1), lg);
  const u64 x = gl_mul(GL_MULT_GEN, gl_pow(gl_root_of_unity(lg), i));
  const u64* w = W + b * w_bstride + p;
  const u64* sg = S + p;
  const u64* z = Z + b * z_bstride;
  u64 acc[2] = {0, 0}, apow[2] = {1, 1}, al[2];
  for (u32 a = 0; a < nc; a++) al[a] = alphas[b * al_bstride + a];
  auto push = [&](u64 term) {
    for (u32 a = 0; a < nc; a++) {
      acc[a] = gl_mul_add(term, apow[a], acc[a]);
      apow[a] = gl_mul(apow[a], al[a]);
    }
  };
  const u64 zh = gl_inv(zh_inv[i & 7]);
  const u64 l0 = gl_mul(zh, gl_inv(gl_mul(((u64)1 << log_n) % GL_P, gl_sub(x, 1))));
  for (u32 c = 0; c < nc; c++) push(gl_mul(l0, gl_sub(z[((u64)c << lg) + p], 1)));
  for (u32 c = 0; c < nc; c++) {
    const u64 beta = bg[b * bg_bstride + c], gamma = bg[b * bg_bstride + nc + c];
    const u64 bx = gl_mul(beta, x);
    const u64* pp = z + ((u64)(nc + c * num_prods) << lg);
    u32 j = 0;
    u64 prev = z[((u64)c << lg) + p];
    for (u32 k = 0; k < chunks; k++) {
      u64 num = 1, den = 1;
      for (u32 t = 0; t < degree; t++, j++) {
        u64 wv = w[(u64)j << lg];
        const u64 wg = gl_addw(wv, gamma);
        num = gl_mulw(num, gl_mul_addw(bx, kis[j], wg));
        den = gl_mulw(den, gl_mul_addw(beta, sg[(u64)j << lg], wg));
      }
      u64 next = k == chunks - 1 ? z[((u64)c << lg) + pn] : pp[((u64)k << lg) + p];
      push(gl_sub(gl_mul(prev, num), gl_mul(next, den)));
      prev = next;
    }
  }
  if (gates)
    for (u32 a = 0; a < nc; a++) acc[a] = gl_add(acc[a], gl_mul(apow[a], q[(((u64)b * nc + a) << lg) + i]));
  for (u32 a = 0; a < nc; a++) q[(((u64)b * nc + a) << lg) + i] = gl_mul(acc[a], zh_inv[i & 7]);
}
hipError_t quotient_perm_values(hipStream_t s, u32 B, const u64* W, u64 w_bstride, const u64* S, const u64* Z, u64 z_bstride,
                                u32 log_n, u32 num_routed, u32 degree, const u64* bg, u64 bg_bstride, const u64* alphas,
                                u64 al_bstride, u32 nc, bool gates, u64* q) {
  if (nc < 1 || nc > 2 || !degree || num_routed % degree || num_routed > ZP_MAX_ROUTED) return hipErrorInvalidValue;
  const u64 N = (u64)8 << log_n;
  hipLaunchKernelGGL(quotient_perm_kernel, dim3((u32)((N + 255) / 256), B), dim3(256), 0, s, W, w_bstride, S, Z, z_bstride, log_n,
                     num_routed, degree, bg, bg_bstride, alphas, al_bstride, nc, gates, q);
  return hipGetLastError();
}

__global__ void zpp_wrap_check_kernel(const u64* __restrict__ chunk_q, const u64* __restrict__ zs, u64 zs_bstride, u32 log_n, u32 chunks,
                                      u32 nc, u32 B, u32* __restrict__ flags) {
  const u32 t = blockIdx.x * blockDim.x + threadIdx.x;
  if (t >= B * nc) return;
  const u32 b = t / nc, c = t % nc, last = (1u << log_n) - 1;
  u64 acc = zs[b * zs_bstride + ((u64)c << log_n) + last];
  const u64* q = chunk_q + ((u64)(b * nc + c) * chunks << log_n);
  for (u32 k = 0; k < chunks; k++) acc = gl_mul(acc, q[((u64)k << log_n) + last]);
  if (acc != 1) atomicOr(&flags[b], 1u);
}
hipError_t zpp_wrap_check(hipStream_t s, u32 B, const u64* chunk_q, const u64* zs, u64 zs_bstride, u32 log_n, u32 chunks, u32 nc,
                          u32* flags) {
  hipLaunchKernelGGL(zpp_wrap_check_kernel, dim3((B * nc + 63) / 64), dim3(64), 0, s, chunk_q, zs, zs_bstride, log_n, chunks, nc, B, flags);
  return hipGetLastError();
}

hipError_t zpp_compute(hipStream_t s, u32 B, const u64* wires, u64 wires_bstride, const u64* sigmas, u32 log_n, u32 num_routed,
                       u32 degree, const u64* betas, const u64* gammas, u64 chal_bstride, u32 nc, u64* chunk_q, u64* out,
                       u64 out_bstride) {
  if (!degree || num_routed % degree || num_routed / degree > ZP_MAX_CHUNKS || num_routed / degree < 1 || num_routed > ZP_MAX_ROUTED)
    return hipErrorInvalidValue;
  const u32 n = 1u << log_n, chunks = num_routed / degree;
  hipLaunchKernelGGL(zpp_chunk_kernel, dim3((n + 255) / 256, nc, B), dim3(256), 0, s, wires, wires_bstride, sigmas, log_n, num_routed,
                     degree, betas, gammas, chal_bstride, nc, chunk_q);
  hipLaunchKernelGGL(zpp_scan_kernel, dim3(nc, B), dim3(1024), 0, s, chunk_q, log_n, chunks, nc, out, out_bstride);
  return hipGetLastError();
}
}
```

Baseline: 901.3.

## Precompute power tables and replace Horner chains with table-driven lazy accumulations

Adds device kernels that materialise powers of zeta and alpha, plus host-built tables for domain points, L0 values, zh inverses and k_i. Openings, compose, combine, gate-constraint and quotient-permutation kernels now read these tables instead of running per-thread pow/inv and serial Horner chains. Openings also handle four polynomials per block so each zeta-power load is reused across them. The cost is extra memory traffic for the tables, a few extra launches, and host-side table construction that must be uploaded.

Result: faster. 921.3, median of 6 (+2.2%).

```diff
diff --git a/mapreduce-plonky2_amd/csrc/fri.h b/mapreduce-plonky2_amd/csrc/fri.h
--- a/mapreduce-plonky2_amd/csrc/fri.h
+++ b/mapreduce-plonky2_amd/csrc/fri.h
@@ -45,9 +45,10 @@
 hipError_t challenger_init(hipStream_t s, ChState* st, u32 B);
 hipError_t challenger_step(hipStream_t s, int variant, ChState* st, u32 B, const u64* obs, u64 obs_bstride, u32 n_obs,
                            u64* out, u64 out_bstride, u32 n_get);
-hipError_t fri_openings(hipStream_t s, const FriShape& sh, u32 B, const u64* zeta, u64 zeta_bstride, u64* out);
+hipError_t fri_openings(hipStream_t s, const FriShape& sh, u32 B, const u64* zeta, u64 zeta_bstride, u64* zpw, u64* out);
+GLHD u32 fri_alpha_powers_len(const FriShape& sh) { return sh.n_polys + 1; }
 hipError_t fri_final_poly(hipStream_t s, const FriShape& sh, u32 B, const u64* alpha, u64 alpha_bstride, const u64* zeta,
-                          u64 zeta_bstride, u64* comp, u64* quot, u64* final_poly);
+                          u64 zeta_bstride, u64* apw, u64* comp, u64* quot, u64* final_poly);
 hipError_t fri_fold_values(hipStream_t s, u32 B, u32 log_m, u32 ab, const u64* in, u64 in_bstride, u64* out, u64 out_bstride,
                            const u64* beta, u64 beta_bstride, u64 shift);
 hipError_t fri_fold_coeffs(hipStream_t s, u32 B, u32 n_in, u32 ab, const u64* in, u64 in_bstride, u64* out, u64 out_bstride,
diff --git a/mapreduce-plonky2_amd/csrc/fri.hip b/mapreduce-plonky2_amd/csrc/fri.hip
--- a/mapreduce-plonky2_amd/csrc/fri.hip
+++ b/mapreduce-plonky2_amd/csrc/fri.hip
@@ -92,63 +92,99 @@
   return hipGetLastError();
 }
 
-__global__ void __launch_bounds__(256) openings_kernel(FriShape sh, const u64* zeta , u64 zeta_bstride, u64* out ) {
-  const u32 j = blockIdx.x, b = blockIdx.y, t = threadIdx.x;
-  const u32 n = 1u << sh.log_n;
-  u32 o, p;
-  gl2 x = gl2_make(zeta[b * zeta_bstride], zeta[b * zeta_bstride + 1]);
-  if (j >= sh.n_polys) {
-    fri_batch_poly(sh, 1, j - sh.n_polys, o, p);
-    x = gl2_scale(x, gl_root_of_unity(sh.log_n));
-  } else {
-    fri_batch_poly(sh, 0, j, o, p);
-  }
-  const u64* c = sh.o[o].coeffs + b * sh.o[o].coeff_bstride + ((u64)p << sh.log_n);
-  gl2 x256 = gl2_pow(x, 256), acc = gl2_make(0, 0);
-  if (t < n) {
-    u32 top = ((n - 1 - t) >> 8);
-    for (int k = (int)top; k >= 0; k--) {
-      acc = gl2_mul(acc, x256);
-      acc.a = gl_add(acc.a, c[t + ((u32)k << 8)]);
-    }
-    acc = gl2_mul(acc, gl2_pow(x, t));
-  }
-  __shared__ u64 ra[256], rb[256];
-  ra[t] = acc.a; rb[t] = acc.b;
+#define EP_RUN 16
+__global__ void __launch_bounds__(256) ext_powers_kernel(const u64* __restrict__ x, u64 x_bstride, u64 scale, u32 count,
+                                                         u64* __restrict__ out, u64 out_bstride) {
+  const u32 b = blockIdx.y, e0 = blockIdx.x * 256 * EP_RUN + threadIdx.x;
+  if (e0 >= count) return;
+  const gl2 xb = gl2_scale(gl2_make(x[b * x_bstride], x[b * x_bstride + 1]), scale);
+  const gl2 step = gl2_pow(xb, 256);
+  gl2 pw = gl2_pow(xb, e0);
+  u64* o = out + b * out_bstride;
+  for (u32 r = 0, e = e0; r < EP_RUN && e < count; r++, e += 256) {
+    o[e] = pw.a;
+    o[count + e] = pw.b;
+    pw = gl2_mul(pw, step);
+  }
+}
+static hipError_t ext_powers(hipStream_t s, u32 B, const u64* x, u64 x_bstride, u64 scale, u32 count, u64* out, u64 out_bstride) {
+  hipLaunchKernelGGL(ext_powers_kernel, dim3((count + 256 * EP_RUN - 1) / (256 * EP_RUN), B), dim3(256), 0, s, x, x_bstride, scale, count, out,
+                     out_bstride);
+  return hipGetLastError();
+}
+
+#define OP_POLYS 4
+__global__ void __launch_bounds__(256) openings_kernel(FriShape sh, const u64* __restrict__ zpw, u64 zpw_bstride, u64* out ) {
+  const u32 b = blockIdx.y, t = threadIdx.x;
+  const u32 n = 1u << sh.log_n, n_open = sh.n_polys + sh.zs_count + sh.lookup_count;
+  const u32 blocks0 = (sh.n_polys + OP_POLYS - 1) / OP_POLYS;
+  const bool shifted = blockIdx.x >= blocks0;
+  const u32 j0 = shifted ? sh.n_polys + (blockIdx.x - blocks0) * OP_POLYS : blockIdx.x * OP_POLYS;
+  const u32 nq = min(OP_POLYS, (shifted ? n_open : sh.n_polys) - j0);
+  const u64* pa = zpw + b * zpw_bstride + (shifted ? 2 * (u64)n : 0);
+  const u64* pb = pa + n;
+  const u64* c[OP_POLYS];
+#pragma unroll
+  for (u32 q = 0; q < OP_POLYS; q++) {
+    u32 o, p;
+    const u32 j = j0 + (q < nq ? q : 0);
+    if (shifted) fri_batch_poly(sh, 1, j - sh.n_polys, o, p);
+    else fri_batch_poly(sh, 0, j, o, p);
+    c[q] = sh.o[o].coeffs + b * sh.o[o].coeff_bstride + ((u64)p << sh.log_n);
+  }
+  gl_cols sa[OP_POLYS], sb[OP_POLYS];
+  for (u32 i = t; i < n; i += 256) {
+    const u64 za = pa[i], zb = pb[i];
+#pragma unroll
+    for (u32 q = 0; q < OP_POLYS; q++)
+      if (q < nq) {
+        const u64 v = c[q][i];
+        sa[q].add(v, za);
+        sb[q].add(v, zb);
+      }
+  }
+  __shared__ u64 ra[OP_POLYS][256], rb[OP_POLYS][256];
+#pragma unroll
+  for (u32 q = 0; q < OP_POLYS; q++) { ra[q][t] = sa[q].value(); rb[q][t] = sb[q].value(); }
   __syncthreads();
-  for (int s = 128; s > 0; s >>= 1) {
-    if ((int)t < s) { ra[t] = gl_add(ra[t], ra[t + s]); rb[t] = gl_add(rb[t], rb[t + s]); }
+  for (u32 s = 128; s > 0; s >>= 1) {
+    if (t < s)
+#pragma unroll
+      for (u32 q = 0; q < OP_POLYS; q++) { ra[q][t] = gl_add(ra[q][t], ra[q][t + s]); rb[q][t] = gl_add(rb[q][t], rb[q][t + s]); }
     __syncthreads();
   }
-  if (t == 0) {
-    u64* d = out + ((u64)b * (sh.n_polys + sh.zs_count + sh.lookup_count) + j) * 2;
-    d[0] = ra[0]; d[1] = rb[0];
-  }
-}
-
-__global__ void __launch_bounds__(256) compose_kernel(FriShape sh, const u64* alpha, u64 alpha_bstride, u64* comp) {
+  if (t < nq) {
+    u64* d = out + ((u64)b * n_open + j0 + t) * 2;
+    d[0] = ra[t][0]; d[1] = rb[t][0];
+  }
+}
+
+__global__ void __launch_bounds__(256) compose_kernel(FriShape sh, const u64* __restrict__ apw, u64 apw_bstride, u32 apw_len, u64* comp) {
   const u32 n = 1u << sh.log_n;
   const u32 i = blockIdx.x * 256 + threadIdx.x, b = blockIdx.y, batch = blockIdx.z;
   if (i >= n) return;
-  gl2 al = gl2_make(alpha[b * alpha_bstride], alpha[b * alpha_bstride + 1]);
-  gl2 acc = gl2_make(0, 0);
+  const u64* pa = apw + b * apw_bstride;
+  const u64* pb = pa + apw_len;
+  gl_cols sa, sb;
+  u32 m = 0;
   const u32 zo = sh.zs_oracle, wz = sh.o[zo].w - sh.lookup_count;
   auto run = [&](u32 o, u32 first, u32 count) {
     const u64* base = sh.o[o].coeffs + b * sh.o[o].coeff_bstride + i;
-    for (int p = (int)(first + count) - 1; p >= (int)first; p--) {
-      acc = gl2_mul(acc, al);
-      acc.a = gl_add(acc.a, base[(u64)p << sh.log_n]);
+    for (u32 p = first; p < first + count; p++, m++) {
+      const u64 v = base[(u64)p << sh.log_n];
+      sa.add(v, pa[m]);
+      sb.add(v, pb[m]);
     }
   };
-  if (sh.lookup_count) run(zo, wz, sh.lookup_count);
   if (batch == 0) {
-    for (int o = (int)sh.n_oracles - 1; o >= 0; o--) run((u32)o, 0, (u32)o == zo ? wz : sh.o[o].w);
+    for (u32 o = 0; o < sh.n_oracles; o++) run(o, 0, o == zo ? wz : sh.o[o].w);
   } else {
     run(zo, 0, sh.zs_count);
   }
+  if (sh.lookup_count) run(zo, wz, sh.lookup_count);
   u64* d = comp + (((u64)b * 2 + batch) * 2) * n;
-  d[i] = acc.a;
-  d[n + i] = acc.b;
+  d[i] = sa.value();
+  d[n + i] = sb.value();
 }
 
 __global__ void __launch_bounds__(1024) divide_kernel(u32 log_n, const u64* zeta, u64 zeta_bstride, const u64* comp, u64* quot) {
@@ -194,10 +230,11 @@
     if (t == T - 1) { q0[n - 1] = 0; q1[n - 1] = 0; }
   }
 }
-__global__ void __launch_bounds__(256) combine_kernel(u32 log_n, u32 zs_count, const u64* alpha, u64 alpha_bstride, const u64* quot, u64* final_poly) {
+__global__ void __launch_bounds__(256) combine_kernel(u32 log_n, u32 zs_count, const u64* __restrict__ apw, u64 apw_bstride, u32 apw_len,
+                                                      const u64* quot, u64* final_poly) {
   const u32 n = 1u << log_n, i = blockIdx.x * 256 + threadIdx.x, b = blockIdx.y;
   if (i >= n) return;
-  gl2 sh = gl2_pow(gl2_make(alpha[b * alpha_bstride], alpha[b * alpha_bstride + 1]), zs_count);
+  const gl2 sh = gl2_make(apw[b * apw_bstride + zs_count], apw[b * apw_bstride + apw_len + zs_count]);
   const u64* q = quot + (u64)b * 4 * n;
   gl2 r = gl2_add(gl2_mul(gl2_make(q[i], q[n + i]), sh), gl2_make(q[2 * n + i], q[3 * n + i]));
   final_poly[(u64)b * 2 * n + i] = r.a;
@@ -357,17 +394,22 @@
 
 #define HIPCHK(x) do { hipError_t e_ = (x); if (e_ != hipSuccess) return e_; } while (0)
 
-hipError_t fri_openings(hipStream_t s, const FriShape& sh, u32 B, const u64* zeta, u64 zeta_bstride, u64* out) {
-  hipLaunchKernelGGL(openings_kernel, dim3(sh.n_polys + sh.zs_count + sh.lookup_count, B), dim3(256), 0, s, sh, zeta, zeta_bstride, out);
+hipError_t fri_openings(hipStream_t s, const FriShape& sh, u32 B, const u64* zeta, u64 zeta_bstride, u64* zpw, u64* out) {
+  const u32 n = 1u << sh.log_n, n_shifted = sh.zs_count + sh.lookup_count;
+  HIPCHK(ext_powers(s, B, zeta, zeta_bstride, 1, n, zpw, 4 * (u64)n));
+  if (n_shifted) HIPCHK(ext_powers(s, B, zeta, zeta_bstride, gl_root_of_unity(sh.log_n), n, zpw + 2 * (u64)n, 4 * (u64)n));
+  const u32 blocks = (sh.n_polys + OP_POLYS - 1) / OP_POLYS + (n_shifted + OP_POLYS - 1) / OP_POLYS;
+  hipLaunchKernelGGL(openings_kernel, dim3(blocks, B), dim3(256), 0, s, sh, zpw, 4 * (u64)n, out);
   return hipGetLastError();
 }
 hipError_t fri_final_poly(hipStream_t s, const FriShape& sh, u32 B, const u64* alpha, u64 alpha_bstride, const u64* zeta, u64 zeta_bstride,
-                          u64* comp, u64* quot, u64* final_poly) {
-  const u32 n = 1u << sh.log_n;
-  hipLaunchKernelGGL(compose_kernel, dim3((n + 255) / 256, B, 2), dim3(256), 0, s, sh, alpha, alpha_bstride, comp);
+                          u64* apw, u64* comp, u64* quot, u64* final_poly) {
+  const u32 n = 1u << sh.log_n, apw_len = fri_alpha_powers_len(sh);
+  HIPCHK(ext_powers(s, B, alpha, alpha_bstride, 1, apw_len, apw, 2 * (u64)apw_len));
+  hipLaunchKernelGGL(compose_kernel, dim3((n + 255) / 256, B, 2), dim3(256), 0, s, sh, apw, 2 * (u64)apw_len, apw_len, comp);
   hipLaunchKernelGGL(divide_kernel, dim3(2, B), dim3(1024), 0, s, sh.log_n, zeta, zeta_bstride, comp, quot);
-  hipLaunchKernelGGL(combine_kernel, dim3((n + 255) / 256, B), dim3(256), 0, s, sh.log_n, sh.zs_count + sh.lookup_count, alpha, alpha_bstride, quot,
-                     final_poly);
+  hipLaunchKernelGGL(combine_kernel, dim3((n + 255) / 256, B), dim3(256), 0, s, sh.log_n, sh.zs_count + sh.lookup_count, apw, 2 * (u64)apw_len,
+                     apw_len, quot, final_poly);
   return hipGetLastError();
 }
 hipError_t fri_fold_values(hipStream_t s, u32 B, u32 log_m, u32 ab, const u64* in, u64 in_bstride, u64* out, u64 out_bstride,
diff --git a/mapreduce-plonky2_amd/csrc/gates.h b/mapreduce-plonky2_amd/csrc/gates.h
--- a/mapreduce-plonky2_amd/csrc/gates.h
+++ b/mapreduce-plonky2_amd/csrc/gates.h
@@ -11,7 +11,8 @@
 u32 gate_num_constraints(const mp2g_gate& g);
 u32 gate_degree(const mp2g_gate& g);
 hipError_t gate_constraints_lde(hipStream_t s, u32 B, const GateTable& t, const u64* C, const u64* W, u64 w_bstride, u32 lg,
-                                const u64* alphas, u64 al_bstride, u32 nc, const u64* pi_hash, u64* q);
+                                const u64* apw, u32 nc, const u64* pi_hash, u64* q);
+hipError_t alpha_powers(hipStream_t s, u32 B, const u64* alphas, u64 al_bstride, u32 nc, u64* apw);
 hipError_t gate_constraints_points(hipStream_t s, const GateTable& t, const u64* consts, const u64* wires, u64 npts, u32 max_j,
                                    const u64* pi_hash, u64* out);
 hipError_t gate_check(hipStream_t s, u32 B, const GateTable& t, const u64* consts, const u64* wires, u64 w_bstride, u64 npts,
diff --git a/mapreduce-plonky2_amd/csrc/gates.hip b/mapreduce-plonky2_amd/csrc/gates.hip
--- a/mapreduce-plonky2_amd/csrc/gates.hip
+++ b/mapreduce-plonky2_amd/csrc/gates.hip
@@ -599,15 +599,15 @@
 template <u32 KIND>
 __global__ void __launch_bounds__(256) gate_constraints_lde_kernel(mp2g_gate g, u32 gi, u32 num_selectors, u32 cst_off, u32 n_cons,
                                                                    const u64* __restrict__ C, const u64* __restrict__ W,
-                                                                   u64 w_bstride, u32 lg, const u64* __restrict__ alphas,
-                                                                   u64 al_bstride, u32 nc, const u64* __restrict__ pi_hash,
+                                                                   u64 w_bstride, u32 lg, const u64* __restrict__ apw_tab,
+                                                                   u32 nc, const u64* __restrict__ pi_hash,
                                                                    u64* __restrict__ q, int first) {
   __shared__ u64 apw[2][MP2G_MAX_GATE_CONSTRAINTS];
   const u64 N = (u64)1 << lg;
   const u32 p = blockIdx.x * 256 + threadIdx.x, b = blockIdx.y;
   for (u32 j = threadIdx.x; j < 2 * n_cons; j += 256) {
     const u32 a = j >= n_cons ? 1 : 0, e = j - a * n_cons;
-    apw[a][e] = a < nc ? gl_pow(alphas[b * al_bstride + a], e) : 0;
+    apw[a][e] = apw_tab[((u64)b * 2 + a) * MP2G_MAX_GATE_CONSTRAINTS + e];
   }
   __syncthreads();
   if (p >= N) return;
@@ -654,15 +654,15 @@
 }
 __global__ void __launch_bounds__(256) gate_constraints_lde_light_kernel(LightGates lg_, u32 num_selectors, u32 cst_off, u32 max_cons,
                                                                          const u64* __restrict__ C, const u64* __restrict__ W,
-                                                                         u64 w_bstride, u32 lg, const u64* __restrict__ alphas,
-                                                                         u64 al_bstride, u32 nc, const u64* __restrict__ pi_hash,
+                                                                         u64 w_bstride, u32 lg, const u64* __restrict__ apw_tab,
+                                                                         u32 nc, const u64* __restrict__ pi_hash,
                                                                          u64* __restrict__ q, int first) {
   __shared__ u64 apw[2][MP2G_MAX_GATE_CONSTRAINTS];
   const u64 N = (u64)1 << lg;
   const u32 p = blockIdx.x * 256 + threadIdx.x, b = blockIdx.y;
   for (u32 j = threadIdx.x; j < 2 * max_cons; j += 256) {
     const u32 a = j >= max_cons ? 1 : 0, e = j - a * max_cons;
-    apw[a][e] = a < nc ? gl_pow(alphas[b * al_bstride + a], e) : 0;
+    apw[a][e] = apw_tab[((u64)b * 2 + a) * MP2G_MAX_GATE_CONSTRAINTS + e];
   }
   __syncthreads();
   if (p >= N) return;
@@ -757,8 +757,21 @@
   return hipGetLastError();
 }
 
+__global__ void alpha_powers_kernel(const u64* __restrict__ alphas, u64 al_bstride, u32 nc, u32 B, u64* __restrict__ apw) {
+  const u32 t = blockIdx.x * blockDim.x + threadIdx.x;
+  if (t >= B * 2 * MP2G_MAX_GATE_CONSTRAINTS) return;
+  const u32 e = t % MP2G_MAX_GATE_CONSTRAINTS, a = (t / MP2G_MAX_GATE_CONSTRAINTS) & 1, b = t / (2 * MP2G_MAX_GATE_CONSTRAINTS);
+  apw[t] = a < nc ? gl_pow(alphas[b * al_bstride + a], e) : 0;
+}
+hipError_t alpha_powers(hipStream_t s, u32 B, const u64* alphas, u64 al_bstride, u32 nc, u64* apw) {
+  if (nc < 1 || nc > 2) return hipErrorInvalidValue;
+  const u32 total = B * 2 * MP2G_MAX_GATE_CONSTRAINTS;
+  hipLaunchKernelGGL(alpha_powers_kernel, dim3((total + 255) / 256), dim3(256), 0, s, alphas, al_bstride, nc, B, apw);
+  return hipGetLastError();
+}
+
 hipError_t gate_constraints_lde(hipStream_t s, u32 B, const GateTable& t, const u64* C, const u64* W, u64 w_bstride, u32 lg,
-                                const u64* alphas, u64 al_bstride, u32 nc, const u64* pi_hash, u64* q) {
+                                const u64* apw, u32 nc, const u64* pi_hash, u64* q) {
   if (nc < 1 || nc > 2) return hipErrorInvalidValue;
   const u64 N = (u64)1 << lg;
   const dim3 grid((u32)((N + 255) / 256), B), block(256);
@@ -775,7 +788,7 @@
   if (lgs.n < 2) lgs.n = 0;
   if (lgs.n) {
     hipLaunchKernelGGL(gate_constraints_lde_light_kernel, grid, block, 0, s, lgs, t.num_selectors, t.num_selectors + t.num_lookup_selectors,
-                       light_cons, C, W, w_bstride, lg, alphas, al_bstride, nc, pi_hash, q, first);
+                       light_cons, C, W, w_bstride, lg, apw, nc, pi_hash, q, first);
     first = 0;
   }
   for (u32 gi = 0; gi < t.n_gates; gi++) {
@@ -788,7 +801,7 @@
 #define GATE_CASE(K)                                                                                                        \
   case K:                                                                                                                   \
     hipLaunchKernelGGL(gate_constraints_lde_kernel<K>, grid, block, 0, s, g, gi, t.num_selectors,                          \
-                       t.num_selectors + t.num_lookup_selectors, n_cons, C, W, w_bstride, lg, alphas, al_bstride, nc, pi_hash, q, \
+                       t.num_selectors + t.num_lookup_selectors, n_cons, C, W, w_bstride, lg, apw, nc, pi_hash, q,             \
                        first);                                                                                              \
     break;
     switch (g.kind) {
diff --git a/mapreduce-plonky2_amd/csrc/ntt.h b/mapreduce-plonky2_amd/csrc/ntt.h
--- a/mapreduce-plonky2_amd/csrc/ntt.h
+++ b/mapreduce-plonky2_amd/csrc/ntt.h
@@ -34,6 +34,7 @@
   hipError_t run(const u64* in, u64* out, u32 log_n, u32 polys, u32 logK, u64 in_poly_stride,
                  u64 out_poly_stride, bool inverse, const CosetTables* pre, bool bitrev_out);
   hipError_t scale_powers(u64* data, u32 log_n, u32 batch, u64 base, u64 first);
+  hipError_t scale_table(u64* data, u32 log_n, u32 batch, const u64* table);
 };
 
 }
diff --git a/mapreduce-plonky2_amd/csrc/ntt.hip b/mapreduce-plonky2_amd/csrc/ntt.hip
--- a/mapreduce-plonky2_amd/csrc/ntt.hip
+++ b/mapreduce-plonky2_amd/csrc/ntt.hip
@@ -568,6 +568,11 @@
   u64 k = i & (((u64)1 << log_n) - 1);
   data[i] = gl_mul(data[i], gl_mul(first, gl_pow(base, k)));
 }
+__global__ void scale_table_kernel(u64* __restrict__ data, u32 log_n, u32 batch, const u64* __restrict__ table) {
+  u64 i = (u64)blockIdx.x * blockDim.x + threadIdx.x;
+  if (i >= ((u64)batch << log_n)) return;
+  data[i] = gl_mul(data[i], table[i & (((u64)1 << log_n) - 1)]);
+}
 
 #define HIPCHK(x) do { hipError_t e_ = (x); if (e_ != hipSuccess) return e_; } while (0)
 
@@ -819,6 +824,11 @@
   hipLaunchKernelGGL(scale_powers_kernel, dim3((u32)((total + 255) / 256)), dim3(256), 0, stream, data, log_n, batch, base, first);
   return hipGetLastError();
 }
+hipError_t NttEngine::scale_table(u64* data, u32 log_n, u32 batch, const u64* table) {
+  u64 total = (u64)batch << log_n;
+  hipLaunchKernelGGL(scale_table_kernel, dim3((u32)((total + 255) / 256)), dim3(256), 0, stream, data, log_n, batch, table);
+  return hipGetLastError();
+}
 
 NttEngine::~NttEngine() { if (scratch) (void)hipFree(scratch); }
 
diff --git a/mapreduce-plonky2_amd/csrc/prover.hip b/mapreduce-plonky2_amd/csrc/prover.hip
--- a/mapreduce-plonky2_amd/csrc/prover.hip
+++ b/mapreduce-plonky2_amd/csrc/prover.hip
@@ -29,9 +29,12 @@
   DevBuf coeffs[8], values[8], levels[8];
   DevBuf ch, chal, zeta, alpha, betas, comp, quot, final_poly, witness, qchal;
   DevBuf fvals[9], flevels[8], fcoeffs[9];
+  DevBuf zpw, fapw;
   uint32_t num_routed = 0, degree = 0;
   bool quotient = false;
   DevBuf pre_values, zs_values, chunk_q, bg, alphas, qvals;
+  DevBuf ptab, qtab;
+  DevBuf apw;
   GateTable gates{};
   LookupDev lookups{};
   DevBuf lut_tables, lut_eval;
@@ -74,6 +77,15 @@
   mp2g_prover* pr = nullptr;
   ~ProverGuard();
 };
+template <class F>
+hipError_t upload_table(mp2g_ctx* c, DevBuf& d, size_t words, F fill) {
+  std::vector<u64> h(words);
+  fill(h.data());
+  hipError_t e = d.alloc(words * sizeof(u64));
+  if (e == hipSuccess) e = hipMemcpyAsync(d.p, h.data(), words * sizeof(u64), hipMemcpyHostToDevice, c->stream);
+  if (e == hipSuccess) e = hipStreamSynchronize(c->stream);
+  return e;
+}
 }
 
 namespace mp2g {
@@ -251,6 +263,7 @@
   if (e == hipSuccess) e = pr->ch.alloc(B * sizeof(ChState));
   A(pr->chal, B * 8); A(pr->zeta, B * 2); A(pr->alpha, B * 2); A(pr->betas, B * 16);
   S(pr->comp, B * 4 * n); S(pr->quot, B * 4 * n); S(pr->final_poly, B * 2 * n);
+  S(pr->zpw, B * 4 * n); A(pr->fapw, B * 2 * (pr->n_open + 1));
   A(pr->witness, B * FRI_POW_STRIDE); A(pr->qchal, B * (P.num_queries ? P.num_queries : 1));
   size_t m = N, nc = n;
   uint32_t clg = lg;
@@ -325,6 +338,7 @@
   CK(pr->want(pr->chunk_q, (size_t)pr->Bcap * P.zs_count * (num_routed / degree) * n * sizeof(u64)));
   CK(pr->bg.alloc((size_t)pr->Bcap * 8 * sizeof(u64)));
   CK(pr->alphas.alloc((size_t)pr->Bcap * 2 * sizeof(u64)));
+  CK(upload_table(pr->ctx, pr->ptab, perm_table_words(P.log_n, num_routed), [&](u64* h) { perm_tables_host(P.log_n, num_routed, h); }));
   pr->num_routed = num_routed; pr->degree = degree;
   pr->drop_graph();
   return 0;
@@ -336,6 +350,8 @@
   NEED(P.oracle_w[3] == P.zs_count * 8, "oracle_w[3] must be zs_count * 8 quotient chunks");
   NEED(P.log_n + 3 <= 24, "log_n <= 21");
   CK(pr->want(pr->qvals, (size_t)pr->Bcap * P.zs_count * ((size_t)8 << P.log_n) * sizeof(u64)));
+  CK(pr->apw.alloc((size_t)pr->Bcap * 2 * MP2G_MAX_GATE_CONSTRAINTS * sizeof(u64)));
+  CK(upload_table(pr->ctx, pr->qtab, quotient_table_words(P.log_n), [&](u64* h) { quotient_tables_host(P.log_n, h); }));
   pr->quotient = true;
   pr->drop_graph();
   return 0;
@@ -371,7 +387,7 @@
   const size_t capw = pr->capw;
   u64* chal = pr->chal.p;
   CK(challenger_step(s, V, st, B, chal, 0, 0, pr->alpha.p, 2, 2));
-  CK(fri_final_poly(s, sh, B, pr->alpha.p, 2, pr->zeta.p, 2, pr->comp.p, pr->quot.p, pr->final_poly.p));
+  CK(fri_final_poly(s, sh, B, pr->alpha.p, 2, pr->zeta.p, 2, pr->fapw.p, pr->comp.p, pr->quot.p, pr->final_poly.p));
   CosetTables* pre;
   CK(c->ntt.coset(P.log_n, P.rate_bits, GL_MULT_GEN, &pre));
   CK(c->ntt.run(pr->final_poly.p, pr->fvals[0].p, P.log_n, 2 * B, P.rate_bits, n, N, false, pre, true));
@@ -518,8 +534,8 @@
     const u64* vals = (const u64*)d_values[o - 1];
     if (o == 2 && pr->num_routed) {
       CK(zpp_compute(s, B, (const u64*)d_values[0], (u64)P.oracle_w[1] * n, pr->pre_values.p + (u64)(P.oracle_w[0] - pr->num_routed) * n,
-                     P.log_n, pr->num_routed, pr->degree, pr->bg.p, pr->bg.p + P.zs_count, 8, P.zs_count, pr->chunk_q.p, pr->zs_values.p,
-                     (u64)P.oracle_w[2] * n));
+                     P.log_n, pr->num_routed, pr->degree, pr->bg.p, pr->bg.p + P.zs_count, 8, P.zs_count, pr->ptab.p, pr->chunk_q.p,
+                     pr->zs_values.p, (u64)P.oracle_w[2] * n));
       if (pr->lookups.n_luts) {
         CK(lookup_table_polys(s, B, pr->lookups, pr->bg.p, 8, P.zs_count, pr->lut_eval.p));
         CK(lookup_polys(s, B, pr->lookups, (const u64*)d_values[0], (u64)P.oracle_w[1] * n, P.log_n, pr->bg.p, 8, P.zs_count,
@@ -533,18 +549,19 @@
     }
     if (o == 3 && pr->quotient) {
       const u32 nc = P.zs_count;
+      CK(alpha_powers(s, B, pr->alphas.p, 2, nc, pr->apw.p));
       if (pr->gates.n_gates)
-        CK(gate_constraints_lde(s, B, pr->gates, pr->values[0].p, pr->values[1].p, (u64)P.oracle_w[1] * N, P.log_n + 3, pr->alphas.p, 2,
-                                nc, (const u64*)d_pi_hash, pr->qvals.p));
+        CK(gate_constraints_lde(s, B, pr->gates, pr->values[0].p, pr->values[1].p, (u64)P.oracle_w[1] * N, P.log_n + 3, pr->apw.p, nc,
+                                (const u64*)d_pi_hash, pr->qvals.p));
       if (pr->lookups.n_luts)
         CK(quotient_lookup_values(s, B, pr->lookups, pr->values[0].p, pr->gates.num_selectors, pr->values[1].p, (u64)P.oracle_w[1] * N,
                                   pr->values[2].p, (u64)P.oracle_w[2] * N, nc * (pr->num_routed / pr->degree), P.log_n, pr->bg.p, 8,
                                   pr->lut_eval.p, pr->alphas.p, 2, nc, pr->qvals.p));
       CK(quotient_perm_values(s, B, pr->values[1].p, (u64)P.oracle_w[1] * N, pr->values[0].p + (u64)(P.oracle_w[0] - pr->num_routed) * N,
                               pr->values[2].p, (u64)P.oracle_w[2] * N, P.log_n, pr->num_routed, pr->degree, pr->bg.p, 8,
-                              pr->alphas.p, 2, nc, pr->gates.n_gates != 0, pr->qvals.p));
+                              pr->apw.p, MP2G_MAX_GATE_CONSTRAINTS, nc, pr->gates.n_gates != 0, pr->ptab.p, pr->qtab.p, pr->qvals.p));
       CK(c->ntt.run(pr->qvals.p, pr->coeffs[3].p, P.log_n + 3, B * nc, 0, N, N, true, nullptr, false));
-      CK(c->ntt.scale_powers(pr->coeffs[3].p, P.log_n + 3, B * nc, gl_inv(GL_MULT_GEN), 1));
+      CK(c->ntt.scale_table(pr->coeffs[3].p, P.log_n + 3, B * nc, pr->qtab.p + quotient_unshift_offset(P.log_n)));
       CK(commit_oracle_coeffs(pr, 3, B));
     } else {
       NEED(vals, "d_values[o]");
@@ -575,7 +592,7 @@
     r.level_bstride = o ? LW : 0;
     sh.n_polys += r.w;
   }
-  CK(fri_openings(s, sh, B, pr->zeta.p, 2, (u64*)d_openings));
+  CK(fri_openings(s, sh, B, pr->zeta.p, 2, pr->zpw.p, (u64*)d_openings));
   CK(challenger_step(s, V, st, B, (const u64*)d_openings, 2 * pr->n_open, (u32)(2 * pr->n_open), chal, 8, 0));
   STAGE_MARK(pr, 4);
   int rc = fri_tail(pr, sh, st, (u64*)d_proof);
@@ -701,7 +718,8 @@
   NEED(log_n >= 1 && log_n <= 20 && nc >= 1 && nc <= 4, "log_n/nc");
   NEED(degree >= 1 && num_routed >= degree && num_routed % degree == 0 && num_routed / degree <= 16 && num_routed <= wires_w, "num_routed/degree");
   const size_t n = (size_t)1 << log_n, chunks = num_routed / degree;
-  DevBuf dw, ds, dc, dq, dout;
+  DevBuf dw, ds, dc, dq, dout, dt;
+  CK(upload_table(c, dt, perm_table_words(log_n, num_routed), [&](u64* h) { perm_tables_host(log_n, num_routed, h); }));
   CK(dw.alloc(wires_w * n * sizeof(u64)));
   CK(ds.alloc(num_routed * n * sizeof(u64)));
   CK(dc.alloc(2 * nc * sizeof(u64)));
@@ -711,7 +729,7 @@
   CK(hipMemcpyAsync(ds.p, sigmas, num_routed * n * sizeof(u64), hipMemcpyHostToDevice, c->stream));
   CK(hipMemcpyAsync(dc.p, betas, nc * sizeof(u64), hipMemcpyHostToDevice, c->stream));
   CK(hipMemcpyAsync(dc.p + nc, gammas, nc * sizeof(u64), hipMemcpyHostToDevice, c->stream));
-  CK(zpp_compute(c->stream, 1, dw.p, 0, ds.p, log_n, num_routed, degree, dc.p, dc.p + nc, 0, nc, dq.p, dout.p, 0));
+  CK(zpp_compute(c->stream, 1, dw.p, 0, ds.p, log_n, num_routed, degree, dc.p, dc.p + nc, 0, nc, dt.p, dq.p, dout.p, 0));
   CK(hipMemcpyAsync(out, dout.p, nc * chunks * n * sizeof(u64), hipMemcpyDeviceToHost, c->stream));
   CK(hipStreamSynchronize(c->stream));
   return 0;
@@ -757,11 +775,12 @@
   FriShape sh{};
   sh.log_n = b->log_n; sh.rate_bits = b->rate_bits; sh.cap_h = b->cap_h; sh.n_oracles = 1; sh.n_polys = b->w;
   sh.o[0].coeffs = b->coeffs.p; sh.o[0].w = b->w;
-  DevBuf dz, dout;
+  DevBuf dz, dout, dzpw;
   CK(dz.alloc(2 * sizeof(u64)));
   CK(dout.alloc((size_t)b->w * 2 * sizeof(u64)));
+  CK(dzpw.alloc(((size_t)4 << b->log_n) * sizeof(u64)));
   CK(hipMemcpyAsync(dz.p, point, 2 * sizeof(u64), hipMemcpyHostToDevice, c->stream));
-  CK(fri_openings(c->stream, sh, 1, dz.p, 0, dout.p));
+  CK(fri_openings(c->stream, sh, 1, dz.p, 0, dzpw.p, dout.p));
   CK(hipMemcpyAsync(out, dout.p, (size_t)b->w * 2 * sizeof(u64), hipMemcpyDeviceToHost, c->stream));
   CK(hipStreamSynchronize(c->stream));
   return 0;
diff --git a/mapreduce-plonky2_amd/csrc/zperm.h b/mapreduce-plonky2_amd/csrc/zperm.h
--- a/mapreduce-plonky2_amd/csrc/zperm.h
+++ b/mapreduce-plonky2_amd/csrc/zperm.h
@@ -1,12 +1,17 @@
 #pragma once
 #include "gl.cuh"
 namespace mp2g {
+size_t perm_table_words(u32 log_n, u32 num_routed);
+size_t quotient_table_words(u32 log_n);
+void perm_tables_host(u32 log_n, u32 num_routed, u64* out);
+void quotient_tables_host(u32 log_n, u64* out);
+inline size_t quotient_unshift_offset(u32 log_n) { return ((size_t)16 << log_n) + 8; }
 hipError_t zpp_compute(hipStream_t s, u32 B, const u64* wires, u64 wires_bstride, const u64* sigmas, u32 log_n, u32 num_routed,
-                       u32 degree, const u64* betas, const u64* gammas, u64 chal_bstride, u32 nc, u64* chunk_q, u64* out,
-                       u64 out_bstride);
+                       u32 degree, const u64* betas, const u64* gammas, u64 chal_bstride, u32 nc, const u64* ptab, u64* chunk_q,
+                       u64* out, u64 out_bstride);
 hipError_t quotient_perm_values(hipStream_t s, u32 B, const u64* W, u64 w_bstride, const u64* S, const u64* Z, u64 z_bstride,
-                                u32 log_n, u32 num_routed, u32 degree, const u64* bg, u64 bg_bstride, const u64* alphas,
-                                u64 al_bstride, u32 nc, bool gates, u64* q);
+                                u32 log_n, u32 num_routed, u32 degree, const u64* bg, u64 bg_bstride, const u64* apw, u32 apw_len,
+                                u32 nc, bool gates, const u64* ptab, const u64* qtab, u64* q);
 hipError_t zpp_wrap_check(hipStream_t s, u32 B, const u64* chunk_q, const u64* zs, u64 zs_bstride, u32 log_n, u32 chunks, u32 nc,
                           u32* flags);
 }
diff --git a/mapreduce-plonky2_amd/csrc/zperm.hip b/mapreduce-plonky2_amd/csrc/zperm.hip
--- a/mapreduce-plonky2_amd/csrc/zperm.hip
+++ b/mapreduce-plonky2_amd/csrc/zperm.hip
@@ -1,24 +1,27 @@
 #include "zperm.h"
+#include <vector>
 
 namespace mp2g {
 
 #define ZP_MAX_CHUNKS 16
 #define ZP_MAX_ROUTED 256
-__device__ __forceinline__ void fill_k_is(u64* kis, u32 num_routed) {
-  for (u32 j = threadIdx.x; j < num_routed; j += blockDim.x) kis[j] = gl_pow(GL_MULT_GEN, j);
+#define ZP_MAX_TERMS (2 * (1 + ZP_MAX_CHUNKS))
+__device__ __forceinline__ void fill_k_is(u64* kis, const u64* __restrict__ ktab, u32 num_routed) {
+  for (u32 j = threadIdx.x; j < num_routed; j += blockDim.x) kis[j] = ktab[j];
   __syncthreads();
 }
 
 __global__ void __launch_bounds__(256) zpp_chunk_kernel(const u64* __restrict__ wires, u64 wires_bstride, const u64* __restrict__ sigmas,
                                                         u32 log_n, u32 num_routed, u32 degree, const u64* __restrict__ betas,
-                                                        const u64* __restrict__ gammas, u64 chal_bstride, u32 nc, u64* __restrict__ chunk_q) {
+                                                        const u64* __restrict__ gammas, u64 chal_bstride, u32 nc,
+                                                        const u64* __restrict__ ptab, u64* __restrict__ chunk_q) {
   const u32 n = 1u << log_n, i = blockIdx.x * 256 + threadIdx.x, c = blockIdx.y, b = blockIdx.z;
   __shared__ u64 kis[ZP_MAX_ROUTED];
-  fill_k_is(kis, num_routed);
+  fill_k_is(kis, ptab + n, num_routed);
   if (i >= n) return;
   const u32 chunks = num_routed / degree;
   const u64 beta = betas[b * chal_bstride + c], gamma = gammas[b * chal_bstride + c];
-  const u64 bx = gl_mul(beta, gl_pow(gl_root_of_unity(log_n), i));
+  const u64 bx = gl_mul(beta, ptab[i]);
   const u64* w = wires + b * wires_bstride + i;
   const u64* sg = sigmas + i;
   u64 num[ZP_MAX_CHUNKS], den[ZP_MAX_CHUNKS];
@@ -82,37 +85,35 @@
 __global__ void __launch_bounds__(256) quotient_perm_kernel(const u64* __restrict__ W, u64 w_bstride, const u64* __restrict__ S,
                                                             const u64* __restrict__ Z, u64 z_bstride, u32 log_n, u32 num_routed,
                                                             u32 degree, const u64* __restrict__ bg, u64 bg_bstride,
-                                                            const u64* __restrict__ alphas, u64 al_bstride, u32 nc, bool gates,
+                                                            const u64* __restrict__ apw, u32 apw_len, u32 nc, bool gates,
+                                                            const u64* __restrict__ ptab, const u64* __restrict__ qtab,
                                                             u64* __restrict__ q) {
   const u32 lg = log_n + 3;
   const u64 N = (u64)1 << lg;
   const u32 p = blockIdx.x * 256 + threadIdx.x, b = blockIdx.y;
   const u32 i = bitrev32(p, lg);
+  const u32 chunks = num_routed / degree, num_prods = chunks - 1, n_terms = nc * (1 + chunks);
   __shared__ u64 zh_inv[8];
   __shared__ u64 kis[ZP_MAX_ROUTED];
-  fill_k_is(kis, num_routed);
-  if (threadIdx.x < 8) {
-    u64 gn = gl_pow(GL_MULT_GEN, (u64)1 << log_n);
-    zh_inv[threadIdx.x] = gl_inv(gl_sub(gl_mul(gn, gl_pow(gl_root_of_unity(3), threadIdx.x)), 1));
-  }
-  __syncthreads();
+  __shared__ u64 al[2][ZP_MAX_TERMS + 1];
+  if (threadIdx.x < 8) zh_inv[threadIdx.x] = qtab[2 * N + threadIdx.x];
+  for (u32 e = threadIdx.x; e < 2 * (n_terms + 1); e += 256) {
+    const u32 a = e / (n_terms + 1), k = e % (n_terms + 1);
+    al[a][k] = apw[((u64)b * 2 + a) * apw_len + k];
+  }
+  fill_k_is(kis, ptab + (N >> 3), num_routed);
   if (p >= N) return;
-  const u32 chunks = num_routed / degree, num_prods = chunks - 1;
   const u64 pn = bitrev32((i + 8) & (u32)(N - 1), lg);
-  const u64 x = gl_mul(GL_MULT_GEN, gl_pow(gl_root_of_unity(lg), i));
+  const u64 x = qtab[p], l0 = qtab[N + p];
   const u64* w = W + b * w_bstride + p;
   const u64* sg = S + p;
   const u64* z = Z + b * z_bstride;
-  u64 acc[2] = {0, 0}, apow[2] = {1, 1}, al[2];
-  for (u32 a = 0; a < nc; a++) al[a] = alphas[b * al_bstride + a];
+  gl_cols acc[2];
+  u32 kt = 0;
   auto push = [&](u64 term) {
-    for (u32 a = 0; a < nc; a++) {
-      acc[a] = gl_mul_add(term, apow[a], acc[a]);
-      apow[a] = gl_mul(apow[a], al[a]);
-    }
+    for (u32 a = 0; a < nc; a++) acc[a].add(term, al[a][kt]);
+    kt++;
   };
-  const u64 zh = gl_inv(zh_inv[i & 7]);
-  const u64 l0 = gl_mul(zh, gl_inv(gl_mul(((u64)1 << log_n) % GL_P, gl_sub(x, 1))));
   for (u32 c = 0; c < nc; c++) push(gl_mul(l0, gl_sub(z[((u64)c << lg) + p], 1)));
   for (u32 c = 0; c < nc; c++) {
     const u64 beta = bg[b * bg_bstride + c], gamma = bg[b * bg_bstride + nc + c];
@@ -134,16 +135,18 @@
     }
   }
   if (gates)
-    for (u32 a = 0; a < nc; a++) acc[a] = gl_add(acc[a], gl_mul(apow[a], q[(((u64)b * nc + a) << lg) + i]));
-  for (u32 a = 0; a < nc; a++) q[(((u64)b * nc + a) << lg) + i] = gl_mul(acc[a], zh_inv[i & 7]);
+    for (u32 a = 0; a < nc; a++) acc[a].add(q[(((u64)b * nc + a) << lg) + i], al[a][n_terms]);
+  for (u32 a = 0; a < nc; a++) q[(((u64)b * nc + a) << lg) + i] = gl_mul(acc[a].value(), zh_inv[i & 7]);
 }
 hipError_t quotient_perm_values(hipStream_t s, u32 B, const u64* W, u64 w_bstride, const u64* S, const u64* Z, u64 z_bstride,
-                                u32 log_n, u32 num_routed, u32 degree, const u64* bg, u64 bg_bstride, const u64* alphas,
-                                u64 al_bstride, u32 nc, bool gates, u64* q) {
-  if (nc < 1 || nc > 2 || !degree || num_routed % degree || num_routed > ZP_MAX_ROUTED) return hipErrorInvalidValue;
+                                u32 log_n, u32 num_routed, u32 degree, const u64* bg, u64 bg_bstride, const u64* apw, u32 apw_len,
+                                u32 nc, bool gates, const u64* ptab, const u64* qtab, u64* q) {
+  if (nc < 1 || nc > 2 || !degree || num_routed % degree || num_routed > ZP_MAX_ROUTED || num_routed / degree > ZP_MAX_CHUNKS ||
+      apw_len < nc * (1 + num_routed / degree) + 1)
+    return hipErrorInvalidValue;
   const u64 N = (u64)8 << log_n;
   hipLaunchKernelGGL(quotient_perm_kernel, dim3((u32)((N + 255) / 256), B), dim3(256), 0, s, W, w_bstride, S, Z, z_bstride, log_n,
-                     num_routed, degree, bg, bg_bstride, alphas, al_bstride, nc, gates, q);
+                     num_routed, degree, bg, bg_bstride, apw, apw_len, nc, gates, ptab, qtab, q);
   return hipGetLastError();
 }
 
@@ -164,14 +167,55 @@
 }
 
 hipError_t zpp_compute(hipStream_t s, u32 B, const u64* wires, u64 wires_bstride, const u64* sigmas, u32 log_n, u32 num_routed,
-                       u32 degree, const u64* betas, const u64* gammas, u64 chal_bstride, u32 nc, u64* chunk_q, u64* out,
-                       u64 out_bstride) {
+                       u32 degree, const u64* betas, const u64* gammas, u64 chal_bstride, u32 nc, const u64* ptab, u64* chunk_q,
+                       u64* out, u64 out_bstride) {
   if (!degree || num_routed % degree || num_routed / degree > ZP_MAX_CHUNKS || num_routed / degree < 1 || num_routed > ZP_MAX_ROUTED)
     return hipErrorInvalidValue;
   const u32 n = 1u << log_n, chunks = num_routed / degree;
   hipLaunchKernelGGL(zpp_chunk_kernel, dim3((n + 255) / 256, nc, B), dim3(256), 0, s, wires, wires_bstride, sigmas, log_n, num_routed,
-                     degree, betas, gammas, chal_bstride, nc, chunk_q);
+                     degree, betas, gammas, chal_bstride, nc, ptab, chunk_q);
   hipLaunchKernelGGL(zpp_scan_kernel, dim3(nc, B), dim3(1024), 0, s, chunk_q, log_n, chunks, nc, out, out_bstride);
   return hipGetLastError();
 }
-}
+
+size_t perm_table_words(u32 log_n, u32 num_routed) { return ((size_t)1 << log_n) + num_routed; }
+size_t quotient_table_words(u32 log_n) { return quotient_unshift_offset(log_n) + ((size_t)8 << log_n); }
+void perm_tables_host(u32 log_n, u32 num_routed, u64* out) {
+  const size_t n = (size_t)1 << log_n;
+  const u64 w = gl_root_of_unity(log_n);
+  u64 v = 1;
+  for (size_t i = 0; i < n; i++, v = gl_mul(v, w)) out[i] = v;
+  v = 1;
+  for (u32 j = 0; j < num_routed; j++, v = gl_mul(v, GL_MULT_GEN)) out[n + j] = v;
+}
+void quotient_tables_host(u32 log_n, u64* out) {
+  const u32 lg = log_n + 3;
+  const size_t N = (size_t)1 << lg;
+  u64 *tx = out, *tl = out + N, *zh_inv = out + 2 * N, *unshift = out + quotient_unshift_offset(log_n);
+  u64 zh[8];
+  const u64 gn = gl_pow(GL_MULT_GEN, (u64)1 << log_n), w8 = gl_root_of_unity(3);
+  for (u32 r = 0; r < 8; r++) {
+    zh[r] = gl_sub(gl_mul(gn, gl_pow(w8, r)), 1);
+    zh_inv[r] = gl_inv(zh[r]);
+  }
+  std::vector<u64> x(N), pre(N);
+  const u64 wN = gl_root_of_unity(lg), n_mod = ((u64)1 << log_n) % GL_P;
+  u64 v = GL_MULT_GEN, acc = 1;
+  for (size_t i = 0; i < N; i++, v = gl_mul(v, wN)) {
+    x[i] = v;
+    pre[i] = acc;
+    acc = gl_mul(acc, gl_mul(n_mod, gl_sub(v, 1)));
+  }
+  u64 inv = gl_inv(acc);
+  for (size_t i = N; i-- > 0;) {
+    const u64 d = gl_mul(n_mod, gl_sub(x[i], 1));
+    const u32 p = bitrev32((u32)i, lg);
+    tx[p] = x[i];
+    tl[p] = gl_mul(zh[i & 7], gl_mul(inv, pre[i]));
+    inv = gl_mul(inv, d);
+  }
+  const u64 g_inv = gl_inv(GL_MULT_GEN);
+  v = 1;
+  for (size_t k = 0; k < N; k++, v = gl_mul(v, g_inv)) unshift[k] = v;
+}
+}
```
